# RunpeiDong/ACT

Hardware: AMD Instinct MI355X
Metric: stage2_pretrain_point_clouds_per_sec (higher is better)
Workload: dtype f32

## Files before the change

act_amd/_abi.py:

```python
import ctypes

_vp, _i, _f, _sz = ctypes.c_void_p, ctypes.c_int, ctypes.c_float, ctypes.c_size_t
_u, _u64, _ll, _str = ctypes.c_uint, ctypes.c_uint64, ctypes.c_longlong, ctypes.c_char_p
_d = ctypes.c_double
_P = ctypes.POINTER


class GemmEpilogue(ctypes.Structure):
    _fields_ = [("alpha", _f), ("act", _i), ("accumulate", _i), ("rows_per_scale", _i), ("ldr", _i), ("ldaux", _i),
                ("res_row_div", _i), ("bias", _vp), ("rowscale", _vp), ("res", _vp), ("aux", _vp)]


class GemmTnProblem(ctypes.Structure):
    _fields_ = [("A", _vp), ("lda", _i), ("B", _vp), ("ldb", _i), ("C", _vp), ("ldc", _i), ("M", _i), ("N", _i), ("bias_out", _vp)]


class GemmFx(ctypes.Structure):
    _fields_ = ([(n, _vp) for n in ("a_scale", "a_shift", "b_scale", "b_shift", "tile_stats", "gmax", "garg")] + [("group", _i), ("store_c", _i)]
                + [(n, _vp) for n in ("sa_src", "sa_arg", "ep_src", "ep_arg", "row_groups")])


class BlockParams(ctypes.Structure):
    _fields_ = [(n, _vp) for n in ("norm1_w", "norm1_b", "qkv_w", "qkv_b", "proj_w", "proj_b", "norm2_w", "norm2_b",
                                   "fc1_w", "fc1_b", "fc2_w", "fc2_b")]


class BlockDims(ctypes.Structure):
    _fields_ = [("B", _i), ("S", _i), ("D", _i), ("heads", _i), ("hidden", _i), ("eps", _f)]


class BlockStack(ctypes.Structure):
    _fields_ = [("depth", _i), ("blocks", _vp), ("gate1", _vp), ("gate2", _vp)]


class PrefixVit(ctypes.Structure):
    _fields_ = ([(n, _i) for n in ("B", "P", "G", "D", "heads", "hidden", "depth", "tokens_dims", "pos_hidden")] +
                [("eps", _f), ("drop_p", _f), ("seed_base", _u64), ("seed_dev", _vp)] +
                [(n, _vp) for n in ("pos_w0", "pos_b0", "pos_w1", "pos_b1", "pre_w", "pre_b", "post_w", "post_b", "norm_w", "norm_b")] +
                [("prompt_tok", _P(_vp)), ("prompt_pos", _P(_vp)), ("blocks", _P(BlockParams))])


class VitBf16x3(ctypes.Structure):
    _fields_ = [("w_planes", _vp), ("a_planes", _vp), ("a_planes_elems", _sz)]


class VitF16x3(ctypes.Structure):
    _fields_ = [("w_planes", _vp), ("w_inv_scale", _vp), ("a_scale", _vp), ("a_planes", _vp), ("a_planes_elems", _sz)]


class PointnetParams(ctypes.Structure):
    _fields_ = [(n, _vp) for n in ("c1_w", "c1_b", "bn1_w", "bn1_b", "c2_w", "c2_b", "c3_w", "c3_b", "bn2_w", "bn2_b", "c4_w", "c4_b",
                                   "bn1_mean", "bn1_var", "bn2_mean", "bn2_var")]


class PointnetGrads(ctypes.Structure):
    _fields_ = [(n, _vp) for n in ("c1_w", "c1_b", "bn1_w", "bn1_b", "c2_w", "c2_b", "c3_w", "c3_b", "bn2_w", "bn2_b", "c4_w", "c4_b")]


class PointnetDims(ctypes.Structure):
    _fields_ = [("BG", _i), ("n", _i), ("C", _i), ("eps1", _f), ("eps2", _f), ("momentum1", _f), ("momentum2", _f)]


class Dgcnn(ctypes.Structure):
    _fields_ = ([(n, _i) for n in ("B", "G", "k", "Cin", "Cout", "groups")] + [("eps", _f), ("slope", _f)] +
                [(n, _vp) for n in ("w_in", "b_in", "w5")] + [("stacked", _vp * 4), ("gn_w", _vp * 4), ("gn_b", _vp * 4)])


class DgcnnF16x3(ctypes.Structure):
    _fields_ = [("w5_planes", _vp), ("w5_inv_scale", _vp), ("a_scale", _f), ("a_planes", _vp), ("a_planes_elems", _sz)]


class AugmentOp(ctypes.Structure):
    _fields_ = [("kind", _i), ("p0", _f), ("p1", _f), ("p2", _f), ("draws", _vp), ("draws2", _vp)]


STRUCTS = {
    "act_gemm_epilogue_t": GemmEpilogue, "act_gemm_tn_problem_t": GemmTnProblem, "act_gemm_fx_t": GemmFx,
    "act_block_params_t": BlockParams, "act_block_grads_t": BlockParams, "act_block_dims_t": BlockDims, "act_block_stack_t": BlockStack,
    "act_prefix_vit_t": PrefixVit, "act_vit_bf16x3_t": VitBf16x3, "act_vit_f16x3_t": VitF16x3,
    "act_pointnet_params_t": PointnetParams,
    "act_pointnet_grads_t": PointnetGrads, "act_pointnet_dims_t": PointnetDims, "act_dgcnn_t": Dgcnn, "act_dgcnn_f16x3_t": DgcnnF16x3,
    "act_augment_op_t": AugmentOp,
}

_epi, _probs, _fx = _P(GemmEpilogue), _P(GemmTnProblem), _P(GemmFx)
_dims, _blk, _x3 = _P(BlockDims), _P(BlockParams), _P(VitBf16x3)
_pnd, _pnp = _P(PointnetDims), _P(PointnetParams)

_TABLE = {
    "act_version": [],
    "act_arch": (_str, []),
    "act_prof_enable": [_i],
    "act_prof_reset": [],
    "act_prof_num_kernels": [],
    "act_prof_kernel_name": (_str, [_i]),
    "act_prof_read": [_i, _vp, _vp, _vp, _vp],
    "act_fps_scratch_floats": (_sz, [_i, _i]),
    "act_fps_f32": [_vp, _i, _i, _i, _vp, _vp, _i, _vp, _vp],
    "act_fps_chain_probe": [_i, _i, _vp, _vp, _vp, _vp],
    "act_knn_group_f32": [_vp, _vp, _i, _i, _i, _i, _vp, _i, _vp, _vp, _vp],
    "act_gather_points_f32": [_vp, _vp, _i, _i, _i, _i, _vp, _vp],
    "act_gather_points_bwd_f32": [_vp, _vp, _i, _i, _i, _i, _vp, _vp],
    "act_scale_translate_f32": [_vp, _vp, _vp, _i, _i, _vp],
    "act_rotate_points_f32": [_vp, _vp, _i, _i, _vp],
    "act_augment_f32": [_vp, _i, _i, _P(AugmentOp), _i, _u64, _vp, _i, _vp],
    "act_chamfer_fwd_f32": [_vp, _vp, _i, _i, _i, _vp, _vp, _vp, _vp, _vp],
    "act_chamfer_fwd_ex_f32": [_vp, _vp, _i, _i, _i, _vp, _vp, _vp, _vp, _i, _vp],
    "act_chamfer_bwd_f32": [_vp, _vp, _vp, _vp, _vp, _vp, _i, _i, _i, _vp, _vp, _vp],
    "act_sgemm_f32": [_i, _i, _i, _i, _i, _vp, _i, _vp, _i, _vp, _i, _epi, _vp, _sz, _vp],
    "act_sgemm_ex_f32": [_i, _i, _i, _i, _i, _vp, _i, _vp, _i, _vp, _i, _epi, _vp, _sz, _i, _i, _vp],
    "act_sgemm_tn_grouped_workspace": (_sz, [_probs, _i, _i, _i]),
    "act_sgemm_tn_grouped_splits": [_probs, _i, _i],
    "act_sgemm_tn_grouped_f32": [_probs, _i, _i, _i, _vp, _sz, _vp],
    "act_sgemm_fx_tile_stats_floats": (_sz, [_i, _i]),
    "act_gemm_fx_asm": [_i],
    "act_sgemm_fx_f32": [_i, _i, _i, _i, _i, _vp, _i, _vp, _i, _vp, _i, _epi, _fx, _vp, _sz, _vp],
    "act_bn_tiles_finalize_f32": [_vp, _i, _i, _i, _vp, _vp, _f, _f, _vp, _vp, _vp, _vp, _vp, _vp, _vp],
    "act_layernorm_fwd_f32": [_vp, _vp, _vp, _vp, _vp, _vp, _vp, _vp, _i, _i, _f, _vp],
    "act_prompt_layernorm_fwd_f32": [_vp, _vp, _i, _i, _i, _f, _u64, _vp, _vp, _vp, _f, _vp, _vp],
    "act_prompt_rows_fwd_f32": [_vp, _vp, _vp, _i, _i, _i, _f, _u64, _vp, _vp],
    "act_prompt_rows_bwd_f32": [_vp, _vp, _i, _i, _i, _f, _u64, _vp, _vp, _vp],
    "act_layernorm_bwd_workspace": (_sz, [_i, _i]),
    "act_layernorm_bwd_f32": [_vp, _vp, _vp, _vp, _vp, _vp, _vp, _vp, _vp, _i, _vp, _sz, _i, _i, _vp],
    "act_colsum_workspace": (_sz, [_i, _i]),
    "act_colsum_f32": [_vp, _i, _i, _i, _vp, _i, _vp, _sz, _vp],
    "act_attention_fwd_f32": [_vp, _vp, _vp, _i, _i, _i, _i, _f, _vp],
    "act_attention_fwd_prefix_f32": [_vp, _i, _vp, _i, _vp, _vp, _i, _i, _i, _f, _vp],
    "act_attention_bwd_f32": [_vp, _vp, _vp, _vp, _vp, _i, _i, _i, _i, _f, _vp],
    "act_attention_bwd_prefix_f32": [_vp, _i, _vp, _i, _vp, _vp, _vp, _vp, _vp, _i, _i, _i, _f, _vp],
    "act_cosine_loss_fwd_f32": [_vp, _vp, _i, _i, _f, _vp, _vp, _vp, _vp],
    "act_cosine_loss_bwd_f32": [_vp, _vp, _vp, _vp, _i, _i, _f, _vp, _vp],
    "act_regression_loss_fwd_f32": [_vp, _vp, _i, _i, _i, _vp, _vp, _vp],
    "act_regression_loss_bwd_f32": [_vp, _vp, _vp, _i, _i, _i, _vp, _vp],
    "act_softmax_xent_fwd_f32": [_vp, _vp, _i, _i, _vp, _vp, _vp, _vp],
    "act_softmax_xent_bwd_f32": [_vp, _vp, _vp, _vp, _i, _i, _vp, _vp],
    "act_colstats_workspace": (_sz, [_i, _i]),
    "act_bn_stats_f32": [_vp, _i, _i, _vp, _vp, _f, _f, _vp, _vp, _vp, _vp, _vp, _vp, _vp, _sz, _vp],
    "act_affine_act_f32": [_vp, _vp, _vp, _i, _i, _i, _vp, _vp],
    "act_bn_bwd_f32": [_vp, _vp, _vp, _vp, _vp, _vp, _i, _i, _i, _vp, _vp, _vp, _vp, _sz, _vp],
    "act_bn_bwd_groups_f32": [_vp, _vp, _vp, _vp, _vp, _vp, _i, _i, _i, _vp, _i, _vp, _vp, _vp, _vp, _sz, _vp],
    "act_col_mean_var_f32": [_vp, _i, _i, _vp, _vp, _vp, _sz, _vp],
    "act_bn_bwd_sums_f32": [_vp, _vp, _vp, _vp, _vp, _vp, _i, _i, _i, _vp, _vp, _vp, _sz, _vp],
    "act_bn_bwd_apply_f32": [_vp, _vp, _vp, _vp, _vp, _vp, _vp, _vp, _f, _i, _i, _i, _vp, _vp],
    "act_group_max_f32": [_vp, _i, _i, _i, _vp, _vp, _vp],
    "act_group_max_bwd_f32": [_vp, _vp, _i, _i, _i, _i, _vp, _vp],
    "act_group_max_bwd_matmul_f32": [_vp, _vp, _i, _i, _i, _vp, _i, _i, _vp, _i, _vp],
    "act_group_live_i32": [_vp, _i, _i, _vp, _vp],
    "act_group_max_bwd_matmul_live_f32": [_vp, _vp, _i, _i, _i, _vp, _i, _i, _vp, _i, _vp, _vp],
    "act_group_max_bwd_wgrad_workspace": (_sz, [_i, _i, _i, _i]),
    "act_group_max_bwd_wgrad_f32": [_vp, _vp, _i, _i, _i, _vp, _i, _i, _vp, _vp, _vp, _i, _vp, _sz, _vp],
    "act_group_sum_f32": [_vp, _i, _i, _i, _vp, _vp],
    "act_edge_gn_lrelu_max_f32": [_vp, _i, _i, _vp, _i, _i, _i, _i, _i, _vp, _vp, _f, _f, _vp, _vp, _i, _i, _vp],
    "act_edge_gn_lrelu_max_bwd_f32": [_vp, _i, _i, _vp, _i, _i, _i, _i, _i, _vp, _vp, _vp, _f, _vp, _i, _vp, _vp, _vp, _vp],
    "act_edge_bwd_lds": [_i],
    "act_gn_gumbel_argmax_gather_f32": [_vp, _i, _i, _i, _i, _vp, _vp, _f, _f, _vp, _u64, _vp, _f, _vp, _i, _vp, _vp, _vp, _vp, _vp],
    "act_gumbel_softmax_fwd_f32": [_vp, _i, _i, _vp, _u64, _f, _vp, _vp],
    "act_gumbel_softmax_bwd_f32": [_vp, _vp, _i, _i, _f, _vp, _vp],
    "act_kl_uniform_fwd_f32": [_vp, _i, _i, _i, _vp, _vp, _vp, _vp],
    "act_kl_uniform_bwd_f32": [_vp, _vp, _vp, _vp, _i, _i, _i, _vp, _vp],
    "act_split_bf16x2_f32": [_vp, _i, _i, _i, _vp, _vp, _vp],
    "act_sgemm_nt_bf16x3_supported": [_i, _i, _i],
    "act_sgemm_nt_bf16x3_f32": [_i, _i, _i, _vp, _vp, _vp, _vp, _vp, _i, _epi, _vp],
    "act_layernorm_fwd_planes_f32": [_vp, _vp, _vp, _vp, _vp, _vp, _vp, _vp, _vp, _vp, _i, _i, _f, _vp],
    "act_prompt_layernorm_fwd_planes_f32": [_vp, _vp, _i, _i, _i, _f, _u64, _vp, _vp, _vp, _f, _vp, _vp, _vp],
    "act_attention_fwd_prefix_planes_f32": [_vp, _i, _vp, _i, _vp, _vp, _vp, _vp, _i, _i, _i, _f, _vp],
    "act_sgemm_nt_bf16x3_planes_f32": [_i, _i, _i, _vp, _vp, _vp, _vp, _vp, _i, _vp, _vp, _epi, _vp],
    "act_split_f16x2_f32": [_vp, _i, _i, _i, _f, _vp, _vp, _vp, _vp],
    "act_sgemm_nt_f16x3_supported": [_i, _i, _i],
    "act_sgemm_nt_f16x3_planes_f32": [_i, _i, _i, _vp, _vp, _f, _vp, _vp, _vp, _vp, _i, _vp, _vp, _f, _epi, _vp],
    "act_sgemm_nt_f16x3_pick_tile": [_i, _i, _i, _i],
    "act_sgemm_nt_f16x3_planes_tile_f32": [_i, _i, _i, _vp, _vp, _f, _vp, _vp, _vp, _vp, _i, _vp, _vp, _f, _epi, _vp, _i],
    "act_layernorm_fwd_f16_planes_f32": [_vp, _vp, _vp, _vp, _vp, _vp, _vp, _vp, _f, _vp, _vp, _i, _i, _f, _vp],
    "act_attention_fwd_prefix_f16_planes_f32": [_vp, _i, _vp, _i, _vp, _vp, _vp, _f, _vp, _i, _i, _i, _f, _vp],
    "act_gemm_tune_set": [_i] * 7,
    "act_gemm_tune_get": [_i] * 5 + [_P(_i), _P(_i)],
    "act_gemm_tune_clear": [],
    "act_gemm_tile_info": [_i] + [_P(_i)] * 4,
    "act_scale_rows_f32": [_vp, _vp, _i, _i, _i, _vp, _vp],
    "act_bn_eval_affine_f32": [_vp, _vp, _vp, _vp, _f, _i, _vp, _vp, _vp],
    "act_composite_collect_begin": [],
    "act_composite_collect_end": [_P(_i), _i],
    "act_composite_shutdown": [],
    "act_block_saved_floats": (_sz, [_dims]),
    "act_block_fwd_f32": [_dims, _blk, _vp, _vp, _vp, _vp, _i, _vp, _vp, _vp, _sz, _vp],
    "act_block_bwd_scratch_floats": (_sz, [_dims]),
    "act_block_bwd_f32": [_dims, _blk, _vp, _vp, _vp, _vp, _vp, _blk, _vp, _vp, _sz, _vp, _sz, _vp, _vp],
    "act_block_stack_saved_floats": (_sz, [_dims, _i, _i]),
    "act_block_stack_bwd_scratch_floats": (_sz, [_dims, _i]),
    "act_block_stack_fwd_f32": [_dims, _P(BlockStack), _vp, _vp, _i, _vp, _vp, _vp, _sz, _vp],
    "act_block_stack_bwd_f32": [_dims, _P(BlockStack), _vp, _vp, _vp, _vp, _vp, _vp, _vp, _vp, _sz, _vp, _sz, _vp, _vp],
    "act_add_f32": [_vp, _vp, _vp, _ll, _vp],
    "act_prefix_block_saved_floats": (_sz, [_dims, _i]),
    "act_prefix_block_fwd_f32": [_dims, _i, _blk, _vp, _vp, _vp, _vp, _i, _vp, _vp, _vp, _sz, _vp],
    "act_prefix_block_fwd_kv_f32": [_dims, _i, _blk, _vp, _vp, _vp, _vp, _vp, _vp, _sz, _vp],
    "act_prompt_kv_sparse": [_i],
    "act_prompt_kv_workspace": (_sz, [_i, _i, _i, _i]),
    "act_prompt_kv_fwd_f32": [_vp, _vp, _i, _i, _i, _i, _f, _u64, _vp, _vp, _vp, _f, _vp, _vp, _vp, _vp, _sz, _vp, _sz, _vp],
    "act_prefix_block_bwd_scratch_floats": (_sz, [_dims, _i]),
    "act_prefix_block_bwd_f32": [_dims, _i, _blk, _vp, _vp, _vp, _vp, _vp, _vp, _vp, _sz, _vp],
    "act_prefix_vit_scratch_floats": (_sz, [_P(PrefixVit)]),
    "act_prefix_vit_fwd_bf16x3_f32": [_P(PrefixVit), _x3, _vp, _vp, _vp, _vp, _vp, _sz, _vp],
    "act_prefix_block_fwd_bf16x3_f32": [_dims, _i, _blk, _x3, _vp, _vp, _vp, _i, _vp, _vp, _vp, _sz, _vp],
    "act_prefix_block_bwd_bf16x3_f32": [_dims, _i, _blk, _x3, _vp, _vp, _vp, _vp, _vp, _vp, _vp, _sz, _vp],
    "act_prefix_vit_fwd_f32": [_P(PrefixVit), _vp, _vp, _vp, _vp, _vp, _sz, _vp],
    "act_prefix_vit_fwd_f16x3_f32": [_P(PrefixVit), _P(VitF16x3), _vp, _vp, _vp, _vp, _vp, _sz, _vp],
    "act_pointnet_saved_floats": (_sz, [_pnd]),
    "act_pointnet_fwd_f32": [_pnd, _pnp, _vp, _i, _i, _vp, _vp, _vp, _sz, _vp],
    "act_pointnet_fwd_groups_f32": [_pnd, _pnp, _vp, _i, _i, _vp, _vp, _vp, _i, _vp, _sz, _vp],
    "act_pointnet_bwd_scratch_floats": (_sz, [_pnd]),
    "act_pointnet_bwd_f32": [_pnd, _pnp, _vp, _vp, _vp, _P(PointnetGrads), _vp, _vp, _sz, _vp],
    "act_dgcnn_scratch_floats": (_sz, [_P(Dgcnn)]),
    "act_dgcnn_features_f32": [_P(Dgcnn), _vp, _vp, _vp, _vp, _vp, _sz, _vp],
    "act_dgcnn_features_f16x3_f32": [_P(Dgcnn), _P(DgcnnF16x3), _vp, _vp, _vp, _vp, _vp, _sz, _vp],
    "act_three_nn_f32": [_vp, _vp, _i, _i, _i, _vp, _vp, _vp, _vp, _vp],
    "act_interp_rows_fwd_f32": [_vp, _vp, _vp, _vp, _vp, _vp, _i, _i, _i, _i, _vp, _vp],
    "act_interp_rows_bwd_f32": [_vp, _vp, _vp, _vp, _i, _i, _i, _i, _vp, _vp],
    "act_interp_xyz_grad_workspace": (_sz, [_ll, _i]),
    "act_interp_xyz_grad_f32": [_vp, _vp, _ll, _i, _vp, _vp, _vp, _sz, _vp],
    "act_log_softmax_fwd_f32": [_vp, _ll, _i, _vp, _vp],
    "act_log_softmax_bwd_f32": [_vp, _vp, _ll, _i, _vp, _vp],
    "act_nll_weighted_workspace": (_sz, [_ll]),
    "act_nll_weighted_fwd_f32": [_vp, _vp, _vp, _ll, _i, _vp, _vp, _vp, _vp, _sz, _vp],
    "act_nll_weighted_bwd_f32": [_vp, _vp, _vp, _vp, _ll, _i, _vp, _vp],
    "act_confusion_i64": [_vp, _vp, _ll, _i, _vp, _vp],
    "act_label_branch_fwd_f32": [_vp, _vp, _vp, _vp, _i, _i, _f, _f, _f, _vp, _vp, _vp, _vp],
    "act_label_branch_bwd_f32": [_vp, _vp, _vp, _vp, _vp, _i, _f, _f, _vp, _vp, _vp, _vp],
    "act_part_eval_f32": [_vp, _vp, _i, _i, _i, _vp, _vp, _i, _vp, _vp, _i, _i, _vp, _vp, _vp],
    "act_scene_member_workspace": (_sz, [_ll, _i, _i]),
    "act_scene_member_count": [_vp, _ll, _vp, _i, _i, _vp, _vp, _vp, _sz, _vp],
    "act_scene_member_fill": [_vp, _ll, _vp, _i, _i, _vp, _vp, _vp, _sz, _vp],
    "act_scene_rows": [_vp, _vp, _vp, _vp, _i, _ll, _i, _u, _u, _u, _vp, _vp],
    "act_scene_gather": [_vp, _ll, _vp, _vp, _vp, _vp, _i, _ll, _vp, _vp],
    "act_scene_vote": [_vp, _vp, _ll, _ll, _i, _vp, _vp, _vp, _vp],
    "act_scene_finish": [_vp, _vp, _ll, _i, _vp, _vp, _vp],
    "act_s3dis_sample_workspace": (_sz, [_i, _ll]),
    "act_s3dis_sample_f32": [_vp, _vp, _vp, _i, _vp, _vp, _vp, _vp, _d, _d, _i, _i, _ll, _vp, _vp, _vp, _i, _i, _u, _u, _vp, _vp, _vp, _vp, _vp, _vp,
                             _vp, _sz, _vp],
    "act_cloud_sample_max_points": [],
    "act_cloud_sample_f32": [_vp, _ll, _i, _i, _vp, _vp, _i, _i, _u, _u, _i, _vp, _vp, _vp],
    "act_recon_eval_f32": [_vp, _vp, _vp, _i, _i, _i, _i, _f, _vp, _i, _i, _vp],
    "act_svm_scores_f32": [_vp, _vp, _vp, _vp, _i, _i, _i, _vp, _vp],
    "act_svm_hinge_workspace": (_sz, [_i, _i]),
    "act_svm_hinge_f32": [_vp, _vp, _vp, _i, _i, _vp, _vp, _vp, _sz, _vp],
    "act_svm_tprod_workspace": (_sz, [_i, _i, _i]),
    "act_svm_tprod_f32": [_vp, _vp, _i, _i, _i, _vp, _vp, _vp, _sz, _vp],
    "act_svm_newton_workspace": (_sz, [_i, _i, _i]),
    "act_svm_newton_f32": [_vp, _vp, _vp, _i, _i, _i, _f, _f, _i, _vp, _vp, _vp, _vp, _vp, _sz, _vp],
    "act_tsne_knn_workspace": (_sz, [_i, _i]),
    "act_tsne_knn_cosine_f32": [_vp, _i, _i, _i, _vp, _vp, _vp, _sz, _vp],
    "act_tsne_conditional_p_f32": [_vp, _i, _i, _f, _vp, _vp, _vp],
    "act_tsne_symmetrize_workspace": (_sz, [_i, _i]),
    "act_tsne_symmetrize_f32": [_vp, _vp, _i, _i, _vp, _vp, _vp, _ll, _vp, _sz, _vp],
    "act_tsne_step_workspace": (_sz, [_i]),
    "act_tsne_step_f32": [_vp, _vp, _vp, _i, _f, _f, _f, _vp, _vp, _vp, _vp, _sz, _vp],
    "act_tsne_steps_f32": [_vp, _vp, _vp, _i, _i, _f, _f, _f, _vp, _vp, _vp, _vp, _sz, _vp],
    "act_tsne_kl_f32": [_vp, _vp, _vp, _vp, _i, _vp, _vp, _sz, _vp],
    "act_tsne_pca_workspace": (_sz, [_i, _i]),
    "act_tsne_pca_init_f32": [_vp, _i, _i, _vp, _vp, _vp, _sz, _vp],
    "act_dropout_add_layernorm_fwd_f32": [_vp, _vp, _vp, _i, _i, _f, _u64, _vp, _vp, _vp, _f, _vp, _vp, _vp],
    "act_dropout_add_layernorm_bwd_f32": [_vp, _vp, _vp, _i, _i, _f, _u64, _vp, _vp, _vp, _vp, _vp, _vp, _vp],
    "act_attention_dropout_fwd_f32": [_vp, _vp, _vp, _vp, _i, _i, _i, _i, _f, _f, _u64, _vp, _vp],
    "act_attention_dropout_bwd_f32": [_vp, _vp, _vp, _vp, _vp, _vp, _vp, _i, _i, _i, _i, _f, _f, _u64, _vp, _vp],
    "act_quickgelu_fwd_f32": [_vp, _vp, _i, _i, _vp],
    "act_quickgelu_bwd_f32": [_vp, _vp, _vp, _i, _i, _vp],
    "act_knn_probe_normalize_f32": [_vp, _i, _i, _vp, _vp],
    "act_knn_probe_splits": [_i, _i, _i, _i],
    "act_knn_probe_workspace": (_sz, [_i, _i, _i, _i, _i]),
    "act_knn_probe_search_f32": [_vp, _i, _vp, _i, _i, _i, _i, _i, _i, _vp, _vp, _vp, _sz, _vp],
    "act_knn_probe_vote_f32": [_vp, _vp, _i, _i, _vp, _i, _vp, _i, _P(_i), _i, _f, _vp, _vp, _vp, _vp],
    "act_emd_max_points": [],
    "act_emd_fwd_f32": [_vp, _vp, _i, _i, _f, _i, _vp, _vp, _vp, _vp],
    "act_emd_fwd_ex_f32": [_vp, _vp, _i, _i, _f, _i, _vp, _vp, _vp, _vp, _vp],
    "act_emd_bwd_f32": [_vp, _vp, _vp, _vp, _i, _i, _vp, _vp, _vp],
    "act_emd_wave_max_points": [],
    "act_emd_wave_fwd_f32": [_vp, _vp, _i, _i, _f, _f, _i, _vp, _vp, _vp, _vp, _vp],
    "act_ball_query_f32": [_vp, _vp, _i, _i, _i, _f, _i, _i, _vp, _vp, _vp],
    "act_group_rows_fwd_f32": [_vp, _vp, _vp, _vp, _i, _i, _i, _i, _i, _i, _vp, _vp],
    "act_group_rows_bwd_workspace": (_sz, [_i, _i, _i, _i]),
    "act_group_rows_bwd_f32": [_vp, _vp, _i, _i, _i, _i, _i, _i, _vp, _vp, _sz, _vp],
    "act_group_gather_f32": [_vp, _vp, _i, _i, _i, _i, _i, _vp, _vp],
    "act_group_gather_bwd_f32": [_vp, _vp, _i, _i, _i, _i, _i, _vp, _vp, _sz, _vp],
    "act_three_nn_any_f32": [_vp, _vp, _i, _i, _i, _vp, _vp, _vp, _vp, _vp, _vp],
    "act_three_adj_i32": [_vp, _i, _i, _i, _vp, _vp, _vp],
    "act_interp_rows_any_fwd_f32": [_vp, _vp, _vp, _i, _i, _i, _i, _vp, _vp],
    "act_interp_rows_any_bwd_f32": [_vp, _vp, _vp, _vp, _i, _i, _i, _i, _vp, _vp],
    "act_knn_feat_f32": [_vp, _i, _i, _i, _i, _vp, _vp, _vp],
    "act_edge_bn_workspace": (_sz, [_i, _i, _i, _i]),
    "act_edge_bn_lrelu_max_fwd_f32": [_vp, _i, _i, _vp, _i, _i, _i, _i, _vp, _vp, _vp, _vp, _i, _f, _f, _f, _vp, _i, _i, _vp, _vp, _vp, _vp,
                                      _vp, _vp, _sz, _vp],
    "act_edge_bn_lrelu_max_bwd_f32": [_vp, _i, _i, _vp, _i, _i, _i, _i, _vp, _vp, _vp, _vp, _vp, _f, _vp, _vp, _vp, _i, _vp, _vp, _vp, _vp, _sz, _vp],
    "act_affine_lrelu_f32": [_vp, _vp, _vp, _f, _i, _i, _vp, _vp],
    "act_bn_lrelu_bwd_workspace": (_sz, [_i, _i]),
    "act_bn_lrelu_bwd_f32": [_vp, _vp, _vp, _vp, _vp, _vp, _f, _i, _i, _vp, _vp, _vp, _vp, _sz, _vp],
}

SIGNATURES = {name: sig if isinstance(sig, tuple) else (_i, sig) for name, sig in _TABLE.items()}
```

act_amd/composite.py:

```python
import ctypes
import math
import os
import weakref

import torch

from . import _C
from . import kernels as K
from ._abi import BlockDims, BlockParams, BlockStack, Dgcnn, PointnetDims, PointnetGrads, PointnetParams, PrefixVit, VitBf16x3, VitF16x3, DgcnnF16x3
from ._abi import GemmFx

lib, check = _C.lib, _C.check
_vp, _i = ctypes.c_void_p, ctypes.c_int

ENABLED = os.environ.get("ACT_COMPOSITE", "1") != "0"


def _p(t):
    if t is None:
        return None
    if not t.is_cuda or not t.is_contiguous():
        raise _C.ActHipError("act_amd kernels need contiguous CUDA tensors (there is no CPU fallback)")
    _C._same_device(t)
    return t.data_ptr()


K.publish_table()
_TUNED = set()
_SHAPE_BUF = (_i * (5 * 256))()


def _tune_shape(ak, bk, M, N, Kd, device):
    return lib.act_gemm_tune_get(ak, bk, M, N, Kd, None, None) == 0 or K.gemm_config(ak, bk, M, N, Kd, device, publish=True) is not None


def ensure_tuned(key, call, device):
    if key in _TUNED:
        return
    check(lib.act_composite_collect_begin(), "act_composite_collect_begin")
    try:
        rc = call()
    finally:
        n = lib.act_composite_collect_end(_SHAPE_BUF, 256)
    check(rc, "composite dry call")
    done = True
    for i in range(min(n, 256)):
        done = _tune_shape(*[int(_SHAPE_BUF[5 * i + j]) for j in range(5)], device) and done
    if done:
        _TUNED.add(key)


def reset_tuning():
    _TUNED.clear()
    lib.act_gemm_tune_clear()
    K.publish_table()


def shutdown():
    torch.cuda.synchronize()
    return int(lib.act_composite_shutdown())


_DIMS = {}


def _block_dims(B, S, D, heads, hidden, eps):
    key = (B, S, D, heads, hidden, float(eps))
    d = _DIMS.get(key)
    if d is None:
        d = BlockDims(B, S, D, heads, hidden, float(eps))
        _DIMS[key] = d = (d, int(lib.act_block_saved_floats(ctypes.byref(d))), int(lib.act_block_bwd_scratch_floats(ctypes.byref(d))))
    return d


def _block_params(n1w, n1b, wqkv, bqkv, wproj, bproj, n2w, n2b, w1, b1, w2, b2):
    return BlockParams(_p(n1w), _p(n1b), _p(wqkv), _p(bqkv), _p(wproj), _p(bproj), _p(n2w), _p(n2b), _p(w1), _p(b1), _p(w2), _p(b2))


class BlockFn(torch.autograd.Function):

    @staticmethod
    def forward(ctx, x, pos, gate1, gate2, n1w, n1b, wqkv, bqkv, wproj, bproj, n2w, n2b, w1, b1, w2, b2, heads, eps, train_w):
        B, S, D = x.shape
        dev = x.device
        dims, n_saved, _ = _block_dims(B, S, D, heads, w1.shape[0], eps)
        x2d = K._f32c(x).reshape(B * S, D)
        pos2d = K._f32c(pos).reshape(B * S, D) if pos is not None else None
        need_grad = any(ctx.needs_input_grad)
        prm = _block_params(n1w, n1b, wqkv, bqkv, wproj, bproj, n2w, n2b, w1, b1, w2, b2)
        saved = torch.empty(n_saved, dtype=torch.float32, device=dev)
        out = torch.empty(B, S, D, dtype=torch.float32, device=dev)
        ws = K.workspace(dev)
        args = (ctypes.byref(dims), ctypes.byref(prm), _p(x2d), _p(pos2d), _p(gate1), _p(gate2), int(need_grad), _p(saved), _p(out),
                _p(ws), ws.numel() * 4)
        ensure_tuned(("blk_fwd", B, S, D, heads, w1.shape[0]), lambda: lib.act_block_fwd_f32(*args, _C.stream()), dev)
        check(lib.act_block_fwd_f32(*args, _C.stream()), "act_block_fwd_f32")
        if need_grad:
            ctx.save_for_backward(saved, gate1, gate2, n1w, wqkv, bqkv, wproj, n2w, w1, w2)
            ctx.dims = (B, S, D, heads, w1.shape[0], eps)
            ctx.has_pos = pos is not None
            ctx.train_w = int(train_w)
        return out

    @staticmethod
    def backward(ctx, dout):
        saved, gate1, gate2, n1w, wqkv, bqkv, wproj, n2w, w1, w2 = ctx.saved_tensors
        B, S, D, heads, hidden, eps = ctx.dims
        dev = dout.device
        dims, _, n_scratch = _block_dims(B, S, D, heads, hidden, eps)
        dout = K._f32c(dout).reshape(B * S, D)
        tw = ctx.train_w
        prm = _block_params(n1w, None, wqkv, bqkv, wproj, None, n2w, None, w1, None, w2, None)
        dx = torch.empty(B, S, D, dtype=torch.float32, device=dev)
        scratch = torch.empty(n_scratch, dtype=torch.float32, device=dev)
        grads, gp = (None,) * 12, None
        if tw:
            e = lambda *shape: torch.empty(*shape, dtype=torch.float32, device=dev)
            grads = (e(D), e(D), e(3 * D, D), e(3 * D) if bqkv is not None else None, e(D, D), e(D), e(D), e(D),
                     e(hidden, D), e(hidden), e(D, hidden), e(D))
            gp = ctypes.byref(BlockParams(*[_p(g) for g in grads]))
        ws = K.workspace(dev)
        side, sws = None, None
        if tw == 2 and K.OVERLAP_DW:
            side = K.side_stream(dev, 1).cuda_stream
            sws = K.workspace(dev, stream_handle=side)
        args = (ctypes.byref(dims), ctypes.byref(prm), _p(gate1), _p(gate2), _p(saved), _p(dout), _p(dx), gp, _p(scratch),
                _p(ws), ws.numel() * 4, _p(sws), (sws.numel() * 4 if sws is not None else 0))
        ensure_tuned(("blk_bwd", B, S, D, heads, hidden, bool(tw)), lambda: lib.act_block_bwd_f32(*args, _C.stream(), side), dev)
        check(lib.act_block_bwd_f32(*args, _C.stream(), side), "act_block_bwd_f32")
        dg1, dbt1, dwqkv, dbqkv, dwproj, dbproj, dg2, dbt2, dw1, db1, dw2, db2 = grads
        return (dx, dx if ctx.has_pos else None, None, None, dg1, dbt1, dwqkv, dbqkv, dwproj, dbproj, dg2, dbt2,
                dw1, db1, dw2, db2, None, None, None)


STACK = os.environ.get("ACT_BLOCK_STACK", "1") != "0"
STACK_CHUNK = int(os.environ.get("ACT_BLOCK_STACK_CHUNK", "0"))
_SDIMS = {}
_NPB = 12


def _stack_dims(B, S, D, heads, hidden, eps, depth):
    key = (B, S, D, heads, hidden, float(eps), depth)
    d = _SDIMS.get(key)
    if d is None:
        dims = BlockDims(B, S, D, heads, hidden, float(eps))
        r = ctypes.byref(dims)
        _SDIMS[key] = d = (dims, int(lib.act_block_stack_saved_floats(r, depth, 1)), int(lib.act_block_stack_saved_floats(r, depth, 0)),
                           int(lib.act_block_stack_bwd_scratch_floats(r, depth)))
    return d


def _ptr_array(tensors, dev_index):
    ptrs = []
    for t in tensors:
        if t is None:
            ptrs.append(None)
            continue
        if not t.is_cuda or not t.is_contiguous() or t.device.index != dev_index:
            raise _C.ActHipError("act_amd kernels need contiguous CUDA tensors on the current device (there is no CPU fallback)")
        ptrs.append(t.data_ptr())
    return (_vp * len(ptrs))(*ptrs)


class BlockStackFn(torch.autograd.Function):

    @staticmethod
    def forward(ctx, x, pos, gates, heads, eps, train_w, emit_pos, *params):
        B, S, D = x.shape
        dev = x.device
        depth = len(params) // _NPB
        hidden = params[8].shape[0]
        dims, n_keep, n_nokeep, _ = _stack_dims(B, S, D, heads, hidden, eps, depth)
        _C._same_device(x)
        x2d = K._f32c(x).reshape(B * S, D)
        pos2d = K._f32c(pos).reshape(B * S, D) if pos is not None else None
        need_grad = any(ctx.needs_input_grad)
        parr = _ptr_array(params, dev.index)
        g1 = g2 = None
        gts = ()
        if gates is not None and any(g is not None for g in gates):
            gts = tuple(t for g in gates for t in (g if g is not None else (None, None)))
            g1, g2 = _ptr_array(gts[0::2], dev.index), _ptr_array(gts[1::2], dev.index)
        st = BlockStack(depth, ctypes.cast(parr, _vp), ctypes.cast(g1, _vp) if g1 is not None else None,
                        ctypes.cast(g2, _vp) if g2 is not None else None)
        saved = torch.empty(n_keep if need_grad else n_nokeep, dtype=torch.float32, device=dev)
        out = torch.empty(B, S, D, dtype=torch.float32, device=dev)
        ws = K.workspace(dev)
        args = (ctypes.byref(dims), ctypes.byref(st), x2d.data_ptr(), pos2d.data_ptr() if pos2d is not None else None, int(need_grad),
                saved.data_ptr(), out.data_ptr(), ws.data_ptr(), ws.numel() * 4)
        ensure_tuned(("stack_fwd", B, S, D, heads, hidden, depth), lambda: lib.act_block_stack_fwd_f32(*args, _C.stream()), dev)
        check(lib.act_block_stack_fwd_f32(*args, _C.stream()), "act_block_stack_fwd_f32")
        ctx.set_materialize_grads(False)
        if need_grad:
            ctx.save_for_backward(saved, *[t for t in params if t is not None], *[t for t in gts if t is not None])
            ctx.layout = ([t is not None for t in params], [t is not None for t in gts])
            ctx.dims = (B, S, D, heads, hidden, eps, depth)
            ctx.has_pos = pos is not None
            ctx.train_w = int(train_w)
        return (out, pos) if emit_pos else out

    @staticmethod
    def backward(ctx, dout, dpos_in=None):
        sv = ctx.saved_tensors
        saved = sv[0]
        B, S, D, heads, hidden, eps, depth = ctx.dims
        dev = saved.device
        it = iter(sv[1:])
        params = tuple(next(it) if has else None for has in ctx.layout[0])
        gts = tuple(next(it) if has else None for has in ctx.layout[1])
        parr = _ptr_array(params, dev.index)
        g1 = g2 = None
        if gts:
            g1, g2 = _ptr_array(gts[0::2], dev.index), _ptr_array(gts[1::2], dev.index)
        st = BlockStack(depth, ctypes.cast(parr, _vp), ctypes.cast(g1, _vp) if g1 is not None else None,
                        ctypes.cast(g2, _vp) if g2 is not None else None)
        dims, _, _, n_scratch = _stack_dims(B, S, D, heads, hidden, eps, depth)
        tw = ctx.train_w
        dx = torch.empty(B, S, D, dtype=torch.float32, device=dev)
        if dout is None:
            dout = torch.zeros(B * S, D, dtype=torch.float32, device=dev)
        dout = K._f32c(dout).reshape(B * S, D)
        if dpos_in is not None:
            dpos_in = K._f32c(dpos_in).reshape(B * S, D)
        dpos = torch.empty(B, S, D, dtype=torch.float32, device=dev) if (ctx.has_pos and (depth > 1 or dpos_in is not None)) else None
        scratch = torch.empty(n_scratch, dtype=torch.float32, device=dev)
        grads, garr = (None,) * len(params), None
        if tw:
            grads = tuple(torch.empty_like(t) if t is not None else None for t in params)
            garr = _ptr_array(grads, dev.index)
        ws = K.workspace(dev)
        side, sws = None, None
        if tw == 2 and K.OVERLAP_DW:
            side = K.side_stream(dev, 1).cuda_stream
            sws = K.workspace(dev, stream_handle=side)
        args = (ctypes.byref(dims), ctypes.byref(st), saved.data_ptr(), dout.data_ptr(), dx.data_ptr(), dpos.data_ptr() if dpos is not None else None,
                dpos_in.data_ptr() if (dpos_in is not None and dpos is not None) else None,
                ctypes.cast(garr, _vp) if garr is not None else None, scratch.data_ptr(), ws.data_ptr(), ws.numel() * 4,
                sws.data_ptr() if sws is not None else None, (sws.numel() * 4 if sws is not None else 0))
        ensure_tuned(("stack_bwd", B, S, D, heads, hidden, depth, bool(tw)), lambda: lib.act_block_stack_bwd_f32(*args, _C.stream(), side), dev)
        check(lib.act_block_stack_bwd_f32(*args, _C.stream(), side), "act_block_stack_bwd_f32")
        return (dx, (dpos if dpos is not None else dx) if ctx.has_pos else None, None, None, None, None, None) + grads


_LEAVES = weakref.WeakKeyDictionary()
_VIT_LEAVES = weakref.WeakKeyDictionary()
_VIT_STRUCT = weakref.WeakKeyDictionary()
_VIT_PLANES = weakref.WeakKeyDictionary()
TEACHER_BF16X3 = os.environ.get("ACT_TEACHER_BF16X3", "0") == "1"
TEACHER_BF16X3_BWD = os.environ.get("ACT_TEACHER_BF16X3_BWD", "1") == "1"
TEACHER_F16X3 = os.environ.get("ACT_TEACHER_F16X3", "1") != "0"
_VIT_F16 = weakref.WeakKeyDictionary()
TOKENIZER_F16X3 = os.environ.get("ACT_TOKENIZER_F16X3", "1") != "0"
_DGCNN_F16 = weakref.WeakKeyDictionary()


def _stack_leaves(blocks):
    cache = _LEAVES.get(blocks)
    if cache is None or len(cache) != len(blocks) or any(c[6] is not b for c, b in zip(cache, blocks)):
        cache = _LEAVES[blocks] = [(b.norm1, b.attn.qkv, b.attn.proj, b.norm2, b.mlp.fc1, b.mlp.fc2, b) for b in blocks]
    return cache


def _stock_blocks(blocks):
    from act_amd.models.act import Block
    for b in blocks:
        if type(b).forward is not Block.forward or b._forward_hooks or b._forward_pre_hooks or b._backward_hooks or b._backward_pre_hooks:
            return False
    return True


def block_stack(blocks, x, pos, gates, draws=None, tag="enc", chunk=None, taps=False):
    n = len(blocks)

    def per_block(x, draws):
        outs = []
        every = chunk if chunk else n
        for i, blk in enumerate(blocks):
            x = blk(x, pos, draws, f"{tag}.{i}", gates[i] if gates is not None else None)
            if (i + 1) % every == 0 or i == n - 1:
                outs.append(x)
        return outs if taps else x
    if not (ENABLED and STACK) or n == 0 or not _stock_blocks(blocks):
        return per_block(x, draws)
    if draws is not None:
        gates = [blk.gates(x.shape[0], x.device, draws, f"{tag}.{i}") for i, blk in enumerate(blocks)]
        gates = [tuple(g) if g[0] is not None else None for g in gates]
    leaves = _stack_leaves(blocks)
    b0 = blocks[0]
    heads, eps, tw = b0.attn.num_heads, b0.norm1.eps, (2 if b0.overlap_wgrad else 1)
    if any(l[6].attn.num_heads != heads or l[0].eps != eps or l[3].eps != eps or bool(l[6].overlap_wgrad) != bool(b0.overlap_wgrad) for l in leaves[1:]):
        return per_block(x, None)
    if chunk is None:
        chunk = STACK_CHUNK
    chunk = chunk if chunk > 0 else n
    carry = pos is not None and chunk < n and torch.is_grad_enabled() and pos.requires_grad
    outs = []
    for c0 in range(0, n, chunk):
        params = []
        for n1, qkv, proj, n2, fc1, fc2, _ in leaves[c0:c0 + chunk]:
            p1, pq, pp, p2, pf1, pf2 = n1._parameters, qkv._parameters, proj._parameters, n2._parameters, fc1._parameters, fc2._parameters
            params += [p1["weight"], p1["bias"], pq["weight"], pq["bias"], pp["weight"], pp["bias"], p2["weight"], p2["bias"],
                       pf1["weight"], pf1["bias"], pf2["weight"], pf2["bias"]]
        emit = carry and c0 + chunk < n
        r = BlockStackFn.apply(x, pos, gates[c0:c0 + chunk] if gates is not None else None, heads, eps, tw, emit, *params)
        x, pos = r if emit else (r, pos)
        outs.append(x)
    return outs if taps else x


_PDIMS = {}


def _prefix_dims(B, G, D, heads, hidden, eps, P):
    key = (B, G, D, heads, hidden, float(eps), P)
    d = _PDIMS.get(key)
    if d is None:
        d = BlockDims(B, G, D, heads, hidden, float(eps))
        _PDIMS[key] = d = (d, int(lib.act_prefix_block_saved_floats(ctypes.byref(d), P)),
                           int(lib.act_prefix_block_bwd_scratch_floats(ctypes.byref(d), P)))
    return d


class PrefixBlockFn(torch.autograd.Function):

    @staticmethod
    def forward(ctx, x2d, pos2d, prm2d, B, P, G, n1w, n1b, wqkv, bqkv, wproj, bproj, n2w, n2b, w1, b1, w2, b2, heads, eps):
        D = x2d.shape[1]
        dev = x2d.device
        dims, n_saved, _ = _prefix_dims(B, G, D, heads, w1.shape[0], eps, P)
        x2d, pos2d, prm2d = K._f32c(x2d), K._f32c(pos2d), K._f32c(prm2d)
        prm = _block_params(n1w, n1b, wqkv, bqkv, wproj, bproj, n2w, n2b, w1, b1, w2, b2)
        saved = torch.empty(n_saved, dtype=torch.float32, device=dev)
        out = torch.empty(B * G, D, dtype=torch.float32, device=dev)
        ws = K.workspace(dev)
        args = (ctypes.byref(dims), P, ctypes.byref(prm), _p(x2d), _p(pos2d), _p(prm2d), None, 1, _p(saved), _p(out), _p(ws), ws.numel() * 4)
        ensure_tuned(("pfx_fwd", B, G, D, heads, w1.shape[0], P), lambda: lib.act_prefix_block_fwd_f32(*args, _C.stream()), dev)
        if TEACHER_BF16X3 and not any(w.requires_grad for w in (wqkv, wproj, w1, w2)):
            x3, keep = _block_planes((wqkv, wproj, w1, w2), B * G * w1.shape[0] + B * max(G, P) * D, dev)
            check(lib.act_prefix_block_fwd_bf16x3_f32(*args[:3], ctypes.byref(x3), *args[3:6], 1, *args[8:], _C.stream()), "act_prefix_block_fwd_bf16x3_f32")
            del keep
            ctx.x3 = True
        else:
            check(lib.act_prefix_block_fwd_f32(*args, _C.stream()), "act_prefix_block_fwd_f32")
            ctx.x3 = False
        ctx.save_for_backward(saved, prm2d, n1w, wqkv, wproj, n2w, w1, w2)
        ctx.dims = (B, P, G, D, heads, w1.shape[0], eps)
        return out

    @staticmethod
    def backward(ctx, dout):
        saved, prm2d, n1w, wqkv, wproj, n2w, w1, w2 = ctx.saved_tensors
        B, P, G, D, heads, hidden, eps = ctx.dims
        dev = dout.device
        dims, _, n_scratch = _prefix_dims(B, G, D, heads, hidden, eps, P)
        dout = K._f32c(dout)
        prm = _block_params(n1w, None, wqkv, None, wproj, None, n2w, None, w1, None, w2, None)
        dx = torch.empty(B * G, D, dtype=torch.float32, device=dev)
        dprm = torch.empty(B * P, D, dtype=torch.float32, device=dev)
        scratch = torch.empty(n_scratch, dtype=torch.float32, device=dev)
        ws = K.workspace(dev)
        args = (ctypes.byref(dims), P, ctypes.byref(prm), _p(prm2d), _p(saved), _p(dout), _p(dx), _p(dprm), _p(scratch), _p(ws), ws.numel() * 4)
        ensure_tuned(("pfx_bwd", B, G, D, heads, hidden, P), lambda: lib.act_prefix_block_bwd_f32(*args, _C.stream()), dev)
        if ctx.x3 and TEACHER_BF16X3_BWD:
            x3, keep = _block_planes((wqkv, wproj, w1, w2), B * G * hidden + B * max(G, P) * D, dev, transposed=True)
            check(lib.act_prefix_block_bwd_bf16x3_f32(*args[:3], ctypes.byref(x3), *args[3:], _C.stream()), "act_prefix_block_bwd_bf16x3_f32")
            del keep
            return (dx, dx, dprm) + (None,) * 17
        check(lib.act_prefix_block_bwd_f32(*args, _C.stream()), "act_prefix_block_bwd_f32")
        return (dx, dx, dprm) + (None,) * 17


def block_forward_prefix(x2d, pos2d, prm2d, B, P, G, n1w, n1b, wqkv, bqkv, wproj, bproj, n2w, n2b, w1, b1, w2, b2, heads, eps, n1p=None, kvp=None):
    D = x2d.shape[1]
    dev = x2d.device
    dims, n_saved, _ = _prefix_dims(B, G, D, heads, w1.shape[0], eps, P)
    x2d, pos2d = K._f32c(x2d), K._f32c(pos2d)
    prm2d = K._f32c(prm2d) if prm2d is not None else None
    n1p = K._f32c(n1p) if n1p is not None else None
    prm = _block_params(n1w, n1b, wqkv, bqkv, wproj, bproj, n2w, n2b, w1, b1, w2, b2)
    tmp = torch.empty(n_saved, dtype=torch.float32, device=dev)
    out = torch.empty(B * G, D, dtype=torch.float32, device=dev)
    ws = K.workspace(dev)
    if kvp is not None:
        kargs = (ctypes.byref(dims), P, ctypes.byref(prm), _p(x2d), _p(pos2d), _p(K._f32c(kvp)), _p(tmp), _p(out), _p(ws), ws.numel() * 4)
        ensure_tuned(("pfx_fwd_kv", B, G, D, heads, w1.shape[0], P), lambda: lib.act_prefix_block_fwd_kv_f32(*kargs, _C.stream()), dev)
        check(lib.act_prefix_block_fwd_kv_f32(*kargs, _C.stream()), "act_prefix_block_fwd_kv_f32")
        return out
    args = (ctypes.byref(dims), P, ctypes.byref(prm), _p(x2d), _p(pos2d), _p(prm2d), _p(n1p), 0, _p(tmp), _p(out), _p(ws), ws.numel() * 4)
    ensure_tuned(("pfx_fwd", B, G, D, heads, w1.shape[0], P), lambda: lib.act_prefix_block_fwd_f32(*args, _C.stream()), dev)
    check(lib.act_prefix_block_fwd_f32(*args, _C.stream()), "act_prefix_block_fwd_f32")
    return out


def _vit_tensors(tok):
    lv = _VIT_LEAVES.get(tok)
    blocks = tok.visual_embed[0]
    if lv is None or lv[0] is not blocks:
        vp = tok.visual_pos_embed
        lv = _VIT_LEAVES[tok] = (blocks, vp[0], vp[2], tok.proj_pre, tok.proj_post, tok.visual_embed[1])
    _, vp0, vp2, pre, post, nrm = lv
    ts = []
    for m in (vp0, vp2, pre, post, nrm):
        pr = m._parameters
        ts += [pr["weight"], pr["bias"]]
    for n1, qkv, proj, n2, fc1, fc2, _ in _stack_leaves(blocks):
        p1, pq, pp, p2, pf1, pf2 = n1._parameters, qkv._parameters, proj._parameters, n2._parameters, fc1._parameters, fc2._parameters
        ts += [p1["weight"], p1["bias"], pq["weight"], pq["bias"], pp["weight"], pp["bias"], p2["weight"], p2["bias"],
               pf1["weight"], pf1["bias"], pf2["weight"], pf2["bias"]]
    tp = tok._parameters
    ts += [tp["visual_prompt_token"], tp["visual_prompt_pos"], tp.get("deep_prompt_tokens"), tp.get("deep_prompt_pos")]
    return ts, blocks


def prefix_vit_forward(tok, tokens, center, drop_p, seed_base, seed_dev):
    B, G, td = tokens.shape
    dev = tokens.device
    ts, blocks = _vit_tensors(tok)
    depth = tok.visual_embed_depth
    sig = (B, G, td, dev.index, depth, tuple([t.data_ptr() if t is not None else 0 for t in ts]))
    cache = _VIT_STRUCT.get(tok)
    if cache is None or cache[0] != sig:
        Pn, D = tok.num_prompt_token, tok.visual_embed_dim
        b0 = blocks[0]
        if depth > 1 and (ts[-2] is None or ts[-1] is None):
            raise _C.ActHipError("prefix_vit_forward: a depth > 1 prompt-tuned Transformer needs deep_prompt_tokens / deep_prompt_pos")
        ptr = _ptr_array(ts, dev.index)
        m = PrefixVit()
        m.B, m.P, m.G, m.D, m.heads, m.hidden, m.depth, m.tokens_dims, m.pos_hidden = (B, Pn, G, D, b0.num_heads, ts[18].shape[0], depth, td,
                                                                                        ts[0].shape[0])
        m.eps = float(b0.eps)
        (m.pos_w0, m.pos_b0, m.pos_w1, m.pos_b1, m.pre_w, m.pre_b, m.post_w, m.post_b, m.norm_w, m.norm_b) = [ptr[i] for i in range(10)]
        row = Pn * D * 4
        nb = 10 + _NPB * depth
        toks = (_vp * depth)(*[ptr[nb] if i == 0 else ptr[nb + 2] + (i - 1) * row for i in range(depth)])
        poss = (_vp * depth)(*[ptr[nb + 1] if i == 0 else ptr[nb + 3] + (i - 1) * row for i in range(depth)])
        blks = (_vp * (_NPB * depth))(*[ptr[10 + i] for i in range(_NPB * depth)])
        m.prompt_tok, m.prompt_pos, m.blocks = toks, poss, ctypes.cast(blks, ctypes.POINTER(BlockParams))
        n_scratch = int(lib.act_prefix_vit_scratch_floats(ctypes.byref(m)))
        cache = _VIT_STRUCT[tok] = (sig, m, n_scratch, (toks, poss, blks, ptr))
    _, m, n_scratch, _ = cache
    m.drop_p, m.seed_base, m.seed_dev = float(drop_p), int(seed_base) & (2 ** 64 - 1), _p(seed_dev)
    scratch = torch.empty(n_scratch, dtype=torch.float32, device=dev)
    out = torch.empty(B, G, td, dtype=torch.float32, device=dev)
    ws = K.workspace(dev)
    tokens, center = K._f32c(tokens), K._f32c(center)
    args = (ctypes.byref(m), _p(tokens), _p(center), _p(out), _p(scratch), _p(ws), ws.numel() * 4)
    ensure_tuned(("vit", B, m.P, G, m.D, m.heads, m.hidden, depth, td), lambda: lib.act_prefix_vit_fwd_f32(*args, _C.stream()), dev)
    if TEACHER_BF16X3:
        x3, keep = _vit_planes(tok, ts, depth, B * G * m.hidden + B * max(G, m.P) * m.D, dev)
        check(lib.act_prefix_vit_fwd_bf16x3_f32(args[0], ctypes.byref(x3), *args[1:], _C.stream()), "act_prefix_vit_fwd_bf16x3_f32")
        del keep
        return out
    if TEACHER_F16X3:
        x3, keep = _vit_f16_planes(tok, ts, depth, B * G * m.hidden + B * max(G, m.P) * m.D, dev)
        check(lib.act_prefix_vit_fwd_f16x3_f32(args[0], ctypes.byref(x3), *args[1:], _C.stream()), "act_prefix_vit_fwd_f16x3_f32")
        del keep
        return out
    check(lib.act_prefix_vit_fwd_f32(*args, _C.stream()), "act_prefix_vit_fwd_f32")
    return out


_BLOCK_PLANES = {}


def _block_planes(ws_, act_elems, dev, transposed=False):
    sig = tuple((w.data_ptr(), w._version) for w in ws_)
    key = (id(ws_[0]), transposed)
    cache = _BLOCK_PLANES.get(key)
    if cache is None or cache[0]() is not ws_[0] or cache[1] != sig:
        with torch.no_grad():
            if transposed:
                wqkv, wproj, w1, w2 = (w.detach() for w in ws_)
                D = wqkv.shape[1]
                src = [w2.t(), w1.t(), wproj.t(), wqkv.t(), wqkv[D:].t()]
            else:
                src = [w.detach() for w in ws_]
            planes = [K.split_bf16x2(w.contiguous()) for w in src]
        parr = (_vp * len(planes))(*[pl.data_ptr() for pl in planes])
        cache = _BLOCK_PLANES[key] = (weakref.ref(ws_[0], lambda _, k=key: _BLOCK_PLANES.pop(k, None)), sig, planes, parr)
    a_planes = torch.empty(2 * act_elems, dtype=torch.bfloat16, device=dev)
    return VitBf16x3(ctypes.cast(cache[3], _vp), a_planes.data_ptr(), a_planes.numel()), (a_planes, cache)


def _vit_planes(tok, ts, depth, act_elems, dev):
    ws_ = [ts[10 + _NPB * i + j] for i in range(depth) for j in (2, 4, 8, 10)]
    sig = tuple((w.data_ptr(), w._version) for w in ws_)
    cache = _VIT_PLANES.get(tok)
    if cache is None or cache[0] != sig:
        with torch.no_grad():
            planes = [K.split_bf16x2(w.detach()) for w in ws_]
        parr = (_vp * len(planes))(*[pl.data_ptr() for pl in planes])
        cache = _VIT_PLANES[tok] = (sig, planes, parr)
    a_planes = torch.empty(2 * act_elems, dtype=torch.bfloat16, device=dev)
    x3 = VitBf16x3(ctypes.cast(cache[2], _vp), a_planes.data_ptr(), a_planes.numel())
    return x3, (a_planes, cache)


def f16x3_act_scale(bound):
    bound = float(bound)
    if not math.isfinite(bound) or bound > 32768.0:
        return 0.0
    if bound < 2.0 ** -15:
        return 2.0 ** 30
    s = 2.0 ** (math.frexp(32768.0 / bound)[1] - 1)
    return s if bound * s <= 32768.0 else s / 2


def f16x3_vit_bounds(ts, depth, D):
    rows, rt = [], math.sqrt(D)
    for i in range(depth):
        n1w, n1b, wqkv, bqkv, _, _, n2w, n2b, w1, b1 = (None if t is None else t.detach().double() for t in ts[10 + _NPB * i: 20 + _NPB * i])
        u1, u2 = rt * n1w.abs() + n1b.abs(), rt * n2w.abs() + n2b.abs()
        v = wqkv[2 * D:].abs() @ u1 + (bqkv[2 * D:].abs() if bqkv is not None else 0)
        h = w1.abs() @ u2 + (b1.abs() if b1 is not None else 0)
        rows.append(torch.stack([u1.max(), v.max(), u2.max(), h.max()]))
    return torch.stack(rows)


def _vit_f16_planes(tok, ts, depth, act_elems, dev):
    blk = ts[10:10 + _NPB * depth]
    sig = tuple((t.data_ptr(), t._version) if t is not None else None for t in blk)
    cache = _VIT_F16.get(tok)
    if cache is None or cache[0] != sig:
        ws_ = [ts[10 + _NPB * i + j] for i in range(depth) for j in (2, 4, 8, 10)]
        with torch.no_grad():
            scales = [K.f16x3_row_scales(w) for w in ws_]
            planes = [K.split_f16x2(w.detach(), 1.0, sc[0]) for w, sc in zip(ws_, scales)]
            inv = [sc[1].contiguous() for sc in scales]
            a_scale = [f16x3_act_scale(b) for b in f16x3_vit_bounds(ts, depth, ws_[0].shape[1]).flatten().tolist()]
        parr = (_vp * len(planes))(*[pl.data_ptr() for pl in planes])
        iarr = (_vp * len(inv))(*[t.data_ptr() for t in inv])
        sarr = (ctypes.c_float * len(a_scale))(*a_scale)
        cache = _VIT_F16[tok] = (sig, planes, inv, a_scale, (parr, iarr, sarr))
    a_planes = torch.empty(2 * act_elems, dtype=torch.float16, device=dev)
    parr, iarr, sarr = cache[4]
    x3 = VitF16x3(ctypes.cast(parr, _vp), ctypes.cast(iarr, _vp), ctypes.cast(sarr, _vp), a_planes.data_ptr(), a_planes.numel())
    return x3, (a_planes, cache)


def _pointnet_structs(enc, BG, n):
    c1, bn1, _, c2 = enc.first_conv
    c3, bn2, _, c4 = enc.second_conv
    dims = PointnetDims(BG, n, c4.weight.shape[0], float(bn1.eps), float(bn2.eps), float(bn1.momentum), float(bn2.momentum))
    return dims, (c1, bn1, c2, c3, bn2, c4)


class PointnetFn(torch.autograd.Function):

    @staticmethod
    def forward(ctx, x, c1w, c1b, g1, b1, c2w, c2b, c3w, c3b, g2, b2, c4w, c4b, buffers, dims, training, groups=None):
        dev = x.device
        x = K._f32c(x)
        need_grad = any(ctx.needs_input_grad)
        prm = PointnetParams(*[_p(t) for t in (c1w, c1b, g1, b1, c2w, c2b, c3w, c3b, g2, b2, c4w, c4b) + tuple(buffers)])
        saved = torch.empty(int(lib.act_pointnet_saved_floats(ctypes.byref(dims))), dtype=torch.float32, device=dev)
        out = torch.empty(dims.BG, dims.C, dtype=torch.float32, device=dev)
        ws = K.workspace(dev)
        ng = 0 if groups is None else int(groups.numel())
        args = (ctypes.byref(dims), ctypes.byref(prm), _p(x), int(training), int(need_grad), _p(saved), _p(out),
                _p(groups) if ng else None, ng, _p(ws), ws.numel() * 4)
        ensure_tuned(("pn_fwd", dims.BG, dims.n, dims.C, ng), lambda: lib.act_pointnet_fwd_groups_f32(*args, _C.stream()), dev)
        check(lib.act_pointnet_fwd_groups_f32(*args, _C.stream()), "act_pointnet_fwd_groups_f32")
        if need_grad:
            ctx.save_for_backward(x, saved, c1w, c1b, g1, b1, c2w, c2b, c3w, c3b, g2, b2, c4w, c4b)
            ctx.dims, ctx.training = dims, bool(training)
        return out

    @staticmethod
    def backward(ctx, dout):
        if not ctx.training:
            raise NotImplementedError("mini-PointNet backward in eval mode (running statistics) is off the training path")
        x, saved = ctx.saved_tensors[:2]
        params = ctx.saved_tensors[2:]
        dims = ctx.dims
        dev = dout.device
        dout = K._f32c(dout)
        prm = PointnetParams(*([_p(t) for t in params] + [None] * 4))
        grads = tuple(torch.empty_like(t) for t in params)
        gp = PointnetGrads(*[_p(g) for g in grads])
        scratch = torch.empty(int(lib.act_pointnet_bwd_scratch_floats(ctypes.byref(dims))), dtype=torch.float32, device=dev)
        ws = K.workspace(dev)
        args = (ctypes.byref(dims), ctypes.byref(prm), _p(x), _p(saved), _p(dout), ctypes.byref(gp), _p(scratch), _p(ws), ws.numel() * 4)
        ensure_tuned(("pn_bwd", dims.BG, dims.n, dims.C), lambda: lib.act_pointnet_bwd_f32(*args, _C.stream()), dev)
        check(lib.act_pointnet_bwd_f32(*args, _C.stream()), "act_pointnet_bwd_f32")
        return (None,) + grads + (None, None, None, None)


def pointnet_forward(enc, point_groups, need=None):
    bs, g, n, _ = point_groups.shape
    groups = None
    if need is not None and need.shape[1] < g and n in (32, 64):
        ids = (need + torch.arange(bs, device=need.device).unsqueeze(1) * g).reshape(-1).to(torch.int32)
        pad = (-ids.numel()) % (128 // n)
        groups = torch.cat([ids, ids[-1:].expand(pad)]) if pad else ids
        groups = groups.contiguous()
    dims, (c1, bn1, c2, c3, bn2, c4) = _pointnet_structs(enc, bs * g, n)
    training = enc.training
    if training:
        for bn in (bn1, bn2):
            if bn.num_batches_tracked is not None:
                bn.num_batches_tracked.add_(1)
    w2 = lambda c: c.weight.view(c.weight.shape[0], c.weight.shape[1])
    out = PointnetFn.apply(point_groups.reshape(bs * g * n, 3), w2(c1), c1.bias, bn1.weight, bn1.bias, w2(c2), c2.bias, w2(c3), c3.bias,
                           bn2.weight, bn2.bias, w2(c4), c4.bias,
                           (bn1.running_mean, bn1.running_var, bn2.running_mean, bn2.running_var), dims, training, groups)
    return out.reshape(bs, g, dims.C)


def dgcnn_features(dg, f, idx, stacked):
    B, G, Cin = f.shape
    dev = f.device
    w5 = dg.layer5[0].weight
    m = Dgcnn()
    gn0 = dg.layer1[1]
    m.B, m.G, m.k, m.Cin, m.Cout, m.groups = B, G, idx.shape[1], Cin, w5.shape[0], gn0.num_groups
    m.eps, m.slope = float(gn0.eps), 0.2
    m.w_in, m.b_in, m.w5 = _p(dg.input_trans.weight), _p(dg.input_trans.bias), _p(w5)
    for l, layer in enumerate((dg.layer1, dg.layer2, dg.layer3, dg.layer4)):
        m.stacked[l], m.gn_w[l], m.gn_b[l] = _p(stacked[l]), _p(layer[1].weight), _p(layer[1].bias)
    scratch = torch.empty(int(lib.act_dgcnn_scratch_floats(ctypes.byref(m))), dtype=torch.float32, device=dev)
    h = torch.empty(B * G, m.Cout, dtype=torch.float32, device=dev)
    ws = K.workspace(dev)
    f = K._f32c(f)
    args = (ctypes.byref(m), _p(f), _p(idx), _p(h), _p(scratch), _p(ws), ws.numel() * 4)
    ensure_tuned(("dgcnn", B, G, Cin, m.Cout), lambda: lib.act_dgcnn_features_f32(*args, _C.stream()), dev)
    if TOKENIZER_F16X3 and m.Cout >= 1024:
        x3, keep = _dgcnn_f16_planes(dg, B * G, G, m.k, dev)
        check(lib.act_dgcnn_features_f16x3_f32(args[0], ctypes.byref(x3), *args[1:], _C.stream()), "act_dgcnn_features_f16x3_f32")
        del keep
        return h
    check(lib.act_dgcnn_features_f32(*args, _C.stream()), "act_dgcnn_features_f32")
    return h


def f16x3_dgcnn_bound(gmax, bmax, couts, groups, G, k):
    return max(math.sqrt((c // g) * G * k) * gm + bm for gm, bm, c, g in zip(gmax, bmax, couts, groups))


def _dgcnn_f16_planes(dg, T, G, k, dev):
    gns = [layer[1] for layer in (dg.layer1, dg.layer2, dg.layer3, dg.layer4)]
    w5 = dg.layer5[0].weight
    sig = tuple((t.data_ptr(), t._version) for t in [w5] + [t for gn in gns for t in (gn.weight, gn.bias)])
    cache = _DGCNN_F16.get(dg)
    if cache is None or cache[0] != sig:
        with torch.no_grad():
            w = w5.detach().reshape(w5.shape[0], w5.shape[1])
            scale, inv = K.f16x3_row_scales(w)
            planes = K.split_f16x2(w, 1.0, scale)
            inv = inv.contiguous()
            mx = torch.stack([t.detach().double().abs().max() for gn in gns for t in (gn.weight, gn.bias)]).tolist()
        cache = _DGCNN_F16[dg] = (sig, planes, inv, mx[0::2], mx[1::2], [gn.num_channels for gn in gns], [gn.num_groups for gn in gns], {})
    _, planes, inv, gmax, bmax, couts, groups, scales = cache
    a_scale = scales.get((G, k))
    if a_scale is None:
        a_scale = scales[(G, k)] = f16x3_act_scale(f16x3_dgcnn_bound(gmax, bmax, couts, groups, G, k))
    a_planes = torch.empty(2 * T * planes.shape[2], dtype=torch.float16, device=dev)
    x3 = DgcnnF16x3(planes.data_ptr(), inv.data_ptr(), a_scale, a_planes.data_ptr(), a_planes.numel())
    return x3, (a_planes, cache)
```

act_amd/csrc/composite.hip:

```cpp
#include "common.h"
#include "split_planes.h"
#include <atomic>
#include <mutex>
#include <unordered_map>
#include <vector>
#include <stdlib.h>

#define CK(expr) do { const int rc__ = (expr); if (rc__ != 0) return rc__; } while (0)
#define RUN(expr) do { if (!t_collect) { const int rc__ = (expr); if (rc__ != 0) return rc__; } } while (0)

namespace {

struct GemmShape { int ak, bk, M, N, K; };
thread_local std::vector<GemmShape>* t_collect = nullptr;
inline bool collecting(int ak, int bk, int M, int N, int K) {
    if (!t_collect) return false;
    t_collect->push_back({ak, bk, M, N, K});
    return true;
}

struct EventRing {
    std::vector<hipEvent_t> ev;
    size_t next = 0;
    hipEvent_t get() {
// ... 507 lines not shown
}
static bool bad_vit(const act_prefix_vit_t* m) {
    return !m || m->B <= 0 || m->P <= 0 || m->G <= 0 || m->D <= 0 || m->heads <= 0 || m->D % m->heads || m->hidden <= 0 || m->depth <= 0 ||
           m->tokens_dims <= 0 || m->pos_hidden <= 0;
}
size_t act_prefix_vit_scratch_floats(const act_prefix_vit_t* m) {
    if (bad_vit(m)) return 0;
    float *a, *b, *c, *d, *e, *f, *g;
    return carve_vit(nullptr, *m, a, b, c, d, e, f, g);
}

static int prefix_vit_fwd(const act_prefix_vit_t* m, const act_vit_bf16x3_t* x3, const act_vit_f16x3_t* h3, const float* tokens, const float* center, float* out,
                          float* scratch, float* ws, size_t wsb, act_stream_t stream);
int act_prefix_vit_fwd_f32(const act_prefix_vit_t* m, const float* tokens, const float* center, float* out, float* scratch, float* ws,
                           size_t wsb, act_stream_t stream) {
    return prefix_vit_fwd(m, nullptr, nullptr, tokens, center, out, scratch, ws, wsb, stream);
}
int act_prefix_vit_fwd_bf16x3_f32(const act_prefix_vit_t* m, const act_vit_bf16x3_t* x3, const float* tokens, const float* center, float* out,
                                  float* scratch, float* ws, size_t wsb, act_stream_t stream) {
    if (!x3 || !x3->w_planes || !x3->a_planes) return ACT_E_NULLPTR;
    return prefix_vit_fwd(m, x3, nullptr, tokens, center, out, scratch, ws, wsb, stream);
}
int act_prefix_vit_fwd_f16x3_f32(const act_prefix_vit_t* m, const act_vit_f16x3_t* h3, const float* tokens, const float* center, float* out,
                                 float* scratch, float* ws, size_t wsb, act_stream_t stream) {
    if (!h3 || !h3->w_planes || !h3->w_inv_scale || !h3->a_scale || !h3->a_planes) return ACT_E_NULLPTR;
    return prefix_vit_fwd(m, nullptr, h3, tokens, center, out, scratch, ws, wsb, stream);
}
static int prefix_vit_fwd(const act_prefix_vit_t* m, const act_vit_bf16x3_t* x3, const act_vit_f16x3_t* h3, const float* tokens, const float* center, float* out,
                          float* scratch, float* ws, size_t wsb, act_stream_t stream) {
    if (bad_vit(m)) return ACT_E_BADARG;
    if (!tokens || !center || !out || !scratch || !m->blocks || !m->prompt_tok || !m->prompt_pos) return ACT_E_NULLPTR;
    hipStream_t s = (hipStream_t)stream;
    const int TG = m->B * m->G, D = m->D;
    float *pos_h, *pos, *xa, *xb, *n1p, *blk, *feat, *pkv;
    carve_vit(scratch, *m, pos_h, pos, xa, xb, n1p, blk, feat, &pkv);
    const size_t pkv_bytes = act_prompt_kv_workspace(m->B, m->P, m->D, 2 * m->D);
    const act_block_dims_t d{m->B, m->G, m->D, m->heads, m->hidden, m->eps};
    PrefixSaved sv; carve_prefix(blk, d, m->P, sv);
    act_gemm_epilogue_t e = epi0(); e.bias = m->pos_b0; e.act = ACT_EPI_GELU;
    CK(gemm_nt(TG, m->pos_hidden, 3, center, 3, m->pos_w0, 3, pos_h, m->pos_hidden, e, ws, wsb, s));
    e = epi0(); e.bias = m->pos_b1;
    CK(gemm_nt(TG, D, m->pos_hidden, pos_h, m->pos_hidden, m->pos_w1, m->pos_hidden, pos, D, e, ws, wsb, s));
    e = epi0(); e.bias = m->pre_b;
    CK(gemm_nt(TG, D, m->tokens_dims, tokens, m->tokens_dims, m->pre_w, m->tokens_dims, xa, D, e, ws, wsb, s));
    float* cur = xa; float* nxt = xb;
    for (int i = 0; i < m->depth; ++i) {
        const act_block_params_t& w = m->blocks[i];
        const uint64_t seed = (m->seed_base + 7919ull * (uint64_t)(i + 1)) & ((1ull << 62) - 1);
        X3Block hb{};
        if (h3) {
            hb.a_planes = h3->a_planes; hb.a_elems = h3->a_planes_elems;
            const size_t sD = D, sHd = m->hidden, elems[4] = {3 * sD * sD, sD * sD, sHd * sD, sD * sHd};
            X3Linear* lin[4] = {&hb.qkv, &hb.proj, &hb.fc1, &hb.fc2};
            for (int j = 0; j < 4; ++j) {
                const float sa = h3->a_scale[4 * i + j];
                if (sa > 0.f && h3->w_planes[4 * i + j] && h3->w_inv_scale[4 * i + j])
                    *lin[j] = x3_linear_of(h3->w_planes[4 * i + j], elems[j], PlaneFmt::f16(sa), h3->w_inv_scale[4 * i + j]);
            }
        }
        if (!x3) {
            const int rc = act_prompt_kv_fwd_f32(m->prompt_tok[i], m->prompt_pos[i], m->B, m->P, D, 2 * D, m->drop_p, seed, m->seed_dev, w.norm1_w, w.norm1_b,
                                                 m->eps, w.qkv_w + (size_t)D * D, w.qkv_b ? w.qkv_b + D : nullptr, sv.kvp, pkv, pkv_bytes, ws, wsb, stream);
            if (rc == 0) {
                (void)collecting(1, 1, m->B * m->P, 2 * D, D);
                CK(prefix_block_core(d, m->P, w, cur, pos, nullptr, false, sv, nxt, ws, wsb, s, h3 ? &hb : nullptr, true));
                float* t = cur; cur = nxt; nxt = t;
                continue;
            }
            if (rc != ACT_E_UNSUPPORTED) return rc;
        }
        X3Block xb{};
        if (x3) xb = x3_block_bf16(d, x3->w_planes + 4 * i, x3->a_planes, x3->a_planes_elems);
        if (x3 && x3_fits(d, m->P, x3->a_planes_elems) && x3_takes(xb.kv, m->B * m->P, 2 * D, D)) {
            uint16_t* tp = x3->a_planes + (size_t)2 * TG * m->hidden;
            RUN(act_prompt_layernorm_fwd_planes_f32(m->prompt_tok[i], m->prompt_pos[i], m->B, m->P, D, m->drop_p, seed, m->seed_dev, w.norm1_w, w.norm1_b,
                                                   m->eps, tp, tp + (size_t)m->B * m->P * D, s));
            xb.n1p_is_planes = true;
        } else
        RUN(act_prompt_layernorm_fwd_f32(m->prompt_tok[i], m->prompt_pos[i], m->B, m->P, D, m->drop_p, seed, m->seed_dev, w.norm1_w, w.norm1_b,
                                        m->eps, n1p, s));
        CK(prefix_block_core(d, m->P, w, cur, pos, n1p, false, sv, nxt, ws, wsb, s, x3 ? &xb : (h3 ? &hb : nullptr)));
        float* t = cur; cur = nxt; nxt = t;
    }
    RUN(act_layernorm_fwd_f32(cur, nullptr, m->norm_w, m->norm_b, nullptr, feat, nullptr, nullptr, TG, D, m->eps, s));
    e = epi0(); e.bias = m->post_b;
    CK(gemm_nt(TG, m->tokens_dims, D, feat, D, m->post_w, D, out, m->tokens_dims, e, ws, wsb, s));
    return 0;
}

namespace {
struct PnSaved { float *h1, *a1, *h2, *fg, *gw, *h3, *a3, *h4, *st1, *st2, *tstats, *w32, *b32; int32_t *arg1, *arg2; };
bool pn_fused(const act_pointnet_dims_t& d) {
    static const bool on = [] { const char* e = getenv("ACT_PN_FUSE"); return !(e && e[0] == '0'); }();
    const long long R = (long long)d.BG * d.n;
    return on && (d.n == 32 || d.n == 64) && R % 128 == 0 && d.C % 64 == 0;
}
bool pn_compose(const act_pointnet_dims_t& d) {
    static const bool on = [] { const char* e = getenv("ACT_PN_COMPOSE"); return !(e && e[0] == '0'); }();
    return on && pn_fused(d);
}
bool pn_pool_bwd_on_load(const act_pointnet_dims_t& d) {
    static const bool on = [] { const char* e = getenv("ACT_PN_POOL_BWD_FUSE"); return !(e && e[0] == '0'); }();
    return on && pn_fused(d) && d.C % 128 == 0;
}
bool pn_pool_bwd_sparse() {
    static const bool on = [] { const char* e = getenv("ACT_PN_POOL_BWD_SPARSE"); return !(e && e[0] == '0'); }();
    return on;
}
bool pn_pool_bwd_live() {
    static const bool on = [] { const char* e = getenv("ACT_POOL_BWD_LIVE"); return !(e && e[0] == '0'); }();
    return on;
}
size_t carve_pn(float* base, const act_pointnet_dims_t& d, PnSaved& sv) {
    const size_t R = (size_t)d.BG * d.n, BG = d.BG, C = d.C;
    const bool fused = pn_fused(d), composed = pn_compose(d);
    Carver c(base);
    sv.h1 = c.take(R * 128); sv.h2 = composed ? nullptr : c.take(R * 256); sv.fg = c.take(BG * 256); sv.gw = c.take(BG * 512); sv.h3 = c.take(R * 512);
    sv.w32 = composed ? c.take(512 * 128) : nullptr; sv.b32 = composed ? c.take(512) : nullptr;
    sv.st1 = c.take(4 * 128); sv.st2 = c.take(4 * 512);
    sv.arg1 = reinterpret_cast<int32_t*>(c.take(BG * 256)); sv.arg2 = reinterpret_cast<int32_t*>(c.take(BG * C));
    if (fused) { sv.a1 = sv.a3 = sv.h4 = nullptr; sv.tstats = c.take(act_sgemm_fx_tile_stats_floats((int)R, 512)); }
    else { sv.a1 = c.take(R * 128); sv.a3 = c.take(R * 512); sv.h4 = c.take(R * C); sv.tstats = nullptr; }
    return c.used;
}
struct PnBwdScratch { float *dh4, *da3, *dh3, *dgw, *dh2, *dfg, *da1, *dh1, *act, *g32; int32_t* live; };
size_t carve_pn_bwd(float* base, const act_pointnet_dims_t& d, PnBwdScratch& sc) {
    const size_t R = (size_t)d.BG * d.n, BG = d.BG, C = d.C;
    Carver c(base);
    sc.dh4 = pn_pool_bwd_on_load(d) ? nullptr : c.take(R * C); sc.da3 = c.take(R * 512); sc.dh3 = c.take(R * 512); sc.dgw = c.take(BG * 512);
    const bool composed = pn_compose(d);
    sc.dh2 = composed ? nullptr : c.take(R * 256); sc.g32 = composed ? c.take(512 * 128) : nullptr;
    sc.dfg = c.take(BG * 256); sc.da1 = c.take(R * 128); sc.dh1 = c.take(R * 128);
    sc.act = (pn_fused(d) && d.C % 128 != 0) ? c.take(R * 512) : nullptr;
    sc.live = reinterpret_cast<int32_t*>(c.take(BG));
    return c.used;
}
bool bad_pn(const act_pointnet_dims_t* d) { return !d || d->BG <= 0 || d->n <= 0 || d->C <= 0 || (d->C & 3); }

int gemm_fx(int ak, int bk, int M, int N, int K, const float* A, int lda, const float* B, int ldb, float* C, int ldc, const act_gemm_epilogue_t& e,
            const act_gemm_fx_t& fx, float* ws, size_t wsb, hipStream_t s) {
    if (collecting(ak, bk, M, N, K)) return 0;
    return act_sgemm_fx_f32(ak, bk, M, N, K, A, lda, B, ldb, C, ldc, &e, &fx, ws, wsb, s);
}
}

size_t act_pointnet_saved_floats(const act_pointnet_dims_t* d) { if (bad_pn(d)) return 0; PnSaved sv; return carve_pn(nullptr, *d, sv); }
size_t act_pointnet_bwd_scratch_floats(const act_pointnet_dims_t* d) { if (bad_pn(d)) return 0; PnBwdScratch sc; return carve_pn_bwd(nullptr, *d, sc); }

int act_pointnet_fwd_f32(const act_pointnet_dims_t* d, const act_pointnet_params_t* w, const float* x, int training, int keep_for_backward,
                         float* saved, float* out, float* ws, size_t wsb, act_stream_t stream) {
    return act_pointnet_fwd_groups_f32(d, w, x, training, keep_for_backward, saved, out, nullptr, 0, ws, wsb, stream);
}

int act_pointnet_fwd_groups_f32(const act_pointnet_dims_t* d, const act_pointnet_params_t* w, const float* x, int training, int keep_for_backward,
                                float* saved, float* out, const int32_t* groups, int n_groups, float* ws, size_t wsb, act_stream_t stream) {
    if (!w || !x || !saved || !out) return ACT_E_NULLPTR;
    if (bad_pn(d)) return ACT_E_BADARG;
    if (groups && (n_groups <= 0 || ((long long)n_groups * d->n) % 128)) return ACT_E_BADARG;
    if (groups && !pn_fused(*d)) groups = nullptr;
    hipStream_t s = (hipStream_t)stream;
    const int BG = d->BG, n = d->n, C = d->C, R = BG * n;
    const bool fused = pn_fused(*d), composed = pn_compose(*d);
    PnSaved sv; carve_pn(saved, *d, sv);
    float *scale1 = sv.st1 + 2 * 128, *shift1 = sv.st1 + 3 * 128, *scale2 = sv.st2 + 2 * 512, *shift2 = sv.st2 + 3 * 512;
    auto stats = [&](const float* h, int Cc, const float* g_, const float* b_, float* rm, float* rv, float eps, float mom, float* st) -> int {
        if (training) {
            if (wsb < act_colstats_workspace(R, Cc)) return ACT_E_BADARG;
            RUN(act_bn_stats_f32(h, R, Cc, g_, b_, eps, mom, rm, rv, st, st + Cc, st + 2 * Cc, st + 3 * Cc, ws, wsb, s));
        } else {
            RUN(act_bn_eval_affine_f32(g_, b_, rm, rv, eps, Cc, st + 2 * Cc, st + 3 * Cc, s));
        }
        return 0;
    };
    act_gemm_epilogue_t e = epi0(); e.bias = w->c1_b;
    CK(gemm_nt(R, 128, 3, x, 3, w->c1_w, 3, sv.h1, 128, e, ws, wsb, s));
    CK(stats(sv.h1, 128, w->bn1_w, w->bn1_b, w->bn1_mean, w->bn1_var, d->eps1, d->momentum1, sv.st1));
    if (!fused) {
        RUN(act_affine_act_f32(sv.h1, scale1, shift1, 1, R, 128, sv.a1, s));
        e = epi0(); e.bias = w->c2_b;
        CK(gemm_nt(R, 256, 128, sv.a1, 128, w->c2_w, 128, sv.h2, 256, e, ws, wsb, s));
        RUN(act_group_max_f32(sv.h2, BG, n, 256, sv.fg, sv.arg1, s));
    } else {
        act_gemm_fx_t fx{}; fx.a_scale = scale1; fx.a_shift = shift1; fx.gmax = sv.fg; fx.garg = sv.arg1; fx.group = n; fx.store_c = composed ? 0 : 1;
        e = epi0(); e.bias = w->c2_b;
        CK(gemm_fx(1, 1, R, 256, 128, sv.h1, 128, w->c2_w, 128, sv.h2, 256, e, fx, ws, wsb, s));
    }
    if (composed) {
        CK(gemm_nn(512, 128, 256, w->c3_w + 256, 512, w->c2_w, 128, sv.w32, 128, epi0(), ws, wsb, s));
        CK(gemm_nt(1, 512, 256, w->c2_b, 256, w->c3_w + 256, 512, sv.b32, 512, epi0(), ws, wsb, s));
    }
    e = epi0(); e.bias = w->c3_b;
    CK(gemm_nt(BG, 512, 256, sv.fg, 256, w->c3_w, 512, sv.gw, 512, e, ws, wsb, s));
    e = epi0(); e.res = sv.gw; e.ldr = 512; e.res_row_div = n;
    if (!fused) {
        CK(gemm_nt(R, 512, 256, sv.h2, 256, w->c3_w + 256, 512, sv.h3, 512, e, ws, wsb, s));
        CK(stats(sv.h3, 512, w->bn2_w, w->bn2_b, w->bn2_mean, w->bn2_var, d->eps2, d->momentum2, sv.st2));
        RUN(act_affine_act_f32(sv.h3, scale2, shift2, 1, R, 512, sv.a3, s));
        e = epi0(); e.bias = w->c4_b;
        CK(gemm_nt(R, C, 512, sv.a3, 512, w->c4_w, 512, sv.h4, C, e, ws, wsb, s));
        RUN(act_group_max_f32(sv.h4, BG, n, C, out, keep_for_backward ? sv.arg2 : nullptr, s));
        return 0;
    }
    if (composed) {
        e.bias = sv.b32;
        act_gemm_fx_t fx{}; fx.a_scale = scale1; fx.a_shift = shift1; fx.tile_stats = training ? sv.tstats : nullptr; fx.store_c = 1;
        CK(gemm_fx(1, 1, R, 512, 128, sv.h1, 128, sv.w32, 128, sv.h3, 512, e, fx, ws, wsb, s));
        if (training) RUN(act_bn_tiles_finalize_f32(sv.tstats, R / 128, 128, 512, w->bn2_w, w->bn2_b, d->eps2, d->momentum2, w->bn2_mean, w->bn2_var, sv.st2,
                                                    sv.st2 + 512, scale2, shift2, s));
        else RUN(act_bn_eval_affine_f32(w->bn2_w, w->bn2_b, w->bn2_mean, w->bn2_var, d->eps2, 512, scale2, shift2, s));
    } else if (training) {
        act_gemm_fx_t fx{}; fx.tile_stats = sv.tstats; fx.store_c = 1;
        CK(gemm_fx(1, 1, R, 512, 256, sv.h2, 256, w->c3_w + 256, 512, sv.h3, 512, e, fx, ws, wsb, s));
        RUN(act_bn_tiles_finalize_f32(sv.tstats, R / 128, 128, 512, w->bn2_w, w->bn2_b, d->eps2, d->momentum2, w->bn2_mean, w->bn2_var, sv.st2, sv.st2 + 512,
                                      scale2, shift2, s));
    } else {
        CK(gemm_nt(R, 512, 256, sv.h2, 256, w->c3_w + 256, 512, sv.h3, 512, e, ws, wsb, s));
        RUN(act_bn_eval_affine_f32(w->bn2_w, w->bn2_b, w->bn2_mean, w->bn2_var, d->eps2, 512, scale2, shift2, s));
    }
    {
        act_gemm_fx_t fx{}; fx.a_scale = scale2; fx.a_shift = shift2; fx.gmax = out; fx.garg = keep_for_backward ? sv.arg2 : nullptr; fx.group = n; fx.store_c = 0;
        e = epi0(); e.bias = w->c4_b;
        if (groups) {
            if (!t_collect) {
                if (hipMemsetAsync(out, 0, (size_t)BG * C * sizeof(float), s) != hipSuccess) return ACT_E_BADARG;
                if (keep_for_backward && hipMemsetAsync(sv.arg2, 0xFF, (size_t)BG * C * sizeof(int32_t), s) != hipSuccess) return ACT_E_BADARG;
            }
            fx.row_groups = groups;
            CK(gemm_fx(1, 1, n_groups * n, C, 512, sv.h3, 512, w->c4_w, 512, nullptr, C, e, fx, ws, wsb, s));
        } else {
            CK(gemm_fx(1, 1, R, C, 512, sv.h3, 512, w->c4_w, 512, nullptr, C, e, fx, ws, wsb, s));
        }
    }
    return 0;
}

int act_pointnet_bwd_f32(const act_pointnet_dims_t* d, const act_pointnet_params_t* w, const float* x, const float* saved, const float* dout,
                         const act_pointnet_grads_t* g, float* scratch, float* ws, size_t wsb, act_stream_t stream) {
    if (!w || !x || !saved || !dout || !g || !scratch) return ACT_E_NULLPTR;
    if (bad_pn(d)) return ACT_E_BADARG;
    hipStream_t s = (hipStream_t)stream;
    const int BG = d->BG, n = d->n, C = d->C, R = BG * n;
    const bool fused = pn_fused(*d), composed = pn_compose(*d);
    PnSaved sv; carve_pn(const_cast<float*>(saved), *d, sv);
    PnBwdScratch sc; carve_pn_bwd(scratch, *d, sc);
    auto st = [](float* base, int Cc, int which) { return base + which * Cc; };
    auto wgrad_act = [&](const float* dy, int N_, const float* h, const float* a, float* stt, int Cc, float* dw) -> int {
        if (!fused) return gemm_tn(N_, Cc, R, dy, N_, a, Cc, dw, Cc, ws, wsb, s);
        if (N_ % 128 == 0 && Cc % 128 == 0) {
            act_gemm_fx_t fx{}; fx.b_scale = st(stt, Cc, 2); fx.b_shift = st(stt, Cc, 3);
            return gemm_fx(0, 0, N_, Cc, R, dy, N_, h, Cc, dw, Cc, epi0(), fx, ws, wsb, s);
        }
        RUN(act_affine_act_f32(h, st(stt, Cc, 2), st(stt, Cc, 3), 1, R, Cc, sc.act, s));
        return gemm_tn(N_, Cc, R, dy, N_, sc.act, Cc, dw, Cc, ws, wsb, s);
    };
    const bool pool_on_load = pn_pool_bwd_on_load(*d);
    const int32_t* live = nullptr;
    if (pool_on_load && pn_pool_bwd_sparse()) {
        RUN(act_group_max_bwd_wgrad_f32(dout, sv.arg2, BG, n, C, sv.h3, 512, 512, st(sv.st2, 512, 2), st(sv.st2, 512, 3), g->c4_w, 512, ws, wsb, s));
        CK(colsum(dout, BG, C, g->c4_b, ws, wsb, s));
        live = pn_pool_bwd_live() ? sc.live : nullptr;
        if (live) RUN(act_group_live_i32(dout, BG, C, sc.live, s));
        RUN(act_group_max_bwd_matmul_live_f32(dout, sv.arg2, BG, n, C, w->c4_w, 512, 512, sc.da3, 512, live, s));
    } else if (pool_on_load) {
        act_gemm_fx_t fx{}; fx.sa_src = dout; fx.sa_arg = sv.arg2; fx.group = n; fx.b_scale = st(sv.st2, 512, 2); fx.b_shift = st(sv.st2, 512, 3);
        CK(gemm_fx(0, 0, C, 512, R, nullptr, C, sv.h3, 512, g->c4_w, 512, epi0(), fx, ws, wsb, s));
        CK(colsum(dout, BG, C, g->c4_b, ws, wsb, s));
        act_gemm_fx_t fa{}; fa.sa_src = dout; fa.sa_arg = sv.arg2; fa.group = n;
        CK(gemm_fx(1, 0, R, 512, C, nullptr, C, w->c4_w, 512, sc.da3, 512, epi0(), fa, ws, wsb, s));
    } else {
        RUN(act_group_max_bwd_f32(dout, sv.arg2, BG, n, C, 0, sc.dh4, s));
        CK(wgrad_act(sc.dh4, C, sv.h3, sv.a3, sv.st2, 512, g->c4_w));
        if (fused) CK(colsum(dout, BG, C, g->c4_b, ws, wsb, s));
        else       CK(colsum(sc.dh4, R, C, g->c4_b, ws, wsb, s));
        CK(gemm_nn(R, 512, C, sc.dh4, C, w->c4_w, 512, sc.da3, 512, epi0(), ws, wsb, s));
    }
    RUN(act_bn_bwd_groups_f32(sv.h3, sc.da3, st(sv.st2, 512, 2), st(sv.st2, 512, 3), st(sv.st2, 512, 0), st(sv.st2, 512, 1), 1, R, 512, live, n, sc.dh3,
                              g->bn2_w, g->bn2_b, ws, wsb, s));
    if (!composed) CK(gemm_tn(512, 256, R, sc.dh3, 512, sv.h2, 256, g->c3_w + 256, 512, ws, wsb, s));
    RUN(act_group_sum_f32(sc.dh3, BG, n, 512, sc.dgw, s));
    CK(gemm_tn(512, 256, BG, sc.dgw, 512, sv.fg, 256, g->c3_w, 512, ws, wsb, s));
    CK(colsum(sc.dgw, BG, 512, g->c3_b, ws, wsb, s));
    CK(gemm_nn(BG, 256, 512, sc.dgw, 512, w->c3_w, 512, sc.dfg, 256, epi0(), ws, wsb, s));
    if (composed) {
        act_gemm_epilogue_t ea = epi0(); ea.accumulate = 1;
        CK(wgrad_act(sc.dh3, 512, sv.h1, nullptr, sv.st1, 128, sc.g32));
        CK(gemm_nt(512, 256, 128, sc.g32, 128, w->c2_w, 128, g->c3_w + 256, 512, epi0(), ws, wsb, s));
        CK(gemm_nt(512, 256, 1, g->c3_b, 1, w->c2_b, 1, g->c3_w + 256, 512, ea, ws, wsb, s));
        RUN(act_group_max_bwd_wgrad_f32(sc.dfg, sv.arg1, BG, n, 256, sv.h1, 128, 128, st(sv.st1, 128, 2), st(sv.st1, 128, 3), g->c2_w, 128, ws, wsb, s));
        CK(gemm_tn(256, 128, 512, w->c3_w + 256, 512, sc.g32, 128, g->c2_w, 128, ea, ws, wsb, s));
        CK(colsum(sc.dfg, BG, 256, g->c2_b, ws, wsb, s));
        CK(gemm_nn(1, 256, 512, g->c3_b, 512, w->c3_w + 256, 512, g->c2_b, 256, ea, ws, wsb, s));
        RUN(act_group_max_bwd_matmul_live_f32(sc.dfg, sv.arg1, BG, n, 256, w->c2_w, 128, 128, sc.da1, 128, nullptr, s));
        CK(gemm_nn(R, 128, 512, sc.dh3, 512, sv.w32, 128, sc.da1, 128, ea, ws, wsb, s));
    } else {
        if (pool_on_load) {
            act_gemm_fx_t fe{}; fe.ep_src = sc.dfg; fe.ep_arg = sv.arg1; fe.group = n;
            CK(gemm_fx(1, 0, R, 256, 512, sc.dh3, 512, w->c3_w + 256, 512, sc.dh2, 256, epi0(), fe, ws, wsb, s));
        } else {
            CK(gemm_nn(R, 256, 512, sc.dh3, 512, w->c3_w + 256, 512, sc.dh2, 256, epi0(), ws, wsb, s));
            RUN(act_group_max_bwd_f32(sc.dfg, sv.arg1, BG, n, 256, 1, sc.dh2, s));
        }
        CK(wgrad_act(sc.dh2, 256, sv.h1, sv.a1, sv.st1, 128, g->c2_w));
        CK(colsum(sc.dh2, R, 256, g->c2_b, ws, wsb, s));
        CK(gemm_nn(R, 128, 256, sc.dh2, 256, w->c2_w, 128, sc.da1, 128, epi0(), ws, wsb, s));
    }
    RUN(act_bn_bwd_f32(sv.h1, sc.da1, st(sv.st1, 128, 2), st(sv.st1, 128, 3), st(sv.st1, 128, 0), st(sv.st1, 128, 1), 1, R, 128, sc.dh1, g->bn1_w, g->bn1_b,
                       ws, wsb, s));
    CK(gemm_tn(128, 3, R, sc.dh1, 128, x, 3, g->c1_w, 3, ws, wsb, s));
    CK(colsum(sc.dh1, R, 128, g->c1_b, ws, wsb, s));
    return 0;
}

static const int kDgcnnCin[4] = {128, 256, 512, 512}, kDgcnnCout[4] = {256, 512, 512, 1024};
static size_t carve_dgcnn(float* base, const act_dgcnn_t& m, float*& x0, float*& yz, float*& cat, float*& stats) {
    const size_t T = (size_t)m.B * m.G;
    Carver c(base);
    x0 = c.take(T * 128); yz = c.take(T * 2048); cat = c.take(T * 2304); stats = c.take((size_t)18 * m.B * m.groups);
    return c.used;
}
size_t act_dgcnn_scratch_floats(const act_dgcnn_t* m) {
    if (!m || m->B <= 0 || m->G <= 0 || m->groups <= 0) return 0;
    float *a, *b, *c, *d; return carve_dgcnn(nullptr, *m, a, b, c, d);
}
static int dgcnn_features(const act_dgcnn_t* m, const act_dgcnn_f16x3_t* x3, const float* f, const int64_t* idx, float* h, float* scratch, float* ws, size_t wsb,
                          act_stream_t stream);
int act_dgcnn_features_f32(const act_dgcnn_t* m, const float* f, const int64_t* idx, float* h, float* scratch, float* ws, size_t wsb,
                           act_stream_t stream) {
    return dgcnn_features(m, nullptr, f, idx, h, scratch, ws, wsb, stream);
}
int act_dgcnn_features_f16x3_f32(const act_dgcnn_t* m, const act_dgcnn_f16x3_t* x3, const float* f, const int64_t* idx, float* h, float* scratch,
                                 float* ws, size_t wsb, act_stream_t stream) {
    return dgcnn_features(m, x3, f, idx, h, scratch, ws, wsb, stream);
}
static int dgcnn_features(const act_dgcnn_t* m, const act_dgcnn_f16x3_t* x3, const float* f, const int64_t* idx, float* h, float* scratch, float* ws, size_t wsb,
                          act_stream_t stream) {
    if (!m || !f || !idx || !h || !scratch) return ACT_E_NULLPTR;
    if (m->B <= 0 || m->G <= 0 || m->k <= 0 || m->Cin <= 0 || m->Cout <= 0 || m->groups <= 0) return ACT_E_BADARG;
    hipStream_t s = (hipStream_t)stream;
    const int T = m->B * m->G;
    float *x0, *yz, *cat, *stats;
    carve_dgcnn(scratch, *m, x0, yz, cat, stats);
    act_gemm_epilogue_t e = epi0(); e.bias = m->b_in;
    CK(gemm_nt(T, 128, m->Cin, f, m->Cin, m->w_in, m->Cin, x0, 128, e, ws, wsb, s));
    const float* xin = x0; int ldx = 128, off = 0;
    for (int l = 0; l < 4; ++l) {
        const int cin = kDgcnnCin[l], cout = kDgcnnCout[l];
        CK(gemm_nt(T, 2 * cout, cin, xin, ldx, m->stacked[l], cin, yz, 2 * cout, epi0(), ws, wsb, s));
        RUN(act_edge_gn_lrelu_max_f32(yz, 2 * cout, cout, idx, m->B, m->G, m->k, cout, m->groups, m->gn_w[l], m->gn_b[l], m->eps, m->slope, stats,
                                     cat, 2304, off, s));
        xin = cat + off; ldx = 2304; off += cout;
    }
    if (x3 && x3->w5_planes && x3->w5_inv_scale && x3->a_planes && x3->a_scale > 0.f && x3->a_planes_elems >= (size_t)2 * T * 2304) {
        const X3Linear w5 = x3_linear_of(x3->w5_planes, (size_t)m->Cout * 2304, PlaneFmt::f16(x3->a_scale), x3->w5_inv_scale);
        if (x3_takes(w5, T, m->Cout, 2304)) return x3_linear(w5, T, m->Cout, 2304, cat, nullptr, x3->a_planes, h, nullptr, w5.a_fmt, epi0(), s);
    }
    CK(gemm_nt(T, m->Cout, 2304, cat, 2304, m->w5, 2304, h, m->Cout, epi0(), ws, wsb, s));
    return 0;
}

}
```

act_amd/csrc/gemm_bf16x3.hip:

```cpp
#include "gemm_common.h"
#include "split_planes.h"
#include <stdlib.h>

typedef short bf16x8 __attribute__((ext_vector_type(8)));
typedef _Float16 f16x8 __attribute__((ext_vector_type(8)));
typedef unsigned u32x4v __attribute__((ext_vector_type(4)));

namespace {

template <bool F16>
__global__ __launch_bounds__(256) void split_planes_kernel(const float* __restrict__ x, int K4, int ldx, long long n4, float scale,
                                                           const float* __restrict__ row_scale, unsigned short* __restrict__ p1, unsigned short* __restrict__ p2) {
    for (long long i = (long long)blockIdx.x * blockDim.x + threadIdx.x; i < n4; i += (long long)gridDim.x * blockDim.x) {
        const long long row = i / K4; const int c4 = (int)(i - row * K4);
        const float4 v = *reinterpret_cast<const float4*>(x + row * ldx + c4 * 4);
        store_planes4<F16>(p1, p2, (size_t)i, v, F16 && row_scale ? scale * row_scale[row] : scale);
    }
}

constexpr int BK = 32;
constexpr int LROW = 40;

struct X3Params {
    const unsigned short *Ah, *Al, *Bh, *Bl;
    float* C; int ldc;
    unsigned short *Oh, *Ol;
    int M, N, K;
    act_gemm_epilogue_t epi;
    const float* b_inv; float a_inv, o_scale;
};

template <bool F16>
__device__ __forceinline__ f32x4 x3_mfma(const bf16x8& b, const bf16x8& a, const f32x4& c) {
    if constexpr (F16) return __builtin_amdgcn_mfma_f32_16x16x32_f16(__builtin_bit_cast(f16x8, b), __builtin_bit_cast(f16x8, a), c, 0, 0, 0);
    else return __builtin_amdgcn_mfma_f32_16x16x32_bf16(b, a, c, 0, 0, 0);
}

constexpr int x3_wgs_per_cu(int waves) { return waves <= 4 ? 2 : 1; }

template <int BM, int BN, int WGM, int WGN, int ACT, bool PLANES, bool F16>
__global__ __launch_bounds__(64 * WGM * WGN, x3_wgs_per_cu(WGM * WGN) * WGM * WGN / 4) void sgemm_nt_bf16x3_kernel(const X3Params p) {
    constexpr int NT = 64 * WGM * WGN, RP = NT / 4;
    constexpr int WM = BM / WGM, WN = BN / WGN;
    constexpr int TM = WM / 16, TN = WN / 16;
    constexpr int PA = BM * LROW, PB = BN * LROW;
    constexpr int NA = (BM + RP - 1) / RP, NB = (BN + RP - 1) / RP;
    constexpr int STAGE = 2 * (PA + PB);
    static_assert(WM % 16 == 0 && WN % 16 == 0 && BM % 16 == 0 && BN % 16 == 0, "whole 16 x 16 blocks per wave, whole waves per staging row test");
    __shared__ __attribute__((aligned(16))) unsigned short L[2 * STAGE];
    const int tid = threadIdx.x, lane = tid & 63, wave = tid >> 6;
    const int wm = wave / WGN, wn = wave % WGN;
    const int tiles_n = p.N / BN, tiles_m = p.M / BM;
    int wg = blockIdx.x;
    {
        const int nwg = tiles_m * tiles_n, q = nwg >> 3, r = nwg & 7, xcd = wg & 7, loc = wg >> 3;
        wg = (xcd < r ? xcd * (q + 1) : r * (q + 1) + (xcd - r) * q) + loc;
    }
    constexpr int GM = 8;
    const int per_group = GM * tiles_n, group = wg / per_group, first_m = group * GM;
    const int gsz = min(tiles_m - first_m, GM), in_group = wg - group * per_group;
    const int tile_m = first_m + in_group % gsz, tile_n = in_group / gsz;
    const int m0 = tile_m * BM, n0 = tile_n * BN;
    const int K = p.K, ntiles = K / BK, last = ntiles - 1;

    constexpr int X = F16 ? 1 : 0;
    f32x4 acc[X + 1][TM][TN];
#pragma unroll
    for (int x = 0; x <= X; ++x)
#pragma unroll
        for (int i = 0; i < TM; ++i)
#pragma unroll
            for (int j = 0; j < TN; ++j) acc[x][i][j] = f32x4{0.f, 0.f, 0.f, 0.f};

    const int srow = tid >> 2, sch = tid & 3;
    const size_t goa = (size_t)(m0 + srow) * K + sch * 8, gob = (size_t)(n0 + srow) * K + sch * 8;
    const unsigned short* gA[2] = {p.Ah + goa, p.Al + goa};
    const unsigned short* gB[2] = {p.Bh + gob, p.Bl + gob};
    u32x4v ra0[2][NA], rb0[2][NB], ra1[2][NA], rb1[2][NB];
    const int s_off = srow * LROW + sch * 8;
    const int r = lane & 15, g = lane >> 4;
    const int a_off = (wm * WM + r) * LROW + g * 8, b_off = (wn * WN + r) * LROW + g * 8;
    const long long ta = (long long)(min(srow + RP * (NA - 1), BM - 1) - srow) * K, tb = (long long)(min(srow + RP * (NB - 1), BN - 1) - srow) * K;
#define X3_WHOLE(I, ROWS) (RP * ((I) + 1) <= (ROWS))
#define X3_LOAD(RA, RB, T)                                                                                                             \
    _Pragma("unroll") for (int s_ = 0; s_ < 2; ++s_) {                                                                                 \
        _Pragma("unroll") for (int i_ = 0; i_ < NA; ++i_)                                                                              \
            RA[s_][i_] = *reinterpret_cast<const u32x4v*>(gA[s_] + (X3_WHOLE(i_, BM) ? (long long)(RP * i_) * K : ta) + (T) * BK);      \
        _Pragma("unroll") for (int i_ = 0; i_ < NB; ++i_)                                                                              \
            RB[s_][i_] = *reinterpret_cast<const u32x4v*>(gB[s_] + (X3_WHOLE(i_, BN) ? (long long)(RP * i_) * K : tb) + (T) * BK);      \
    }
#define X3_STORE(RA, RB, STG)                                                                                                          \
    _Pragma("unroll") for (int s_ = 0; s_ < 2; ++s_) {                                                                                 \
        _Pragma("unroll") for (int i_ = 0; i_ < NA; ++i_)                                                                              \
            if (X3_WHOLE(i_, BM) || srow + RP * i_ < BM)                                                                               \
                *reinterpret_cast<u32x4v*>(&L[(STG) * STAGE + s_ * PA + s_off + RP * i_ * LROW]) = RA[s_][i_];                         \
        _Pragma("unroll") for (int i_ = 0; i_ < NB; ++i_)                                                                              \
            if (X3_WHOLE(i_, BN) || srow + RP * i_ < BN)                                                                               \
                *reinterpret_cast<u32x4v*>(&L[(STG) * STAGE + 2 * PA + s_ * PB + s_off + RP * i_ * LROW]) = RB[s_][i_];                \
    }
#define X3_COMPUTE(STG)                                                                                                                \
    {                                                                                                                                  \
        const unsigned short* As_ = L + (STG) * STAGE; const unsigned short* Bs_ = As_ + 2 * PA;                                       \
        bf16x8 af[TM][2];                                                                                                              \
        _Pragma("unroll") for (int i_ = 0; i_ < TM; ++i_)                                                                              \
            _Pragma("unroll") for (int s_ = 0; s_ < 2; ++s_) af[i_][s_] = *reinterpret_cast<const bf16x8*>(&As_[s_ * PA + a_off + i_ * 16 * LROW]); \
        _Pragma("unroll") for (int j_ = 0; j_ < TN; ++j_) {                                                                            \
            bf16x8 bf[2];                                                                                                              \
            _Pragma("unroll") for (int s_ = 0; s_ < 2; ++s_) bf[s_] = *reinterpret_cast<const bf16x8*>(&Bs_[s_ * PB + b_off + j_ * 16 * LROW]); \
             \
             \
            _Pragma("unroll") for (int i_ = 0; i_ < TM; ++i_) acc[X][i_][j_] = x3_mfma<F16>(bf[0], af[i_][1], acc[X][i_][j_]);           \
            _Pragma("unroll") for (int i_ = 0; i_ < TM; ++i_) acc[X][i_][j_] = x3_mfma<F16>(bf[1], af[i_][0], acc[X][i_][j_]);           \
            _Pragma("unroll") for (int i_ = 0; i_ < TM; ++i_) acc[0][i_][j_] = x3_mfma<F16>(bf[0], af[i_][0], acc[0][i_][j_]);           \
        }                                                                                                                              \
    }
    X3_LOAD(ra0, rb0, 0)
    X3_LOAD(ra1, rb1, min(1, last))
    X3_STORE(ra0, rb0, 0)
    __syncthreads();
    for (int t = 0; t < ntiles; t += 2) {
        X3_LOAD(ra0, rb0, min(t + 2, last))
        X3_COMPUTE(0)
        X3_STORE(ra1, rb1, 1)
        __syncthreads();
        X3_LOAD(ra1, rb1, min(t + 3, last))
        X3_COMPUTE(1)
        X3_STORE(ra0, rb0, 0)
        __syncthreads();
    }
#undef X3_WHOLE
#undef X3_LOAD
#undef X3_STORE
#undef X3_COMPUTE
    const bool vec = (((uintptr_t)p.C | (uintptr_t)p.epi.bias | (uintptr_t)p.epi.res | (uintptr_t)p.epi.aux) & 15) == 0 &&
                     ((p.ldc | (p.epi.res ? p.epi.ldr : 0) | (p.epi.aux ? p.epi.ldaux : 0)) & 3) == 0;
#pragma unroll
    for (int i = 0; i < TM; ++i)
#pragma unroll
        for (int j = 0; j < TN; ++j) {
            const int row = m0 + wm * WM + i * 16 + r;
            const int col = n0 + wn * WN + j * 16 + g * 4;
            float4 v = make_float4(acc[0][i][j][0], acc[0][i][j][1], acc[0][i][j][2], acc[0][i][j][3]);
            if constexpr (F16) {
                const float4 bi = *reinterpret_cast<const float4*>(p.b_inv + col);
                constexpr float W = 1.0f / 2048.0f;
                v.x = __builtin_fmaf(acc[1][i][j][0], W, v.x) * bi.x * p.a_inv; v.y = __builtin_fmaf(acc[1][i][j][1], W, v.y) * bi.y * p.a_inv;
                v.z = __builtin_fmaf(acc[1][i][j][2], W, v.z) * bi.z * p.a_inv; v.w = __builtin_fmaf(acc[1][i][j][3], W, v.w) * bi.w * p.a_inv;
            }
            if (vec) v = epilogue_apply4_act<ACT>(p.epi, v, row, col);
            else {
                v.x = epilogue_apply<ACT>(p.epi, v.x, row, col); v.y = epilogue_apply<ACT>(p.epi, v.y, row, col + 1);
                v.z = epilogue_apply<ACT>(p.epi, v.z, row, col + 2); v.w = epilogue_apply<ACT>(p.epi, v.w, row, col + 3);
            }
            if (!PLANES || p.C) {
                float* cp = p.C + (size_t)row * p.ldc + col;
                if (vec) *reinterpret_cast<float4*>(cp) = v; else { cp[0] = v.x; cp[1] = v.y; cp[2] = v.z; cp[3] = v.w; }
            }
            if constexpr (PLANES) store_planes4<F16>(p.Oh, p.Ol, ((size_t)row * p.N + col) >> 2, v, p.o_scale);
        }
}

template <int BM, int BN, int WGM, int WGN, bool F16>
int launch_x3(const X3Params& p, hipStream_t s) {
    const dim3 grid((p.M / BM) * (p.N / BN)), block(64 * WGM * WGN);
    const bool planes = p.Oh != nullptr;
    switch (p.epi.act) {
        case ACT_EPI_NONE:
            if (planes) hipLaunchKernelGGL((sgemm_nt_bf16x3_kernel<BM, BN, WGM, WGN, ACT_EPI_NONE, true, F16>), grid, block, 0, s, p);
            else        hipLaunchKernelGGL((sgemm_nt_bf16x3_kernel<BM, BN, WGM, WGN, ACT_EPI_NONE, false, F16>), grid, block, 0, s, p);
            break;
        case ACT_EPI_GELU:
            if (planes) hipLaunchKernelGGL((sgemm_nt_bf16x3_kernel<BM, BN, WGM, WGN, ACT_EPI_GELU, true, F16>), grid, block, 0, s, p);
            else        hipLaunchKernelGGL((sgemm_nt_bf16x3_kernel<BM, BN, WGM, WGN, ACT_EPI_GELU, false, F16>), grid, block, 0, s, p);
            break;
        case ACT_EPI_MUL_GELU_GRAD:
            if (planes) hipLaunchKernelGGL((sgemm_nt_bf16x3_kernel<BM, BN, WGM, WGN, ACT_EPI_MUL_GELU_GRAD, true, F16>), grid, block, 0, s, p);
            else        hipLaunchKernelGGL((sgemm_nt_bf16x3_kernel<BM, BN, WGM, WGN, ACT_EPI_MUL_GELU_GRAD, false, F16>), grid, block, 0, s, p);
            break;
        default: return ACT_E_BADARG;
    }
    ACT_LAUNCH_CHECK();
    return 0;
}

template <bool F16>
int split_planes(const float* x, int R, int K, int ldx, float scale, const float* row_scale, uint16_t* p1, uint16_t* p2, act_stream_t stream) {
    if (!x || !p1 || !p2) return ACT_E_NULLPTR;
    if (R < 0 || K <= 0 || (K & 3) || ldx < K || (ldx & 3) || (F16 && !(scale > 0.f)) || (((uintptr_t)x | (uintptr_t)p1 | (uintptr_t)p2) & 15)) return ACT_E_BADARG;
    const long long n4 = (long long)R * K / 4; if (n4 == 0) return 0;
    hipStream_t s = (hipStream_t)stream;
    ActProfScope ps(KID_ELTWISE, s, 0.0, 8.0 * R * (double)K);
    long long g = (n4 + 255) / 256; if (g > 8192) g = 8192;
    hipLaunchKernelGGL(split_planes_kernel<F16>, dim3((unsigned)g), dim3(256), 0, s, x, K / 4, ldx, n4, scale, row_scale, p1, p2);
    ACT_LAUNCH_CHECK(); return 0;
}

}

extern "C" int act_split_bf16x2_f32(const float* x, int R, int K, int ldx, uint16_t* hi, uint16_t* lo, act_stream_t stream) {
    return split_planes<false>(x, R, K, ldx, 0.f, nullptr, hi, lo, stream);
}
extern "C" int act_split_f16x2_f32(const float* x, int R, int K, int ldx, float scale, const float* row_scale, uint16_t* h1, uint16_t* h2,
                                   act_stream_t stream) {
    return split_planes<true>(x, R, K, ldx, scale, row_scale, h1, h2, stream);
}

extern "C" int act_sgemm_nt_bf16x3_supported(int M, int N, int K) { return M > 0 && N > 0 && K > 0 && M % 128 == 0 && N % 128 == 0 && K % 64 == 0; }
extern "C" int act_sgemm_nt_f16x3_supported(int M, int N, int K) { return act_sgemm_nt_bf16x3_supported(M, N, K); }

extern "C" int act_sgemm_nt_f16x3_pick_tile(int M, int N, int K, int cus) {
    if (!act_sgemm_nt_f16x3_supported(M, N, K) || cus <= 0) return 0;
    if (N % 384) return 128;
    const long long t128 = (long long)(M / 128) * (N / 128), t192 = (long long)(M / 128) * (N / 192);
    const long long tail = t128 % (2 * cus);
    const long long c128 = t128 / (2 * cus) * 4 + (tail == 0 ? 0 : tail <= cus ? 2 : 4), c192 = (t192 + cus - 1) / cus * 3;
    return 8 * c192 <= 7 * c128 ? 192 : 128;
}

namespace {
int x3_cu_count() {
    static const int n = [] {
        int dev = 0, v = 0;
        if (hipGetDevice(&dev) != hipSuccess || hipDeviceGetAttribute(&v, hipDeviceAttributeMultiprocessorCount, dev) != hipSuccess || v <= 0) v = 256;
        return v;
    }();
    return n;
}
bool x3_only_128() {
    static const bool v = [] { const char* e = getenv("ACT_X3_TILE"); return e && atoi(e) == 128; }();
    return v;
}
template <bool F16>
int multiply_planes(int M, int N, int K, const uint16_t* a1, const uint16_t* a2, float a_scale, const uint16_t* b1, const uint16_t* b2, const float* b_inv,
                    float* C, int ldc, uint16_t* o1, uint16_t* o2, float out_scale, const act_gemm_epilogue_t* epilogue, act_stream_t stream, int tile) {
    if (!a1 || !a2 || !b1 || !b2 || (F16 && !b_inv) || (!C && !o1) || ((o1 == nullptr) != (o2 == nullptr))) return ACT_E_NULLPTR;
    if (!act_sgemm_nt_bf16x3_supported(M, N, K) || (C && ldc < N) || (F16 && (!(a_scale > 0.f) || (o1 && !(out_scale > 0.f))))) return ACT_E_BADARG;
    if ((((uintptr_t)a1 | (uintptr_t)a2 | (uintptr_t)b1 | (uintptr_t)b2 | (uintptr_t)o1 | (uintptr_t)o2 | (uintptr_t)b_inv) & 15)) return ACT_E_BADARG;
    if (F16 && tile != 0 && tile != 128 && !(tile == 192 && N % 192 == 0)) return ACT_E_BADARG;
    if (F16 && tile == 0) tile = x3_only_128() ? 128 : act_sgemm_nt_f16x3_pick_tile(M, N, K, x3_cu_count());
    X3Params p{};
    p.Ah = a1; p.Al = a2; p.Bh = b1; p.Bl = b2; p.C = C; p.ldc = ldc; p.M = M; p.N = N; p.K = K; p.Oh = o1; p.Ol = o2;
    if (F16) { p.b_inv = b_inv; p.a_inv = 1.0f / a_scale; p.o_scale = out_scale; }
    if (epilogue) p.epi = *epilogue; else { p.epi = act_gemm_epilogue_t{}; p.epi.alpha = 1.0f; }
    if (p.epi.accumulate || (p.epi.act != ACT_EPI_NONE && p.epi.act != ACT_EPI_GELU && p.epi.act != ACT_EPI_MUL_GELU_GRAD)) return ACT_E_BADARG;
    hipStream_t s = (hipStream_t)stream;
    ActProfScope ps(KID_GEMM_BF16X3, s, 2.0 * M * (double)N * K, 4.0 * ((double)M * K + (double)N * K + (double)M * N));
    if constexpr (F16) return tile == 192 ? launch_x3<128, 192, 2, 4, true>(p, s) : launch_x3<128, 128, 2, 2, true>(p, s);
    else return launch_x3<128, 128, 2, 2, false>(p, s);
}
}

extern "C" int act_sgemm_nt_bf16x3_f32(int M, int N, int K, const uint16_t* a_hi, const uint16_t* a_lo, const uint16_t* b_hi, const uint16_t* b_lo,
                                       float* C, int ldc, const act_gemm_epilogue_t* epilogue, act_stream_t stream) {
    return multiply_planes<false>(M, N, K, a_hi, a_lo, 0.f, b_hi, b_lo, nullptr, C, ldc, nullptr, nullptr, 0.f, epilogue, stream, 128);
}
extern "C" int act_sgemm_nt_bf16x3_planes_f32(int M, int N, int K, const uint16_t* a_hi, const uint16_t* a_lo, const uint16_t* b_hi, const uint16_t* b_lo,
                                              float* C, int ldc, uint16_t* out_hi, uint16_t* out_lo, const act_gemm_epilogue_t* epilogue,
                                              act_stream_t stream) {
    return multiply_planes<false>(M, N, K, a_hi, a_lo, 0.f, b_hi, b_lo, nullptr, C, ldc, out_hi, out_lo, 0.f, epilogue, stream, 128);
}
extern "C" int act_sgemm_nt_f16x3_planes_f32(int M, int N, int K, const uint16_t* a_h1, const uint16_t* a_h2, float a_scale, const uint16_t* b_h1,
                                             const uint16_t* b_h2, const float* b_inv_scale, float* C, int ldc, uint16_t* out_h1, uint16_t* out_h2,
                                             float out_scale, const act_gemm_epilogue_t* epilogue, act_stream_t stream) {
    return multiply_planes<true>(M, N, K, a_h1, a_h2, a_scale, b_h1, b_h2, b_inv_scale, C, ldc, out_h1, out_h2, out_scale, epilogue, stream, 0);
}
extern "C" int act_sgemm_nt_f16x3_planes_tile_f32(int M, int N, int K, const uint16_t* a_h1, const uint16_t* a_h2, float a_scale, const uint16_t* b_h1,
                                                  const uint16_t* b_h2, const float* b_inv_scale, float* C, int ldc, uint16_t* out_h1, uint16_t* out_h2,
                                                  float out_scale, const act_gemm_epilogue_t* epilogue, act_stream_t stream, int tile) {
    return multiply_planes<true>(M, N, K, a_h1, a_h2, a_scale, b_h1, b_h2, b_inv_scale, C, ldc, out_h1, out_h2, out_scale, epilogue, stream, tile);
}
```

act_amd/kernels.py:

```python
import ctypes
import os

import numpy as np

import torch

from . import _C
from ._abi import GemmEpilogue, GemmTnProblem

EPI_NONE, EPI_GELU, EPI_RELU, EPI_MUL_GELU_GRAD, EPI_MUL_RELU_MASK = 0, 1, 2, 3, 4

lib, ptr, stream, check = _C.lib, _C.ptr, _C.stream, _C.check

_WS = {}
_WS_BYTES = 160 << 20


def workspace(device, nbytes=_WS_BYTES, stream_handle=None):
    idx = device.index if device.index is not None else torch.cuda.current_device()
    key = (idx, _C.stream_handle(idx) if stream_handle is None else stream_handle)
    w = _WS.get(key)
    if w is None or w.numel() * 4 < nbytes:
        w = torch.empty(max(nbytes, _WS_BYTES) // 4, dtype=torch.float32, device=device)
        _WS[key] = w
# ... 42 lines not shown

def _f32c(t, name="tensor"):
    if t.dtype != torch.float32:
        raise _C.ActHipError(f"{name}: expected float32")
    return t if t.is_contiguous() else t.contiguous()


def _f32rows(t, name="tensor"):
    if t.dtype != torch.float32:
        raise _C.ActHipError(f"{name}: expected float32")
    if t.dim() == 2 and t.stride(1) == 1 and t.stride(0) >= t.shape[1] and (
            t.is_contiguous() or (t.stride(0) % 4 == 0 and t.data_ptr() % 16 == 0)):
        return t
    return t.contiguous()


def gemm(a, b, a_kmajor=True, b_kmajor=True, bias=None, act=EPI_NONE, aux=None, res=None, rowscale=None,
         rows_per_scale=0, out=None, accumulate=False, alpha=1.0, res_row_div=0, cfg=None):
    a = _f32rows(a, "a"); b = _f32rows(b, "b")
    if a_kmajor:
        M, K = a.shape
    else:
        K, M = a.shape
    if b_kmajor:
        N, Kb = b.shape
    else:
        Kb, N = b.shape
    if K != Kb:
        raise _C.ActHipError(f"gemm: inner dimensions differ ({K} vs {Kb})")
    if out is None:
        out = torch.empty(M, N, dtype=torch.float32, device=a.device)
    e = GemmEpilogue(alpha=alpha, act=act, accumulate=int(accumulate), rows_per_scale=int(rows_per_scale),
                     ldr=(res.stride(0) if res is not None else 0), ldaux=(aux.stride(0) if aux is not None else 0),
                     res_row_div=int(res_row_div), bias=ptr(bias), rowscale=ptr(rowscale), res=ptr(res), aux=ptr(aux))
    ws = workspace(a.device)
    if cfg is None:
        cfg = gemm_config(a_kmajor, b_kmajor, M, N, K, a.device, a, b, ws)
    tile, splits = cfg if cfg is not None else (0, 0)
    check(lib.act_sgemm_ex_f32(int(a_kmajor), int(b_kmajor), M, N, K, _C.ptr_rows(a), a.stride(0), _C.ptr_rows(b), b.stride(0), ptr(out),
                               out.stride(0), ctypes.byref(e), ptr(ws), ws.numel() * 4, tile, splits, stream()), "act_sgemm_f32")
    return out


def gemm_tn_grouped(pairs, want_bias=True, splits=0):
    if not pairs or len(pairs) > 8:
        raise _C.ActHipError(f"gemm_tn_grouped: 1..8 problems per launch, got {len(pairs)}")
    pairs = [(_f32rows(dy, "dy"), _f32rows(x, "x")) for dy, x in pairs]
    T = pairs[0][0].shape[0]
    dev = pairs[0][0].device
    probs = (GemmTnProblem * len(pairs))()
    dws, dbs = [], []
    for i, (dy, x) in enumerate(pairs):
        if dy.dim() != 2 or x.dim() != 2 or dy.shape[0] != T or x.shape[0] != T:
            raise _C.ActHipError("gemm_tn_grouped: every operand needs the same number of rows")
        M, N = dy.shape[1], x.shape[1]
        dw = torch.empty(M, N, dtype=torch.float32, device=dev)
        db = torch.empty(M, dtype=torch.float32, device=dev) if want_bias else None
        dws.append(dw); dbs.append(db)
        probs[i] = GemmTnProblem(_C.ptr_rows(dy).value, dy.stride(0), _C.ptr_rows(x).value, x.stride(0), dw.data_ptr(), N, M, N,
                                 db.data_ptr() if db is not None else None)
    ws = workspace(dev)
    if splits <= 0:
        splits = lib.act_sgemm_tn_grouped_splits(probs, len(pairs), T)
        while splits > 1 and lib.act_sgemm_tn_grouped_workspace(probs, len(pairs), T, splits) > ws.numel() * 4:
            splits -= 1
    else:
        ws = workspace(dev, lib.act_sgemm_tn_grouped_workspace(probs, len(pairs), T, splits))
    check(lib.act_sgemm_tn_grouped_f32(probs, len(pairs), T, splits, ptr(ws), ws.numel() * 4, stream()), "act_sgemm_tn_grouped_f32")
    return dws, dbs


def split_bf16x2(x, out=None):
    x = _f32rows(x, "x")
    R, Kd = x.shape
    if out is None:
        out = torch.empty(2, R, Kd, dtype=torch.bfloat16, device=x.device)
    check(lib.act_split_bf16x2_f32(_C.ptr_rows(x), R, Kd, x.stride(0), ptr(out[0]), ptr(out[1]), stream()), "act_split_bf16x2_f32")
    return out


def layernorm_planes(x, gamma, beta, eps, pos=None):
    x = _f32c(x)
    T, D = x.shape
    planes = torch.empty(2, T, D, dtype=torch.bfloat16, device=x.device)
    check(lib.act_layernorm_fwd_planes_f32(ptr(x), ptr(_f32c(pos)) if pos is not None else None, ptr(gamma), ptr(beta), None, None, ptr(planes[0]), ptr(planes[1]),
                                           None, None, T, D, float(eps), stream()), "act_layernorm_fwd_planes_f32")
    return planes


def _x3_problem(name, dtype, a_planes, b_planes, bias, act, res, out, planes_out):
    fmt = "bf16" if dtype == torch.bfloat16 else "f16"
    _, M, Kd = a_planes.shape
    _, N, Kb = b_planes.shape
    if Kd != Kb or a_planes.dtype != dtype or b_planes.dtype != dtype or not (a_planes.is_contiguous() and b_planes.is_contiguous()):
        raise _C.ActHipError(f"{name}: contiguous {fmt} planes [2, rows, K] with equal K expected")
    if not lib.act_sgemm_nt_bf16x3_supported(M, N, Kd):
        raise _C.ActHipError(f"{name}: unsupported shape {M} x {N} x {Kd} (M, N % 128, K % 64)")
    if out is None:
        out = torch.empty(M, N, dtype=torch.float32, device=a_planes.device)
    e = GemmEpilogue(alpha=1.0, act=act, accumulate=0, rows_per_scale=0, ldr=(res.stride(0) if res is not None else 0), ldaux=0, res_row_div=0,
                     bias=ptr(bias), rowscale=None, res=ptr(res), aux=None)
    o1, o2 = (None, None)
    if planes_out is not None:
        if planes_out.dtype != dtype or tuple(planes_out.shape) != (2, M, N) or not planes_out.is_contiguous():
            raise _C.ActHipError(f"{name}: planes_out must be a contiguous {fmt} tensor [2, M, N]")
        o1, o2 = ptr(planes_out[0]), ptr(planes_out[1])
    return M, N, Kd, ptr(a_planes[0]), ptr(a_planes[1]), ptr(b_planes[0]), ptr(b_planes[1]), out, o1, o2, e


def gemm_nt_bf16x3(a_planes, b_planes, bias=None, act=EPI_NONE, res=None, out=None, planes_out=None):
    M, N, Kd, a1, a2, b1, b2, out, o1, o2, e = _x3_problem("gemm_nt_bf16x3", torch.bfloat16, a_planes, b_planes, bias, act, res, out, planes_out)
    if planes_out is not None:
        check(lib.act_sgemm_nt_bf16x3_planes_f32(M, N, Kd, a1, a2, b1, b2, ptr(out), out.stride(0), o1, o2, ctypes.byref(e), stream()),
              "act_sgemm_nt_bf16x3_planes_f32")
    else:
        check(lib.act_sgemm_nt_bf16x3_f32(M, N, Kd, a1, a2, b1, b2, ptr(out), out.stride(0), ctypes.byref(e), stream()), "act_sgemm_nt_bf16x3_f32")
    return out


def f16x3_row_scales(w):
    mx = w.detach().abs().amax(dim=1).float()
    e = torch.frexp(mx).exponent
    e = torch.where(mx > 0, e, torch.full_like(e, 15))
    one = torch.ones(e.shape, dtype=torch.float32, device=w.device)
    return torch.ldexp(one, 15 - e), torch.ldexp(one, e - 15)


def split_f16x2(x, scale=1.0, row_scale=None, out=None):
    x = _f32rows(x, "x")
    R, Kd = x.shape
    if out is None:
        out = torch.empty(2, R, Kd, dtype=torch.float16, device=x.device)
    check(lib.act_split_f16x2_f32(_C.ptr_rows(x), R, Kd, x.stride(0), float(scale), ptr(_f32c(row_scale)) if row_scale is not None else None,
                                  ptr(out[0]), ptr(out[1]), stream()), "act_split_f16x2_f32")
    return out


def layernorm_f16_planes(x, gamma, beta, eps, scale, pos=None):
    x = _f32c(x)
    T, D = x.shape
    planes = torch.empty(2, T, D, dtype=torch.float16, device=x.device)
    check(lib.act_layernorm_fwd_f16_planes_f32(ptr(x), ptr(_f32c(pos)) if pos is not None else None, ptr(gamma), ptr(beta), None, None, ptr(planes[0]),
                                               ptr(planes[1]), float(scale), None, None, T, D, float(eps), stream()), "act_layernorm_fwd_f16_planes_f32")
    return planes


def gemm_nt_f16x3(a_planes, a_scale, b_planes, b_inv_scale, bias=None, act=EPI_NONE, res=None, out=None, planes_out=None, out_scale=1.0, tile=0):
    M, N, Kd, a1, a2, b1, b2, out, o1, o2, e = _x3_problem("gemm_nt_f16x3", torch.float16, a_planes, b_planes, bias, act, res, out, planes_out)
    b_inv_scale = _f32c(b_inv_scale)
    if b_inv_scale.numel() != N:
        raise _C.ActHipError("gemm_nt_f16x3: b_inv_scale must hold one value per row of b")
    check(lib.act_sgemm_nt_f16x3_planes_tile_f32(M, N, Kd, a1, a2, float(a_scale), b1, b2, ptr(b_inv_scale), ptr(out), out.stride(0), o1, o2, float(out_scale),
                                                 ctypes.byref(e), stream(), int(tile)), "act_sgemm_nt_f16x3_planes_tile_f32")
    return out


_GEMM_CACHE = {}
AUTOTUNE = os.environ.get("ACT_GEMM_AUTOTUNE", "1") != "0"
AUTOTUNE_FULL = os.environ.get("ACT_GEMM_AUTOTUNE", "1") == "full"
_TUNE_FILE = os.environ.get("ACT_GEMM_TUNE_FILE") or os.path.join(os.path.dirname(os.path.abspath(__file__)), "gemm_tune_gfx950.json")
_GEMM_TABLE = {}
_MAX_SPLIT = int(os.environ.get("ACT_GEMM_MAX_SPLIT", "0"))
if os.environ.get("ACT_GEMM_TUNE_TABLE", "1") != "0" and os.path.exists(_TUNE_FILE):
    import json as _json
    with open(_TUNE_FILE) as _fh:
        _GEMM_TABLE = {tuple(int(v) for v in k.split(",")): tuple(c) for k, c in _json.load(_fh)["configs"].items()}
    if _MAX_SPLIT > 0:
        _GEMM_TABLE = {k: c for k, c in _GEMM_TABLE.items() if c[1] <= _MAX_SPLIT or k[4] > 8192}
_NEW_TUNED = {}
if os.environ.get("ACT_GEMM_TUNE_SAVE"):
    import atexit as _atexit

    def _dump_tuned(path=os.environ["ACT_GEMM_TUNE_SAVE"].replace("%p", str(os.getpid()))):
        import json
        merged = dict(_GEMM_TABLE); merged.update(_NEW_TUNED)
        with open(path, "w") as f:
            json.dump({"arch": "gfx950", "key": "a_kmajor,b_kmajor,M,N,K", "value": "[tile id, split-K]",
                       "configs": {",".join(str(v) for v in k): list(c) for k, c in sorted(merged.items())}}, f, indent=0)
    _atexit.register(_dump_tuned)


def stable_split(M, N, K, ws_bytes):
    nb = -(-M // 64) * -(-N // 64)
    if nb >= 384 or K < 1024:
        return 1
    s = max(1, min(8, K // 256, int(round(512.0 / nb))))
    while s > 1 and s * M * N * 4 > ws_bytes:
        s -= 1
    return s


_TILE_BN = {}


def tile_bn(tile):
    if not _TILE_BN:
        bn = ctypes.c_int()
        for t in range(1, 64):
            if lib.act_gemm_tile_info(t, None, ctypes.byref(bn), None, None) == 0:
                _TILE_BN[t] = bn.value
    return _TILE_BN[tile]


def stable_candidates(a, b, ak, bk, M, N, K, ws):
    aligned = ((a.data_ptr() | b.data_ptr()) & 15) == 0 and a.stride(0) % 4 == 0 and b.stride(0) % 4 == 0
    if not aligned or K % 32 != 0:
        return []
    sp = stable_split(M, N, K, ws.numel() * 4)
    if ak and bk:
        return [(t, sp) for t in (30, 31, 32, 10, 11, 12) if N % tile_bn(t) == 0]
    if ak and not bk:
        return [(t, sp) for t in (33, 34, 36, 35, 13, 14, 16, 15) if N % tile_bn(t) == 0]
    if not ak and not bk and M % 128 == 0 and N % 128 == 0:
        return [(33, sp), (13, sp)]
    return []


def first_use_config(a, b, ak, bk, M, N, K, ws):
    if AUTOTUNE_FULL:
        return gemm_tune(a, b, ak, bk, M, N, K, ws)[0]
    cands = stable_candidates(a, b, ak, bk, M, N, K, ws)
    if not cands:
        return 0, 0
    if len(cands) == 1:
        return cands[0]
    best, t = gemm_tune(a, b, ak, bk, M, N, K, ws, cands=cands)
    return best if t < float("inf") else (0, 0)


def gemm_candidates(ak, bk, M, N, K, ws_bytes, max_split=0):
    k32 = K % 32 == 0

    def fits(s):
        return s * M * N * 4 <= ws_bytes

    def capped(sp):
        return [s for s in sp if s <= max_split] if max_split > 0 and K <= 8192 else sp

    def quad_splits(nbq):
        sp = [1]
        if K >= 1024 and nbq < 2048:
            sp += [s for s in (2, 3, 4, 6, 8, 12, 16, 24, 32) if K // s >= 256 and fits(s) and nbq * s <= 8192]
        if K >= 65536 and nbq <= 64:
            sp += [s for s in (48, 64, 96, 128, 192, 256) if fits(s) and nbq * s <= 1024]
        if K >= 512 and nbq < 128:
            sp += [s for s in (5, 7, 9, 10, 12, 14, 16) if s not in sp and K // s >= 128 and fits(s) and nbq * s <= 512]
        return capped(sp)

    cands = []
    for tile, (bm, bn) in ((1, (128, 128)), (2, (128, 64)), (3, (64, 64))):
        nb = -(-M // bm) * -(-N // bn)
        if nb > 16384 and tile > 1:
            continue
        sp = [1]
        if K >= 1024 and nb < 2048:
            sp += [s for s in (2, 3, 4, 6, 8, 12, 16, 24, 32) if K // s >= 256 and fits(s) and nb * s <= 8192]
        sp = capped([s for s in sp if not (K // s > 8192 and nb * s < 256) or s == sp[-1]])
        cands += [(tile, s) for s in sp]
        if k32 and N % bn == 0:
            if M % bm == 0:
                cands += [(tile + 3, s) for s in sp if s <= 4]
            if M % bm == 0 or ak:
                cands += [(tile + 6, s) for s in sp]
                if ak and bk:
                    cands += [(tile + 9, s) for s in sp]
                    cands += [(29 + tile, s) for s in sp]
                    if tile in (1, 2) and M % bm == 0:
                        cands += [(19 + tile, s) for s in sp]
                    if tile == 1 and M % bm == 0 and K >= 1536:
                        cands += [(17, s) for s in sp]
        if k32 and not bk and N % 128 == 0 and ((tile == 1 and (ak or M % 128 == 0)) or (tile == 2 and ak)):
            qsp = quad_splits(-(-M // (128 if tile == 1 else 64)) * (N // 128))
            cands += [(12 + tile, s) for s in qsp]
            cands += [(32 + tile, s) for s in qsp]
        if k32 and ak and not bk and N % 64 == 0 and tile in (2, 3):
            qsp = quad_splits(-(-M // (128 if tile == 2 else 64)) * (N // 64))
            cands += [(16 if tile == 2 else 15, s) for s in qsp]
            cands += [(36 if tile == 2 else 35, s) for s in qsp]
    return cands


def gemm_tune(a, b, ak, bk, M, N, K, ws, reps=3, rounds=1, trace=None, cands=None):
    cands = list(cands) if cands is not None else gemm_candidates(ak, bk, M, N, K, ws.numel() * 4, _MAX_SPLIT)
    scratch = torch.empty(M, N, dtype=torch.float32, device=a.device)
    e = GemmEpilogue(alpha=1.0)
    best, best_t = (0, 0), float("inf")
    ev = [torch.cuda.Event(enable_timing=True) for _ in range(2)]
    for tile, sp in cands:
        def run():
            return lib.act_sgemm_ex_f32(int(ak), int(bk), M, N, K, _C.ptr_rows(a), a.stride(0), _C.ptr_rows(b), b.stride(0), ptr(scratch), N,
                                        ctypes.byref(e), ptr(ws), ws.numel() * 4, tile, sp, stream())
        if run() != 0:
            continue
        t = float("inf")
        for _ in range(rounds):
            ev[0].record()
            for _ in range(reps):
                run()
            ev[1].record()
            ev[1].synchronize()
            t = min(t, ev[0].elapsed_time(ev[1]) / reps)
        if trace is not None:
            trace.append((tile, sp, t))
        if t < best_t:
            best, best_t = (tile, sp), t
    return best, best_t
# ... 2079 lines not shown
```

include/act_hip.h:

```cpp
#ifndef ACT_HIP_H
#define ACT_HIP_H
#include <stdint.h>
#include <stddef.h>
#ifdef __cplusplus
extern "C" {
#endif

typedef void* act_stream_t;

#define ACT_E_BADARG   (-1)
#define ACT_E_NULLPTR  (-2)
#define ACT_E_UNSUPPORTED (-3)

int         act_version(void);
const char* act_arch(void);

int         act_prof_enable(int on);
int         act_prof_reset(void);
int         act_prof_num_kernels(void);
const char* act_prof_kernel_name(int id);
int         act_prof_read(int id, double* total_ms, long long* launches, double* flops, double* bytes);

size_t act_fps_scratch_floats(int B, int N);
int act_fps_f32(const float* xyz, int B, int N, int G, int32_t* idx_out, float* centers_out,
// ... 59 lines not shown

typedef struct {
    const float* A; int lda;
    const float* B; int ldb;
    float* C; int ldc;
    int M, N;
    float* bias_out;
} act_gemm_tn_problem_t;
size_t act_sgemm_tn_grouped_workspace(const act_gemm_tn_problem_t* probs, int nprob, int K, int splits);
int act_sgemm_tn_grouped_splits(const act_gemm_tn_problem_t* probs, int nprob, int K);
int act_sgemm_tn_grouped_f32(const act_gemm_tn_problem_t* probs, int nprob, int K, int splits, float* workspace, size_t workspace_bytes,
                             act_stream_t stream);

typedef struct {
    const float *a_scale, *a_shift, *b_scale, *b_shift;
    float*   tile_stats;
    float*   gmax;
    int32_t* garg;
    int      group, store_c;
    const float*   sa_src;
    const int32_t* sa_arg;
    const float*   ep_src;
    const int32_t* ep_arg;
    const int32_t* row_groups;
} act_gemm_fx_t;
size_t act_sgemm_fx_tile_stats_floats(int M, int N);
int act_gemm_fx_asm(int on);
int act_sgemm_fx_f32(int a_kmajor, int b_kmajor, int M, int N, int K, const float* A, int lda, const float* B, int ldb, float* C, int ldc,
                     const act_gemm_epilogue_t* epilogue, const act_gemm_fx_t* fx, float* workspace, size_t workspace_bytes, act_stream_t stream);
int act_bn_tiles_finalize_f32(const float* tile_stats, int tiles, int rows_per_tile, int C, const float* gamma, const float* beta, float eps,
                              float momentum, float* running_mean, float* running_var, float* mean, float* rstd, float* scale, float* shift,
                              act_stream_t stream);

int act_layernorm_fwd_f32(const float* x, const float* pos, const float* gamma, const float* beta, float* xin_out,
                          float* y, float* mean, float* rstd, int T, int D, float eps, act_stream_t stream);
int act_prompt_layernorm_fwd_f32(const float* tok, const float* ppos, int B, int P, int D, float drop_p, uint64_t seed,
                                 const uint64_t* seed_dev, const float* gamma, const float* beta, float eps, float* y,
                                 act_stream_t stream);
int act_prompt_rows_fwd_f32(const float* tok, const float* ppos, const float* mask, int B, int P, int D, float drop_p, uint64_t seed,
                            float* y, act_stream_t stream);
int act_prompt_rows_bwd_f32(const float* dy, const float* mask, int B, int P, int D, float drop_p, uint64_t seed, float* dtok, float* dppos,
                            act_stream_t stream);
size_t act_layernorm_bwd_workspace(int T, int D);
int act_layernorm_bwd_f32(const float* dy, const float* xin, const float* gamma, const float* mean, const float* rstd,
                          const float* dres, float* dx, float* dgamma, float* dbeta, int accumulate_params,
                          float* workspace, size_t workspace_bytes, int T, int D, act_stream_t stream);
size_t act_colsum_workspace(int R, int C);
int act_colsum_f32(const float* in, int R, int C, int ld, float* out, int accumulate, float* workspace,
                   size_t workspace_bytes, act_stream_t stream);

int act_attention_fwd_f32(const float* qkv, float* out, float* lse, int B, int S, int H, int head_dim, float scale,
                          act_stream_t stream);
int act_attention_fwd_prefix_f32(const float* kv0, int S0, const float* qkv1, int Sq, float* out, float* lse, int B,
                                 int H, int head_dim, float scale, act_stream_t stream);
int act_attention_bwd_f32(const float* qkv, const float* out, const float* dout, const float* lse, float* dqkv,
                          int B, int S, int H, int head_dim, float scale, act_stream_t stream);
int act_attention_bwd_prefix_f32(const float* kv0, int S0, const float* qkv1, int Sq, const float* out, const float* dout,
                                 const float* lse, float* dkv0, float* dqkv1, int B, int H, int head_dim, float scale,
                                 act_stream_t stream);

int act_cosine_loss_fwd_f32(const float* student, const float* teacher, int R, int D, float eps, float* loss_out,
                            float* row_loss, float* stats, act_stream_t stream);
int act_cosine_loss_bwd_f32(const float* student, const float* teacher, const float* stats, const float* grad_loss,
                            int R, int D, float eps, float* grad_student, act_stream_t stream);

int act_regression_loss_fwd_f32(const float* student, const float* teacher, int R, int D, int kind, float* loss_out,
                                float* row_loss, act_stream_t stream);
int act_regression_loss_bwd_f32(const float* student, const float* teacher, const float* grad_loss, int R, int D, int kind,
                                float* grad_student, act_stream_t stream);

int act_softmax_xent_fwd_f32(const float* logits, const int64_t* labels, int R, int C, float* loss_out, float* row_buf,
                             float* acc_out, act_stream_t stream);
int act_softmax_xent_bwd_f32(const float* logits, const int64_t* labels, const float* row_buf, const float* grad_loss,
                             int R, int C, float* grad_logits, act_stream_t stream);

size_t act_colstats_workspace(int R, int C);
int act_bn_stats_f32(const float* x, int R, int C, const float* gamma, const float* beta, float eps, float momentum,
                     float* running_mean, float* running_var, float* mean, float* rstd, float* scale, float* shift,
                     float* workspace, size_t workspace_bytes, act_stream_t stream);
int act_affine_act_f32(const float* x, const float* scale, const float* shift, int relu, int R, int C, float* y,
                       act_stream_t stream);
int act_bn_bwd_f32(const float* x, const float* dy, const float* scale, const float* shift, const float* mean,
                   const float* rstd, int relu, int R, int C, float* dx, float* dgamma, float* dbeta,
                   float* workspace, size_t workspace_bytes, act_stream_t stream);
int act_bn_bwd_groups_f32(const float* x, const float* dy, const float* scale, const float* shift, const float* mean, const float* rstd, int relu,
                          int R, int C, const int32_t* live, int n, float* dx, float* dgamma, float* dbeta, float* workspace,
                          size_t workspace_bytes, act_stream_t stream);
int act_col_mean_var_f32(const float* x, int R, int C, float* mean, float* var, float* workspace, size_t workspace_bytes, act_stream_t stream);
int act_bn_bwd_sums_f32(const float* x, const float* dy, const float* scale, const float* shift, const float* mean, const float* rstd,
                        int relu, int R, int C, float* sum_dy, float* sum_dy_xhat, float* workspace, size_t workspace_bytes,
                        act_stream_t stream);
int act_bn_bwd_apply_f32(const float* x, const float* dy, const float* scale, const float* shift, const float* mean, const float* rstd,
                         const float* sum_dy, const float* sum_dy_xhat, float count, int relu, int R, int C, float* dx, act_stream_t stream);
int act_group_max_f32(const float* in, int G, int n, int C, float* out, int32_t* arg, act_stream_t stream);
int act_group_max_bwd_f32(const float* dout, const int32_t* arg, int G, int n, int C, int accumulate, float* din,
                          act_stream_t stream);
int act_group_max_bwd_matmul_f32(const float* dout, const int32_t* arg, int G, int n, int C, const float* w, int ldw, int N, float* dx, int lddx,
                                 act_stream_t stream);
int act_group_live_i32(const float* d, int G, int C, int32_t* live, act_stream_t stream);
int act_group_max_bwd_matmul_live_f32(const float* dout, const int32_t* arg, int G, int n, int C, const float* w, int ldw, int N, float* dx, int lddx,
                                      const int32_t* live, act_stream_t stream);
size_t act_group_max_bwd_wgrad_workspace(int G, int n, int C, int N);
int act_group_max_bwd_wgrad_f32(const float* dout, const int32_t* arg, int G, int n, int C, const float* x, int ldx, int N, const float* scale,
                                const float* shift, float* dw, int lddw, float* workspace, size_t workspace_bytes, act_stream_t stream);
int act_group_sum_f32(const float* in, int G, int n, int C, float* out, act_stream_t stream);

int act_edge_gn_lrelu_max_f32(const float* yz, int ldy, int zoff, const int64_t* idx, int B, int G, int k, int C,
                              int groups, const float* gamma, const float* beta, float eps, float slope, float* stats,
                              float* out, int ldo, int ooff, act_stream_t stream);
int act_edge_gn_lrelu_max_bwd_f32(const float* yz, int ldy, int zoff, const int64_t* idx, int B, int G, int k, int C, int groups,
                                  const float* gamma, const float* beta, const float* stats, float slope,
                                  const float* dout, int ldd, float* dyz, float* part, float* mstat, act_stream_t stream);
int act_edge_bwd_lds(int on);
int act_gn_gumbel_argmax_gather_f32(const float* h, int B, int G, int C, int groups, const float* gamma, const float* beta,
                                    float eps, float slope, const float* noise, uint64_t seed, const uint64_t* seed_dev, float tau,
                                    const float* codebook, int D, float* stats, int64_t* index_out, float* out,
                                    float* logits_out, act_stream_t stream);
int act_gumbel_softmax_fwd_f32(const float* logits, int R, int C, const float* noise, uint64_t seed, float tau, float* y,
                               act_stream_t stream);
int act_gumbel_softmax_bwd_f32(const float* y, const float* dy, int R, int C, float tau, float* dlogits, act_stream_t stream);
int act_kl_uniform_fwd_f32(const float* logits, int B, int G, int C, float* lse, float* qbar, float* klv_out, act_stream_t stream);
int act_kl_uniform_bwd_f32(const float* logits, const float* lse, const float* qbar, const float* grad_klv, int B, int G, int C,
                           float* dlogits, act_stream_t stream);

int act_split_bf16x2_f32(const float* x, int R, int K, int ldx, uint16_t* hi, uint16_t* lo, act_stream_t stream);
int act_sgemm_nt_bf16x3_supported(int M, int N, int K);
int act_sgemm_nt_bf16x3_f32(int M, int N, int K, const uint16_t* a_hi, const uint16_t* a_lo, const uint16_t* b_hi, const uint16_t* b_lo,
                            float* C, int ldc, const act_gemm_epilogue_t* epilogue, act_stream_t stream);
int act_layernorm_fwd_planes_f32(const float* x, const float* pos, const float* gamma, const float* beta, float* xin_out, float* y,
                                 uint16_t* y_hi, uint16_t* y_lo, float* mean , float* rstd , int T, int D, float eps,
                                 act_stream_t stream);
int act_prompt_layernorm_fwd_planes_f32(const float* tok, const float* ppos, int B, int P, int D, float drop_p, uint64_t seed,
                                        const uint64_t* seed_dev, const float* gamma, const float* beta, float eps, uint16_t* y_hi, uint16_t* y_lo,
                                        act_stream_t stream);
int act_attention_fwd_prefix_planes_f32(const float* kv0, int S0, const float* qkv1, int Sq, float* out, uint16_t* out_hi, uint16_t* out_lo, float* lse,
                                        int B, int H, int head_dim, float scale, act_stream_t stream);
int act_sgemm_nt_bf16x3_planes_f32(int M, int N, int K, const uint16_t* a_hi, const uint16_t* a_lo, const uint16_t* b_hi, const uint16_t* b_lo,
                                   float* C, int ldc, uint16_t* out_hi, uint16_t* out_lo, const act_gemm_epilogue_t* epilogue, act_stream_t stream);

int act_split_f16x2_f32(const float* x, int R, int K, int ldx, float scale, const float* row_scale, uint16_t* h1, uint16_t* h2, act_stream_t stream);
int act_sgemm_nt_f16x3_supported(int M, int N, int K);
int act_sgemm_nt_f16x3_planes_f32(int M, int N, int K, const uint16_t* a_h1, const uint16_t* a_h2, float a_scale, const uint16_t* b_h1,
                                  const uint16_t* b_h2, const float* b_inv_scale, float* C, int ldc, uint16_t* out_h1, uint16_t* out_h2, float out_scale,
                                  const act_gemm_epilogue_t* epilogue, act_stream_t stream);
int act_sgemm_nt_f16x3_pick_tile(int M, int N, int K, int cus);
int act_sgemm_nt_f16x3_planes_tile_f32(int M, int N, int K, const uint16_t* a_h1, const uint16_t* a_h2, float a_scale, const uint16_t* b_h1,
                                       const uint16_t* b_h2, const float* b_inv_scale, float* C, int ldc, uint16_t* out_h1, uint16_t* out_h2,
                                       float out_scale, const act_gemm_epilogue_t* epilogue, act_stream_t stream, int tile);
int act_layernorm_fwd_f16_planes_f32(const float* x, const float* pos, const float* gamma, const float* beta, float* xin_out, float* y,
                                     uint16_t* y_h1, uint16_t* y_h2, float plane_scale, float* mean , float* rstd , int T, int D,
                                     float eps, act_stream_t stream);
int act_attention_fwd_prefix_f16_planes_f32(const float* kv0, int S0, const float* qkv1, int Sq, float* out, uint16_t* out_h1, uint16_t* out_h2,
                                            float plane_scale, float* lse, int B, int H, int head_dim, float scale, act_stream_t stream);

int act_gemm_tune_set(int a_kmajor, int b_kmajor, int M, int N, int K, int tile, int splits);
int act_gemm_tune_get(int a_kmajor, int b_kmajor, int M, int N, int K, int* tile, int* splits);
int act_gemm_tune_clear(void);
#define ACT_GEMM_LAYOUT_TN 1
#define ACT_GEMM_LAYOUT_TT 2
#define ACT_GEMM_LAYOUT_NN 4
#define ACT_GEMM_LAYOUT_NT 8
#define ACT_GEMM_NEED_ANY           0
#define ACT_GEMM_NEED_FULL_OR_MTAIL 1
#define ACT_GEMM_NEED_FULL          2
#define ACT_GEMM_NEED_OFFSET32      4
int act_gemm_tile_info(int tile, int* bm, int* bn, int* layouts, int* need);

int act_scale_rows_f32(const float* x, const float* gate, int T, int D, int rows_per_scale, float* y, act_stream_t stream);
int act_bn_eval_affine_f32(const float* gamma, const float* beta, const float* running_mean, const float* running_var, float eps,
                           int C, float* scale, float* shift, act_stream_t stream);

int act_composite_collect_begin(void);
int act_composite_collect_end(int* shapes, int max);
int act_composite_shutdown(void);

typedef struct {
    const float *norm1_w, *norm1_b, *qkv_w, *qkv_b , *proj_w, *proj_b, *norm2_w, *norm2_b,
                *fc1_w, *fc1_b, *fc2_w, *fc2_b;
} act_block_params_t;
typedef struct {
    float *norm1_w, *norm1_b, *qkv_w, *qkv_b , *proj_w, *proj_b, *norm2_w, *norm2_b, *fc1_w, *fc1_b, *fc2_w, *fc2_b;
} act_block_grads_t;
typedef struct { int B, S, D, heads, hidden; float eps; } act_block_dims_t;

size_t act_block_saved_floats(const act_block_dims_t* d);
int act_block_fwd_f32(const act_block_dims_t* d, const act_block_params_t* w, const float* x, const float* pos,
                      const float* gate1, const float* gate2, int keep_for_backward, float* saved, float* out,
                      float* workspace, size_t workspace_bytes, act_stream_t stream);
size_t act_block_bwd_scratch_floats(const act_block_dims_t* d);
int act_block_bwd_f32(const act_block_dims_t* d, const act_block_params_t* w, const float* gate1, const float* gate2,
                      const float* saved, const float* dout, float* dx, const act_block_grads_t* grads, float* scratch,
                      float* workspace, size_t workspace_bytes, float* side_workspace, size_t side_workspace_bytes,
                      act_stream_t stream, act_stream_t side_stream);

typedef struct {
    int depth;
    const act_block_params_t* blocks;
    const float* const* gate1;
    const float* const* gate2;
} act_block_stack_t;
size_t act_block_stack_saved_floats(const act_block_dims_t* d, int depth, int keep_for_backward);
size_t act_block_stack_bwd_scratch_floats(const act_block_dims_t* d, int depth);
int act_block_stack_fwd_f32(const act_block_dims_t* d, const act_block_stack_t* st, const float* x, const float* pos, int keep_for_backward,
                            float* saved, float* out, float* workspace, size_t workspace_bytes, act_stream_t stream);
int act_block_stack_bwd_f32(const act_block_dims_t* d, const act_block_stack_t* st, const float* saved, const float* dout, float* dx, float* dpos,
                            const float* dpos_in, const act_block_grads_t* grads, float* scratch, float* workspace, size_t workspace_bytes, float* side_workspace,
                            size_t side_workspace_bytes, act_stream_t stream, act_stream_t side_stream);
int act_add_f32(const float* a, const float* b, float* out, long long n, act_stream_t stream);

size_t act_prefix_block_saved_floats(const act_block_dims_t* d, int P);
int act_prefix_block_fwd_f32(const act_block_dims_t* d, int P, const act_block_params_t* w, const float* x, const float* pos,
                             const float* prm, const float* n1p, int keep_for_backward, float* saved, float* out,
                             float* workspace, size_t workspace_bytes, act_stream_t stream);
int act_prefix_block_fwd_kv_f32(const act_block_dims_t* d, int P, const act_block_params_t* w, const float* x, const float* pos,
                                const float* kvp, float* saved, float* out, float* workspace, size_t workspace_bytes, act_stream_t stream);
int act_prompt_kv_sparse(int on );
size_t act_prompt_kv_workspace(int B, int P, int D, int N);
int act_prompt_kv_fwd_f32(const float* tok, const float* ppos, int B, int P, int D, int N, float drop_p, uint64_t seed,
                          const uint64_t* seed_dev, const float* gamma, const float* beta, float eps, const float* W, const float* bias,
                          float* kvp, float* scratch, size_t scratch_bytes, float* workspace, size_t workspace_bytes, act_stream_t stream);
size_t act_prefix_block_bwd_scratch_floats(const act_block_dims_t* d, int P);
int act_prefix_block_bwd_f32(const act_block_dims_t* d, int P, const act_block_params_t* w, const float* prm, const float* saved,
                             const float* dout, float* dx, float* dprm, float* scratch, float* workspace, size_t workspace_bytes,
                             act_stream_t stream);

typedef struct {
    int B, P, G, D, heads, hidden, depth, tokens_dims, pos_hidden;
    float eps, drop_p;
    uint64_t seed_base;
    const uint64_t* seed_dev;
    const float *pos_w0, *pos_b0, *pos_w1, *pos_b1, *pre_w, *pre_b, *post_w, *post_b, *norm_w, *norm_b;
    const float* const* prompt_tok;
    const float* const* prompt_pos;
    const act_block_params_t* blocks;
} act_prefix_vit_t;
size_t act_prefix_vit_scratch_floats(const act_prefix_vit_t* m);
typedef struct {
    const uint16_t* const* w_planes;
    uint16_t* a_planes;
    size_t a_planes_elems;
} act_vit_bf16x3_t;
int act_prefix_vit_fwd_bf16x3_f32(const act_prefix_vit_t* m, const act_vit_bf16x3_t* x3, const float* tokens, const float* center, float* out,
                                  float* scratch, float* workspace, size_t workspace_bytes, act_stream_t stream);
int act_prefix_block_fwd_bf16x3_f32(const act_block_dims_t* d, int P, const act_block_params_t* w, const act_vit_bf16x3_t* x3, const float* x, const float* pos,
                                    const float* prm, int keep_for_backward, float* saved, float* out, float* workspace, size_t workspace_bytes,
                                    act_stream_t stream);
int act_prefix_block_bwd_bf16x3_f32(const act_block_dims_t* d, int P, const act_block_params_t* w, const act_vit_bf16x3_t* x3, const float* prm,
                                    const float* saved, const float* dout, float* dx, float* dprm, float* scratch, float* workspace,
                                    size_t workspace_bytes, act_stream_t stream);
int act_prefix_vit_fwd_f32(const act_prefix_vit_t* m, const float* tokens, const float* center, float* out, float* scratch,
                           float* workspace, size_t workspace_bytes, act_stream_t stream);
typedef struct {
    const uint16_t* const* w_planes;
    const float* const* w_inv_scale;
    const float* a_scale;
    uint16_t* a_planes;
    size_t a_planes_elems;
} act_vit_f16x3_t;
int act_prefix_vit_fwd_f16x3_f32(const act_prefix_vit_t* m, const act_vit_f16x3_t* x3, const float* tokens, const float* center, float* out,
                                 float* scratch, float* workspace, size_t workspace_bytes, act_stream_t stream);

typedef struct {
    const float *c1_w, *c1_b, *bn1_w, *bn1_b, *c2_w, *c2_b, *c3_w, *c3_b, *bn2_w, *bn2_b, *c4_w, *c4_b;
    float *bn1_mean, *bn1_var, *bn2_mean, *bn2_var;
} act_pointnet_params_t;
typedef struct { float *c1_w, *c1_b, *bn1_w, *bn1_b, *c2_w, *c2_b, *c3_w, *c3_b, *bn2_w, *bn2_b, *c4_w, *c4_b; } act_pointnet_grads_t;
typedef struct { int BG, n, C; float eps1, eps2, momentum1, momentum2; } act_pointnet_dims_t;
size_t act_pointnet_saved_floats(const act_pointnet_dims_t* d);
int act_pointnet_fwd_f32(const act_pointnet_dims_t* d, const act_pointnet_params_t* w, const float* x, int training,
                         int keep_for_backward, float* saved, float* out, float* workspace, size_t workspace_bytes,
                         act_stream_t stream);
int act_pointnet_fwd_groups_f32(const act_pointnet_dims_t* d, const act_pointnet_params_t* w, const float* x, int training, int keep_for_backward,
                                float* saved, float* out, const int32_t* groups, int n_groups, float* workspace, size_t workspace_bytes,
                                act_stream_t stream);
size_t act_pointnet_bwd_scratch_floats(const act_pointnet_dims_t* d);
int act_pointnet_bwd_f32(const act_pointnet_dims_t* d, const act_pointnet_params_t* w, const float* x, const float* saved,
                         const float* dout, const act_pointnet_grads_t* grads, float* scratch, float* workspace,
                         size_t workspace_bytes, act_stream_t stream);

typedef struct {
    int B, G, k, Cin, Cout, groups;
    float eps, slope;
    const float *w_in, *b_in, *w5;
    const float* stacked[4];
    const float* gn_w[4];
    const float* gn_b[4];
} act_dgcnn_t;
size_t act_dgcnn_scratch_floats(const act_dgcnn_t* m);
int act_dgcnn_features_f32(const act_dgcnn_t* m, const float* f, const int64_t* idx, float* h, float* scratch, float* workspace,
                           size_t workspace_bytes, act_stream_t stream);
typedef struct {
    const uint16_t* w5_planes;
    const float* w5_inv_scale;
    float a_scale;
    uint16_t* a_planes;
    size_t a_planes_elems;
} act_dgcnn_f16x3_t;
int act_dgcnn_features_f16x3_f32(const act_dgcnn_t* m, const act_dgcnn_f16x3_t* x3, const float* f, const int64_t* idx, float* h, float* scratch,
                                 float* workspace, size_t workspace_bytes, act_stream_t stream);

int act_three_nn_f32(const float* xyz, const float* centers, int B, int N, int G, int32_t* idx, float* weight, int32_t* adj_off,
                     int32_t* adj_ent, act_stream_t stream);
int act_interp_rows_fwd_f32(const float* P, const int32_t* idx, const float* weight, const float* xyz, const float* wxyz, const float* bias,
                            int B, int N, int G, int C, float* Y, act_stream_t stream);
int act_interp_rows_bwd_f32(const float* dY, const int32_t* adj_off, const int32_t* adj_ent, const float* weight, int B, int N, int G, int C,
                            float* dP, act_stream_t stream);
size_t act_interp_xyz_grad_workspace(long long R, int C);
int act_interp_xyz_grad_f32(const float* dY, const float* xyz, long long R, int C, float* dwxyz, float* dbias, float* workspace,
                            size_t workspace_bytes, act_stream_t stream);
int act_log_softmax_fwd_f32(const float* z, long long R, int C, float* out, act_stream_t stream);
int act_log_softmax_bwd_f32(const float* logp, const float* dout, long long R, int C, float* dz, act_stream_t stream);
size_t act_nll_weighted_workspace(long long R);
int act_nll_weighted_fwd_f32(const float* logp, const int64_t* target, const float* weight, long long R, int C, float* loss, float* wsum,
                             int64_t* correct, float* workspace, size_t workspace_bytes, act_stream_t stream);
int act_nll_weighted_bwd_f32(const int64_t* target, const float* weight, const float* wsum, const float* gloss, long long R, int C, float* dlogp,
                             act_stream_t stream);
int act_confusion_i64(const float* pred, const int64_t* target, long long R, int C, int64_t* cm, act_stream_t stream);

int act_label_branch_fwd_f32(const float* cls, const float* W, const float* gamma, const float* beta, int B, int training, float eps, float momentum,
                             float slope, float* running_mean, float* running_var, float* y, act_stream_t stream);
int act_label_branch_bwd_f32(const float* cls, const float* W, const float* gamma, const float* beta, const float* dy, int B, float eps, float slope,
                             float* dW, float* dgamma, float* dbeta, act_stream_t stream);
int act_part_eval_f32(const float* logp, const int64_t* target, int B, int N, int P, const int32_t* part2cat, const int32_t* cat_first, int ncat,
                      int32_t* pred, int32_t* counts, int shape_offset, int num_shapes, int64_t* seen, int64_t* correct, act_stream_t stream);

size_t act_scene_member_workspace(long long P, int gx, int gy);
int act_scene_member_count(const double* xyz, long long P, const double* table, int gx, int gy, int32_t* counts, int32_t* offsets, void* ws,
                           size_t ws_bytes, act_stream_t stream);
int act_scene_member_fill(const double* xyz, long long P, const double* table, int gx, int gy, const int32_t* offsets, int32_t* members, void* ws,
                          size_t ws_bytes, act_stream_t stream);
int act_scene_rows(const int32_t* members, const int32_t* member_off, const int32_t* block_ids, const int32_t* row_off, int nb, long long R,
                   int block_points, unsigned seed, unsigned room, unsigned vote, int32_t* rows, act_stream_t stream);
int act_scene_gather(const double* xyz, long long P, const double* table, const int32_t* rows, const int32_t* block_ids, const int32_t* row_off,
                     int nb, long long R, float* out, act_stream_t stream);
int act_scene_vote(const float* logp, const int32_t* rows, long long n, long long P, int C, const int32_t* label, const float* labelweights,
                   int32_t* votes, act_stream_t stream);
int act_scene_finish(const int32_t* votes, const int32_t* label, long long P, int C, int32_t* pred, int64_t* cm, act_stream_t stream);

size_t act_s3dis_sample_workspace(int B, long long max_window);
int act_s3dis_sample_f32(const double* xyz, const int32_t* labels, const long long* room_off, int R, const double* grid_origin,
                         const long long* grid_dims, const long long* cell_off, const int32_t* cell_pts, double block_size, double cell,
                         int min_points, int max_tries, long long max_window, const int32_t* room_ids, const int32_t* item_ids,
                         const int32_t* center_in, int B, int num_point, unsigned seed, unsigned epoch, float* out_xyz, int64_t* out_labels,
                         int32_t* rows, int32_t* count, int32_t* center_idx, int32_t* info, void* ws, size_t ws_bytes, act_stream_t stream);

#define ACT_CLOUD_PERMUTE   1
#define ACT_CLOUD_NORMALIZE 2
int act_cloud_sample_max_points(void);
int act_cloud_sample_f32(const float* clouds, long long M, int N, int C, const int32_t* item_ids, const int32_t* draw_ids, int B, int n,
                         unsigned seed, unsigned epoch, int flags, float* out, int32_t* src_rows, act_stream_t stream);

#define ACT_RECON_FIELDS 12
int act_recon_eval_f32(const float* coarse, const float* dense, const float* gt, int B, int nc, int nd, int N, float th, double* out, int row0,
                       int num_rows, act_stream_t stream);

int act_svm_scores_f32(const float* X, const float* W, const float* b, const float* mask, int N, int D, int K, float* out, act_stream_t stream);
size_t act_svm_hinge_workspace(int N, int K);
int act_svm_hinge_f32(const float* M, const int64_t* labels, const int64_t* classes, int N, int K, float* R, double* sums, void* workspace,
                      size_t workspace_bytes, act_stream_t stream);
size_t act_svm_tprod_workspace(int N, int D, int K);
int act_svm_tprod_f32(const float* P, const float* X, int N, int D, int K, float* out, float* colsum, void* workspace, size_t workspace_bytes,
                      act_stream_t stream);
size_t act_svm_newton_workspace(int N, int D, int K);
int act_svm_newton_f32(const float* X, const int64_t* labels, const int64_t* classes, int N, int D, int K, float C, float tol, int max_cg,
                       float* W, float* b, int32_t* istate, double* dstate, void* workspace, size_t workspace_bytes, act_stream_t stream);

size_t act_tsne_knn_workspace(int N, int D);
int act_tsne_knn_cosine_f32(const float* X, int N, int D, int k, int32_t* idx, float* dist, void* workspace, size_t workspace_bytes,
                            act_stream_t stream);
int act_tsne_conditional_p_f32(const float* dist, int N, int k, float perplexity, float* p, float* beta, act_stream_t stream);
size_t act_tsne_symmetrize_workspace(int N, int k);
int act_tsne_symmetrize_f32(const int32_t* idx, const float* p, int N, int k, int32_t* indptr, int32_t* indices, float* values,
                            long long capacity, void* workspace, size_t workspace_bytes, act_stream_t stream);
size_t act_tsne_step_workspace(int N);
int act_tsne_step_f32(const int32_t* indptr, const int32_t* indices, const float* values, int N, float exaggeration, float momentum, float lr,
                      float* Y, float* update, float* gains, void* workspace, size_t workspace_bytes, act_stream_t stream);
int act_tsne_steps_f32(const int32_t* indptr, const int32_t* indices, const float* values, int N, int n_steps, float exaggeration,
                       float momentum, float lr, float* Y, float* update, float* gains, void* workspace, size_t workspace_bytes,
                       act_stream_t stream);
int act_tsne_kl_f32(const int32_t* indptr, const int32_t* indices, const float* values, const float* Y, int N, double* out, void* workspace,
                    size_t workspace_bytes, act_stream_t stream);
size_t act_tsne_pca_workspace(int N, int D);
int act_tsne_pca_init_f32(const float* X, int N, int D, float* Y, double* info, void* workspace, size_t workspace_bytes, act_stream_t stream);

int act_dropout_add_layernorm_fwd_f32(const float* t, const float* res, const float* mask, int T, int D, float drop_p, uint64_t seed,
                                      const uint64_t* seed_dev, const float* gamma, const float* beta, float eps, float* y, float* rstd,
                                      act_stream_t stream);
int act_dropout_add_layernorm_bwd_f32(const float* dy, const float* y, const float* mask, int T, int D, float drop_p, uint64_t seed,
                                      const uint64_t* seed_dev, const float* gamma, const float* beta, const float* rstd, float* dt,
                                      float* dres, act_stream_t stream);
int act_attention_dropout_fwd_f32(const float* qkv, const uint8_t* mask, float* out, float* lse, int B, int S, int H, int head_dim,
                                  float scale, float drop_p, uint64_t seed, const uint64_t* seed_dev, act_stream_t stream);
int act_attention_dropout_bwd_f32(const float* qkv, const uint8_t* mask, const float* out, const float* dout, const float* lse,
                                  float* delta, float* dqkv, int B, int S, int H, int head_dim, float scale, float drop_p, uint64_t seed,
                                  const uint64_t* seed_dev, act_stream_t stream);

int act_quickgelu_fwd_f32(const float* pre, float* out, int rows, int cols, act_stream_t stream);
int act_quickgelu_bwd_f32(const float* pre, const float* dy, float* dx, int rows, int cols, act_stream_t stream);

int act_knn_probe_normalize_f32(const float* X, int N, int D, float* out, act_stream_t stream);
int act_knn_probe_splits(int Nq, int Nb, int kmax, int splits);
size_t act_knn_probe_workspace(int Nq, int Nb, int D, int kmax, int splits);
int act_knn_probe_search_f32(const float* Q, int Nq, const float* bank, int Nb, int D, int kmax, int normalize, int exclude_self, int splits,
                             int32_t* idx, float* sim, void* workspace, size_t workspace_bytes, act_stream_t stream);
int act_knn_probe_vote_f32(const float* sim, const int32_t* idx, int Nq, int kmax, const int32_t* bank_cls, int Nb, const int32_t* q_cls, int C,
                           const int* ks, int nk, float T, float* scores, long long* pred, long long* counts, act_stream_t stream);

int act_emd_max_points(void);
int act_emd_fwd_f32(const float* xyz1, const float* xyz2, int B, int N, float eps_final, int max_rounds, float* dist, int32_t* assignment,
                    int32_t* info, act_stream_t stream);
int act_emd_fwd_ex_f32(const float* xyz1, const float* xyz2, int B, int N, float eps_final, int max_rounds, float* dist, int32_t* assignment,
                       int32_t* info, uint64_t* evals, act_stream_t stream);
int act_emd_wave_max_points(void);
int act_emd_wave_fwd_f32(const float* xyz1, const float* xyz2, int B, int N, float eps_final, float eps_rel, int max_bids, float* dist,
                         int32_t* assignment, int32_t* info, float* eps_used, act_stream_t stream);
int act_emd_bwd_f32(const float* xyz1, const float* xyz2, const int32_t* assignment, const float* grad_dist, int B, int N, float* gx1,
                    float* gx2, act_stream_t stream);

int act_ball_query_f32(const float* xyz, const float* new_xyz, int B, int N, int S, float radius, int nsample, int inclusive, int32_t* idx,
                       int32_t* cnt, act_stream_t stream);
int act_group_rows_fwd_f32(const float* xyz, const float* new_xyz, const float* feat, const int32_t* idx, int B, int N, int S, int nsample, int D,
                           int use_xyz, float* rows, act_stream_t stream);
size_t act_group_rows_bwd_workspace(int B, int N, int S, int nsample);
int act_group_rows_bwd_f32(const float* drows, const int32_t* idx, int B, int N, int S, int nsample, int D, int use_xyz, float* dfeat,
                           void* workspace, size_t workspace_bytes, act_stream_t stream);
int act_group_gather_f32(const float* features, const int32_t* idx, int B, int C, int N, int S, int nsample, float* out, act_stream_t stream);
int act_group_gather_bwd_f32(const float* dout, const int32_t* idx, int B, int C, int N, int S, int nsample, float* dfeatures, void* workspace,
// ... 30 lines not shown
```

Baseline: 7036.

## Run frozen PointNet tokenizer's last conv as f16x3 MFMA GEMM with fused group max

For the frozen tokenizer PointNet in no-grad training mode, the final 512->C conv now runs through a new f16x3 split-precision MFMA GEMM. That kernel loads f32 activations, applies the BN2 affine and ReLU, and splits them into f16 planes on load. Its epilogue reduces the per-group max directly, so the f32 FMA GEMM path is replaced with tensor-core work and no intermediate activation planes are written. Weight planes and activation scales are cached per module. The cost is a three-product f16 approximation whose accuracy depends on a scale bound derived from the BN parameters.

```diff
diff --git a/act_amd/_abi.py b/act_amd/_abi.py
--- a/act_amd/_abi.py
+++ b/act_amd/_abi.py
@@ -68,6 +68,10 @@
 
 class DgcnnF16x3(ctypes.Structure):
     _fields_ = [("w5_planes", _vp), ("w5_inv_scale", _vp), ("a_scale", _f), ("a_planes", _vp), ("a_planes_elems", _sz)]
+
+
+class PointnetF16x3(ctypes.Structure):
+    _fields_ = [("c4_planes", _vp), ("c4_inv_scale", _vp), ("a_scale", _f)]
 
 
 class AugmentOp(ctypes.Structure):
@@ -80,6 +84,7 @@
     "act_prefix_vit_t": PrefixVit, "act_vit_bf16x3_t": VitBf16x3, "act_vit_f16x3_t": VitF16x3,
     "act_pointnet_params_t": PointnetParams,
     "act_pointnet_grads_t": PointnetGrads, "act_pointnet_dims_t": PointnetDims, "act_dgcnn_t": Dgcnn, "act_dgcnn_f16x3_t": DgcnnF16x3,
+    "act_pointnet_f16x3_t": PointnetF16x3,
     "act_augment_op_t": AugmentOp,
 }
 
@@ -172,6 +177,10 @@
     "act_sgemm_nt_f16x3_planes_tile_f32": [_i, _i, _i, _vp, _vp, _f, _vp, _vp, _vp, _vp, _i, _vp, _vp, _f, _epi, _vp, _i],
     "act_layernorm_fwd_f16_planes_f32": [_vp, _vp, _vp, _vp, _vp, _vp, _vp, _vp, _f, _vp, _vp, _i, _i, _f, _vp],
     "act_attention_fwd_prefix_f16_planes_f32": [_vp, _i, _vp, _i, _vp, _vp, _vp, _f, _vp, _i, _i, _i, _f, _vp],
+    "act_split_f16x2_affine_relu_f32": [_vp, _i, _i, _i, _vp, _vp, _f, _vp, _vp, _vp],
+    "act_sgemm_nt_f16x3_gmax_supported": [_i, _i, _i, _i],
+    "act_sgemm_nt_f16x3_gmax_pick_tile": [_i, _i, _i, _i],
+    "act_sgemm_nt_f16x3_gmax_f32": [_i, _i, _i, _vp, _i, _vp, _vp, _vp, _vp, _f, _vp, _vp, _vp, _vp, _i, _vp, _i, _i, _vp],
     "act_gemm_tune_set": [_i] * 7,
     "act_gemm_tune_get": [_i] * 5 + [_P(_i), _P(_i)],
     "act_gemm_tune_clear": [],
@@ -207,6 +216,7 @@
     "act_pointnet_saved_floats": (_sz, [_pnd]),
     "act_pointnet_fwd_f32": [_pnd, _pnp, _vp, _i, _i, _vp, _vp, _vp, _sz, _vp],
     "act_pointnet_fwd_groups_f32": [_pnd, _pnp, _vp, _i, _i, _vp, _vp, _vp, _i, _vp, _sz, _vp],
+    "act_pointnet_fwd_groups_f16x3_f32": [_pnd, _pnp, _P(PointnetF16x3), _vp, _i, _i, _vp, _vp, _vp, _i, _vp, _sz, _vp],
     "act_pointnet_bwd_scratch_floats": (_sz, [_pnd]),
     "act_pointnet_bwd_f32": [_pnd, _pnp, _vp, _vp, _vp, _P(PointnetGrads), _vp, _vp, _sz, _vp],
     "act_dgcnn_scratch_floats": (_sz, [_P(Dgcnn)]),
diff --git a/act_amd/composite.py b/act_amd/composite.py
--- a/act_amd/composite.py
+++ b/act_amd/composite.py
@@ -8,6 +8,7 @@
 from . import _C
 from . import kernels as K
 from ._abi import BlockDims, BlockParams, BlockStack, Dgcnn, PointnetDims, PointnetGrads, PointnetParams, PrefixVit, VitBf16x3, VitF16x3, DgcnnF16x3
+from ._abi import PointnetF16x3
 from ._abi import GemmFx
 
 lib, check = _C.lib, _C.check
@@ -251,6 +252,8 @@
 TEACHER_F16X3 = os.environ.get("ACT_TEACHER_F16X3", "1") != "0"
 _VIT_F16 = weakref.WeakKeyDictionary()
 TOKENIZER_F16X3 = os.environ.get("ACT_TOKENIZER_F16X3", "1") != "0"
+TOKENIZER_PN_F16X3 = os.environ.get("ACT_TOKENIZER_PN_F16X3", "1") != "0"
+_PN_F16 = weakref.WeakKeyDictionary()
 _DGCNN_F16 = weakref.WeakKeyDictionary()
 
 
@@ -548,7 +551,7 @@
 class PointnetFn(torch.autograd.Function):
 
     @staticmethod
-    def forward(ctx, x, c1w, c1b, g1, b1, c2w, c2b, c3w, c3b, g2, b2, c4w, c4b, buffers, dims, training, groups=None):
+    def forward(ctx, x, c1w, c1b, g1, b1, c2w, c2b, c3w, c3b, g2, b2, c4w, c4b, buffers, dims, training, groups=None, x3=None):
         dev = x.device
         x = K._f32c(x)
         need_grad = any(ctx.needs_input_grad)
@@ -560,7 +563,10 @@
         args = (ctypes.byref(dims), ctypes.byref(prm), _p(x), int(training), int(need_grad), _p(saved), _p(out),
                 _p(groups) if ng else None, ng, _p(ws), ws.numel() * 4)
         ensure_tuned(("pn_fwd", dims.BG, dims.n, dims.C, ng), lambda: lib.act_pointnet_fwd_groups_f32(*args, _C.stream()), dev)
-        check(lib.act_pointnet_fwd_groups_f32(*args, _C.stream()), "act_pointnet_fwd_groups_f32")
+        if x3 is not None and not need_grad:
+            check(lib.act_pointnet_fwd_groups_f16x3_f32(args[0], args[1], ctypes.byref(x3), *args[2:], _C.stream()), "act_pointnet_fwd_groups_f16x3_f32")
+        else:
+            check(lib.act_pointnet_fwd_groups_f32(*args, _C.stream()), "act_pointnet_fwd_groups_f32")
         if need_grad:
             ctx.save_for_backward(x, saved, c1w, c1b, g1, b1, c2w, c2b, c3w, c3b, g2, b2, c4w, c4b)
             ctx.dims, ctx.training = dims, bool(training)
@@ -583,7 +589,30 @@
         args = (ctypes.byref(dims), ctypes.byref(prm), _p(x), _p(saved), _p(dout), ctypes.byref(gp), _p(scratch), _p(ws), ws.numel() * 4)
         ensure_tuned(("pn_bwd", dims.BG, dims.n, dims.C), lambda: lib.act_pointnet_bwd_f32(*args, _C.stream()), dev)
         check(lib.act_pointnet_bwd_f32(*args, _C.stream()), "act_pointnet_bwd_f32")
-        return (None,) + grads + (None, None, None, None)
+        return (None,) + grads + (None, None, None, None, None)
+
+
+def f16x3_pointnet_bound(gmax, bmax, R):
+    return math.sqrt(R) * gmax + bmax
+
+
+def _pointnet_f16_planes(enc, R):
+    bn2, c4 = enc.second_conv[1], enc.second_conv[3]
+    sig = tuple((t.data_ptr(), t._version) for t in (c4.weight, bn2.weight, bn2.bias))
+    cache = _PN_F16.get(enc)
+    if cache is None or cache[0] != sig:
+        with torch.no_grad():
+            w = c4.weight.detach().reshape(c4.weight.shape[0], c4.weight.shape[1])
+            scale, inv = K.f16x3_row_scales(w)
+            planes = K.split_f16x2(w, 1.0, scale)
+            inv = inv.contiguous()
+            gmax, bmax = torch.stack([bn2.weight.detach().double().abs().max(), bn2.bias.detach().double().abs().max()]).tolist()
+        cache = _PN_F16[enc] = (sig, planes, inv, gmax, bmax, {})
+    _, planes, inv, gmax, bmax, scales = cache
+    a_scale = scales.get(R)
+    if a_scale is None:
+        a_scale = scales[R] = f16x3_act_scale(f16x3_pointnet_bound(gmax, bmax, R))
+    return PointnetF16x3(planes.data_ptr(), inv.data_ptr(), a_scale), cache
 
 
 def pointnet_forward(enc, point_groups, need=None):
@@ -601,9 +630,14 @@
             if bn.num_batches_tracked is not None:
                 bn.num_batches_tracked.add_(1)
     w2 = lambda c: c.weight.view(c.weight.shape[0], c.weight.shape[1])
+    x3 = keep = None
+    if (TOKENIZER_PN_F16X3 and groups is None and training and not torch.is_grad_enabled()
+            and not any(p.requires_grad for p in enc.parameters())):
+        x3, keep = _pointnet_f16_planes(enc, bs * g * n)
     out = PointnetFn.apply(point_groups.reshape(bs * g * n, 3), w2(c1), c1.bias, bn1.weight, bn1.bias, w2(c2), c2.bias, w2(c3), c3.bias,
                            bn2.weight, bn2.bias, w2(c4), c4.bias,
-                           (bn1.running_mean, bn1.running_var, bn2.running_mean, bn2.running_var), dims, training, groups)
+                           (bn1.running_mean, bn1.running_var, bn2.running_mean, bn2.running_var), dims, training, groups, x3)
+    del keep
     return out.reshape(bs, g, dims.C)
 
 
diff --git a/act_amd/csrc/composite.hip b/act_amd/csrc/composite.hip
--- a/act_amd/csrc/composite.hip
+++ b/act_amd/csrc/composite.hip
@@ -683,8 +683,19 @@
     return act_pointnet_fwd_groups_f32(d, w, x, training, keep_for_backward, saved, out, nullptr, 0, ws, wsb, stream);
 }
 
+static int pointnet_fwd(const act_pointnet_dims_t* d, const act_pointnet_params_t* w, const act_pointnet_f16x3_t* x3, const float* x, int training,
+                        int keep_for_backward, float* saved, float* out, const int32_t* groups, int n_groups, float* ws, size_t wsb, act_stream_t stream);
 int act_pointnet_fwd_groups_f32(const act_pointnet_dims_t* d, const act_pointnet_params_t* w, const float* x, int training, int keep_for_backward,
                                 float* saved, float* out, const int32_t* groups, int n_groups, float* ws, size_t wsb, act_stream_t stream) {
+    return pointnet_fwd(d, w, nullptr, x, training, keep_for_backward, saved, out, groups, n_groups, ws, wsb, stream);
+}
+int act_pointnet_fwd_groups_f16x3_f32(const act_pointnet_dims_t* d, const act_pointnet_params_t* w, const act_pointnet_f16x3_t* x3, const float* x,
+                                      int training, int keep_for_backward, float* saved, float* out, const int32_t* groups, int n_groups, float* ws,
+                                      size_t wsb, act_stream_t stream) {
+    return pointnet_fwd(d, w, x3, x, training, keep_for_backward, saved, out, groups, n_groups, ws, wsb, stream);
+}
+static int pointnet_fwd(const act_pointnet_dims_t* d, const act_pointnet_params_t* w, const act_pointnet_f16x3_t* x3, const float* x, int training,
+                        int keep_for_backward, float* saved, float* out, const int32_t* groups, int n_groups, float* ws, size_t wsb, act_stream_t stream) {
     if (!w || !x || !saved || !out) return ACT_E_NULLPTR;
     if (bad_pn(d)) return ACT_E_BADARG;
     if (groups && (n_groups <= 0 || ((long long)n_groups * d->n) % 128)) return ACT_E_BADARG;
@@ -747,6 +758,12 @@
     } else {
         CK(gemm_nt(R, 512, 256, sv.h2, 256, w->c3_w + 256, 512, sv.h3, 512, e, ws, wsb, s));
         RUN(act_bn_eval_affine_f32(w->bn2_w, w->bn2_b, w->bn2_mean, w->bn2_var, d->eps2, 512, scale2, shift2, s));
+    }
+    if (x3 && x3->c4_planes && x3->c4_inv_scale && x3->a_scale > 0.f && !keep_for_backward && !groups && C % 128 == 0 &&
+        act_sgemm_nt_f16x3_gmax_supported(R, C, 512, n)) {
+        if (collecting(1, 1, R, C, 512)) return 0;
+        return act_sgemm_nt_f16x3_gmax_f32(R, C, 512, sv.h3, 512, scale2, shift2, nullptr, nullptr, x3->a_scale, x3->c4_planes,
+                                           x3->c4_planes + (size_t)C * 512, x3->c4_inv_scale, w->c4_b, n, out, C, 0, s);
     }
     {
         act_gemm_fx_t fx{}; fx.a_scale = scale2; fx.a_shift = shift2; fx.gmax = out; fx.garg = keep_for_backward ? sv.arg2 : nullptr; fx.group = n; fx.store_c = 0;
diff --git a/act_amd/csrc/gemm_bf16x3.hip b/act_amd/csrc/gemm_bf16x3.hip
--- a/act_amd/csrc/gemm_bf16x3.hip
+++ b/act_amd/csrc/gemm_bf16x3.hip
@@ -8,13 +8,25 @@
 
 namespace {
 
-template <bool F16>
+__device__ __forceinline__ float4 x3_affine_relu4(const float4& a, const float4& sc, const float4& sh) {
+    return make_float4(fmaxf(__builtin_fmaf(a.x, sc.x, sh.x), 0.f), fmaxf(__builtin_fmaf(a.y, sc.y, sh.y), 0.f),
+                       fmaxf(__builtin_fmaf(a.z, sc.z, sh.z), 0.f), fmaxf(__builtin_fmaf(a.w, sc.w, sh.w), 0.f));
+}
+__device__ __forceinline__ float4 x3_scale4(const float4& a, float s) { return make_float4(a.x * s, a.y * s, a.z * s, a.w * s); }
+
+template <bool F16, bool AFF = false>
 __global__ __launch_bounds__(256) void split_planes_kernel(const float* __restrict__ x, int K4, int ldx, long long n4, float scale,
-                                                           const float* __restrict__ row_scale, unsigned short* __restrict__ p1, unsigned short* __restrict__ p2) {
+                                                           const float* __restrict__ row_scale, unsigned short* __restrict__ p1, unsigned short* __restrict__ p2,
+                                                           const float* __restrict__ col_scale = nullptr, const float* __restrict__ col_shift = nullptr) {
     for (long long i = (long long)blockIdx.x * blockDim.x + threadIdx.x; i < n4; i += (long long)gridDim.x * blockDim.x) {
         const long long row = i / K4; const int c4 = (int)(i - row * K4);
         const float4 v = *reinterpret_cast<const float4*>(x + row * ldx + c4 * 4);
-        store_planes4<F16>(p1, p2, (size_t)i, v, F16 && row_scale ? scale * row_scale[row] : scale);
+        if constexpr (AFF) {
+            const float4 sc = x3_scale4(*reinterpret_cast<const float4*>(col_scale + c4 * 4), scale), sh = x3_scale4(*reinterpret_cast<const float4*>(col_shift + c4 * 4), scale);
+            store_planes4<F16>(p1, p2, (size_t)i, x3_affine_relu4(v, sc, sh), 1.0f);
+        } else {
+            store_planes4<F16>(p1, p2, (size_t)i, v, F16 && row_scale ? scale * row_scale[row] : scale);
+        }
     }
 }
 
@@ -28,7 +40,24 @@
     int M, N, K;
     act_gemm_epilogue_t epi;
     const float* b_inv; float a_inv, o_scale;
+    const float *A32, *a_sc, *a_sh; int lda; float a_fold;
+    int group;
 };
+
+__device__ __forceinline__ void x3_affine_split8(const u32x4v& a0, const u32x4v& a1, const float* sc, const float* sh, u32x4v& h1, u32x4v& h2) {
+#pragma unroll
+    for (int half = 0; half < 2; ++half) {
+        const float4 c = *reinterpret_cast<const float4*>(sc + half * (LROW / 2)), s = *reinterpret_cast<const float4*>(sh + half * (LROW / 2));
+        const float4 v = x3_affine_relu4(__builtin_bit_cast(float4, half ? a1 : a0), c, s);
+        const float e[4] = {v.x, v.y, v.z, v.w};
+        unsigned h[4], l[4];
+#pragma unroll
+        for (int j = 0; j < 4; ++j) split_f16x2(e[j], h[j], l[j]);
+        h1[2 * half] = h[0] | (h[1] << 16); h1[2 * half + 1] = h[2] | (h[3] << 16);
+        h2[2 * half] = l[0] | (l[1] << 16); h2[2 * half + 1] = l[2] | (l[3] << 16);
+        __builtin_amdgcn_sched_barrier(0);
+    }
+}
 
 template <bool F16>
 __device__ __forceinline__ f32x4 x3_mfma(const bf16x8& b, const bf16x8& a, const f32x4& c) {
@@ -38,8 +67,10 @@
 
 constexpr int x3_wgs_per_cu(int waves) { return waves <= 4 ? 2 : 1; }
 
-template <int BM, int BN, int WGM, int WGN, int ACT, bool PLANES, bool F16>
+template <int BM, int BN, int WGM, int WGN, int ACT, bool PLANES, bool F16, bool A32 = false, bool GMAX = false>
 __global__ __launch_bounds__(64 * WGM * WGN, x3_wgs_per_cu(WGM * WGN) * WGM * WGN / 4) void sgemm_nt_bf16x3_kernel(const X3Params p) {
+    static_assert(F16 || !(A32 || GMAX), "the on-load split and the group max belong to the f16 form");
+    static_assert(!GMAX || (BM / WGM == 64 && !PLANES), "a group of 32 or 64 rows lies inside one wave's 64-row block");
     constexpr int NT = 64 * WGM * WGN, RP = NT / 4;
     constexpr int WM = BM / WGM, WN = BN / WGN;
     constexpr int TM = WM / 16, TN = WN / 16;
@@ -73,26 +104,43 @@
             for (int j = 0; j < TN; ++j) acc[x][i][j] = f32x4{0.f, 0.f, 0.f, 0.f};
 
     const int srow = tid >> 2, sch = tid & 3;
-    const size_t goa = (size_t)(m0 + srow) * K + sch * 8, gob = (size_t)(n0 + srow) * K + sch * 8;
-    const unsigned short* gA[2] = {p.Ah + goa, p.Al + goa};
+    const int lda = A32 ? p.lda : K;
+    const size_t goa = (size_t)(m0 + srow) * lda + sch * 8, gob = (size_t)(n0 + srow) * K + sch * 8;
+    const float* gA32[2] = {A32 ? p.A32 + goa : nullptr, A32 ? p.A32 + goa + 4 : nullptr};
+    const unsigned short* gA[2] = {A32 ? nullptr : p.Ah + goa, A32 ? nullptr : p.Al + goa};
     const unsigned short* gB[2] = {p.Bh + gob, p.Bl + gob};
     u32x4v ra0[2][NA], rb0[2][NB], ra1[2][NA], rb1[2][NB];
     const int s_off = srow * LROW + sch * 8;
     const int r = lane & 15, g = lane >> 4;
     const int a_off = (wm * WM + r) * LROW + g * 8, b_off = (wn * WN + r) * LROW + g * 8;
-    const long long ta = (long long)(min(srow + RP * (NA - 1), BM - 1) - srow) * K, tb = (long long)(min(srow + RP * (NB - 1), BN - 1) - srow) * K;
+    const long long ta = (long long)(min(srow + RP * (NA - 1), BM - 1) - srow) * lda, tb = (long long)(min(srow + RP * (NB - 1), BN - 1) - srow) * K;
+    const float* Lf = reinterpret_cast<const float*>(L);
+    const int sx_off = sch * 2 * (LROW / 2) + 16;
 #define X3_WHOLE(I, ROWS) (RP * ((I) + 1) <= (ROWS))
 #define X3_LOAD(RA, RB, T)                                                                                                             \
     _Pragma("unroll") for (int s_ = 0; s_ < 2; ++s_) {                                                                                 \
         _Pragma("unroll") for (int i_ = 0; i_ < NA; ++i_)                                                                              \
-            RA[s_][i_] = *reinterpret_cast<const u32x4v*>(gA[s_] + (X3_WHOLE(i_, BM) ? (long long)(RP * i_) * K : ta) + (T) * BK);      \
+            if constexpr (A32)                                                                                                         \
+                RA[s_][i_] = *reinterpret_cast<const u32x4v*>(gA32[s_] + (X3_WHOLE(i_, BM) ? (long long)(RP * i_) * lda : ta) + (T) * BK); \
+            else                                                                                                                       \
+                RA[s_][i_] = *reinterpret_cast<const u32x4v*>(gA[s_] + (X3_WHOLE(i_, BM) ? (long long)(RP * i_) * K : ta) + (T) * BK);  \
         _Pragma("unroll") for (int i_ = 0; i_ < NB; ++i_)                                                                              \
             RB[s_][i_] = *reinterpret_cast<const u32x4v*>(gB[s_] + (X3_WHOLE(i_, BN) ? (long long)(RP * i_) * K : tb) + (T) * BK);      \
     }
-#define X3_STORE(RA, RB, STG)                                                                                                          \
+#define X3_STORE(RA, RB, STG, T)                                                                                                       \
+    if constexpr (A32) {                                                                                                               \
+        __builtin_amdgcn_sched_barrier(0);                                                                                             \
+        _Pragma("unroll") for (int i_ = 0; i_ < NA; ++i_)                                                                              \
+            if (X3_WHOLE(i_, BM) || srow + RP * i_ < BM) {                                                                             \
+                u32x4v h1_, h2_;                                                                                                       \
+                x3_affine_split8(RA[0][i_], RA[1][i_], Lf + sx_off + (T) * 8 * (LROW / 2), Lf + PA / 2 + sx_off + (T) * 8 * (LROW / 2), h1_, h2_); \
+                *reinterpret_cast<u32x4v*>(&L[(STG) * STAGE + s_off + RP * i_ * LROW]) = h1_;                                          \
+                *reinterpret_cast<u32x4v*>(&L[(STG) * STAGE + PA + s_off + RP * i_ * LROW]) = h2_;                                     \
+            }                                                                                                                          \
+    }                                                                                                                                  \
     _Pragma("unroll") for (int s_ = 0; s_ < 2; ++s_) {                                                                                 \
         _Pragma("unroll") for (int i_ = 0; i_ < NA; ++i_)                                                                              \
-            if (X3_WHOLE(i_, BM) || srow + RP * i_ < BM)                                                                               \
+            if (!A32 && (X3_WHOLE(i_, BM) || srow + RP * i_ < BM))                                                                     \
                 *reinterpret_cast<u32x4v*>(&L[(STG) * STAGE + s_ * PA + s_off + RP * i_ * LROW]) = RA[s_][i_];                         \
         _Pragma("unroll") for (int i_ = 0; i_ < NB; ++i_)                                                                              \
             if (X3_WHOLE(i_, BN) || srow + RP * i_ < BN)                                                                               \
@@ -116,16 +164,24 @@
     }
     X3_LOAD(ra0, rb0, 0)
     X3_LOAD(ra1, rb1, min(1, last))
-    X3_STORE(ra0, rb0, 0)
+    if constexpr (A32) {
+        float* Lw = reinterpret_cast<float*>(L);
+        for (int q = tid; q < K / 4; q += NT) {
+            *reinterpret_cast<float4*>(&Lw[q * (LROW / 2) + 16]) = x3_scale4(*reinterpret_cast<const float4*>(p.a_sc + 4 * q), p.a_fold);
+            *reinterpret_cast<float4*>(&Lw[PA / 2 + q * (LROW / 2) + 16]) = x3_scale4(*reinterpret_cast<const float4*>(p.a_sh + 4 * q), p.a_fold);
+        }
+        __syncthreads();
+    }
+    X3_STORE(ra0, rb0, 0, 0)
     __syncthreads();
     for (int t = 0; t < ntiles; t += 2) {
         X3_LOAD(ra0, rb0, min(t + 2, last))
         X3_COMPUTE(0)
-        X3_STORE(ra1, rb1, 1)
+        X3_STORE(ra1, rb1, 1, min(t + 1, last))
         __syncthreads();
         X3_LOAD(ra1, rb1, min(t + 3, last))
         X3_COMPUTE(1)
-        X3_STORE(ra0, rb0, 0)
+        X3_STORE(ra0, rb0, 0, min(t + 2, last))
         __syncthreads();
     }
 #undef X3_WHOLE
@@ -134,24 +190,57 @@
 #undef X3_COMPUTE
     const bool vec = (((uintptr_t)p.C | (uintptr_t)p.epi.bias | (uintptr_t)p.epi.res | (uintptr_t)p.epi.aux) & 15) == 0 &&
                      ((p.ldc | (p.epi.res ? p.epi.ldr : 0) | (p.epi.aux ? p.epi.ldaux : 0)) & 3) == 0;
+    auto value = [&](int i, int j, int row, int col) -> float4 {
+        float4 v = make_float4(acc[0][i][j][0], acc[0][i][j][1], acc[0][i][j][2], acc[0][i][j][3]);
+        if constexpr (F16) {
+            const float4 bi = *reinterpret_cast<const float4*>(p.b_inv + col);
+            constexpr float W = 1.0f / 2048.0f;
+            v.x = __builtin_fmaf(acc[1][i][j][0], W, v.x) * bi.x * p.a_inv; v.y = __builtin_fmaf(acc[1][i][j][1], W, v.y) * bi.y * p.a_inv;
+            v.z = __builtin_fmaf(acc[1][i][j][2], W, v.z) * bi.z * p.a_inv; v.w = __builtin_fmaf(acc[1][i][j][3], W, v.w) * bi.w * p.a_inv;
+        }
+        if (vec) v = epilogue_apply4_act<ACT>(p.epi, v, row, col);
+        else {
+            v.x = epilogue_apply<ACT>(p.epi, v.x, row, col); v.y = epilogue_apply<ACT>(p.epi, v.y, row, col + 1);
+            v.z = epilogue_apply<ACT>(p.epi, v.z, row, col + 2); v.w = epilogue_apply<ACT>(p.epi, v.w, row, col + 3);
+        }
+        return v;
+    };
+    if constexpr (GMAX) {
+        constexpr float NINF = -__builtin_huge_valf();
+#pragma unroll
+        for (int j = 0; j < TN; ++j) {
+            const int col = n0 + wn * WN + j * 16 + g * 4;
+            float4 m[2] = {make_float4(NINF, NINF, NINF, NINF), make_float4(NINF, NINF, NINF, NINF)};
+#pragma unroll
+            for (int i = 0; i < TM; ++i) {
+                const float4 v = value(i, j, m0 + wm * WM + i * 16 + r, col);
+                float4& d = m[i / (TM / 2)];
+                d.x = fmaxf(d.x, v.x); d.y = fmaxf(d.y, v.y); d.z = fmaxf(d.z, v.z); d.w = fmaxf(d.w, v.w);
+            }
+            if (p.group == 64) { m[0].x = fmaxf(m[0].x, m[1].x); m[0].y = fmaxf(m[0].y, m[1].y); m[0].z = fmaxf(m[0].z, m[1].z); m[0].w = fmaxf(m[0].w, m[1].w); }
+#pragma unroll
+            for (int h = 0; h < 2; ++h) {
+                if (h == 1 && p.group == 64) break;
+#pragma unroll
+                for (int off = 1; off < 16; off <<= 1) {
+                    m[h].x = fmaxf(m[h].x, __shfl_xor(m[h].x, off)); m[h].y = fmaxf(m[h].y, __shfl_xor(m[h].y, off));
+                    m[h].z = fmaxf(m[h].z, __shfl_xor(m[h].z, off)); m[h].w = fmaxf(m[h].w, __shfl_xor(m[h].w, off));
+                }
+                if (r == 0) {
+                    float* cp = p.C + (size_t)((m0 + wm * WM + h * 32) / p.group) * p.ldc + col;
+                    if (vec) *reinterpret_cast<float4*>(cp) = m[h]; else { cp[0] = m[h].x; cp[1] = m[h].y; cp[2] = m[h].z; cp[3] = m[h].w; }
+                }
+            }
+        }
+        return;
+    }
 #pragma unroll
     for (int i = 0; i < TM; ++i)
 #pragma unroll
         for (int j = 0; j < TN; ++j) {
             const int row = m0 + wm * WM + i * 16 + r;
             const int col = n0 + wn * WN + j * 16 + g * 4;
-            float4 v = make_float4(acc[0][i][j][0], acc[0][i][j][1], acc[0][i][j][2], acc[0][i][j][3]);
-            if constexpr (F16) {
-                const float4 bi = *reinterpret_cast<const float4*>(p.b_inv + col);
-                constexpr float W = 1.0f / 2048.0f;
-                v.x = __builtin_fmaf(acc[1][i][j][0], W, v.x) * bi.x * p.a_inv; v.y = __builtin_fmaf(acc[1][i][j][1], W, v.y) * bi.y * p.a_inv;
-                v.z = __builtin_fmaf(acc[1][i][j][2], W, v.z) * bi.z * p.a_inv; v.w = __builtin_fmaf(acc[1][i][j][3], W, v.w) * bi.w * p.a_inv;
-            }
-            if (vec) v = epilogue_apply4_act<ACT>(p.epi, v, row, col);
-            else {
-                v.x = epilogue_apply<ACT>(p.epi, v.x, row, col); v.y = epilogue_apply<ACT>(p.epi, v.y, row, col + 1);
-                v.z = epilogue_apply<ACT>(p.epi, v.z, row, col + 2); v.w = epilogue_apply<ACT>(p.epi, v.w, row, col + 3);
-            }
+            const float4 v = value(i, j, row, col);
             if (!PLANES || p.C) {
                 float* cp = p.C + (size_t)row * p.ldc + col;
                 if (vec) *reinterpret_cast<float4*>(cp) = v; else { cp[0] = v.x; cp[1] = v.y; cp[2] = v.z; cp[3] = v.w; }
@@ -183,6 +272,15 @@
     return 0;
 }
 
+template <int BM, int BN, int WGM, int WGN>
+int launch_x3_gmax(const X3Params& p, bool a32, hipStream_t s) {
+    const dim3 grid((p.M / BM) * (p.N / BN)), block(64 * WGM * WGN);
+    if (a32) hipLaunchKernelGGL((sgemm_nt_bf16x3_kernel<BM, BN, WGM, WGN, ACT_EPI_NONE, false, true, true, true>), grid, block, 0, s, p);
+    else     hipLaunchKernelGGL((sgemm_nt_bf16x3_kernel<BM, BN, WGM, WGN, ACT_EPI_NONE, false, true, false, true>), grid, block, 0, s, p);
+    ACT_LAUNCH_CHECK();
+    return 0;
+}
+
 template <bool F16>
 int split_planes(const float* x, int R, int K, int ldx, float scale, const float* row_scale, uint16_t* p1, uint16_t* p2, act_stream_t stream) {
     if (!x || !p1 || !p2) return ACT_E_NULLPTR;
@@ -250,6 +348,41 @@
 }
 }
 
+extern "C" int act_split_f16x2_affine_relu_f32(const float* x, int R, int K, int ldx, const float* col_scale, const float* col_shift, float scale, uint16_t* h1,
+                                               uint16_t* h2, act_stream_t stream) {
+    if (!x || !col_scale || !col_shift || !h1 || !h2) return ACT_E_NULLPTR;
+    if (R < 0 || K <= 0 || (K & 3) || ldx < K || (ldx & 3) || !(scale > 0.f)) return ACT_E_BADARG;
+    if (((uintptr_t)x | (uintptr_t)h1 | (uintptr_t)h2 | (uintptr_t)col_scale | (uintptr_t)col_shift) & 15) return ACT_E_BADARG;
+    const long long n4 = (long long)R * K / 4; if (n4 == 0) return 0;
+    hipStream_t s = (hipStream_t)stream;
+    ActProfScope ps(KID_ELTWISE, s, 0.0, 8.0 * R * (double)K);
+    long long g = (n4 + 255) / 256; if (g > 8192) g = 8192;
+    hipLaunchKernelGGL((split_planes_kernel<true, true>), dim3((unsigned)g), dim3(256), 0, s, x, K / 4, ldx, n4, scale, nullptr, h1, h2, col_scale, col_shift);
+    ACT_LAUNCH_CHECK(); return 0;
+}
+extern "C" int act_sgemm_nt_f16x3_gmax_supported(int M, int N, int K, int group) {
+    return act_sgemm_nt_f16x3_supported(M, N, K) && K <= 512 && (group == 32 || group == 64);
+}
+extern "C" int act_sgemm_nt_f16x3_gmax_pick_tile(int M, int N, int K, int cus) { return act_sgemm_nt_f16x3_pick_tile(M, N, K, cus); }
+extern "C" int act_sgemm_nt_f16x3_gmax_f32(int M, int N, int K, const float* A, int lda, const float* a_col_scale, const float* a_col_shift,
+                                           const uint16_t* a_h1, const uint16_t* a_h2, float a_scale, const uint16_t* b_h1, const uint16_t* b_h2,
+                                           const float* b_inv_scale, const float* bias, int group, float* out, int ldo, int tile, act_stream_t stream) {
+    const bool a32 = A != nullptr;
+    if (!b_h1 || !b_h2 || !b_inv_scale || !out || (a32 ? (!a_col_scale || !a_col_shift) : (!a_h1 || !a_h2))) return ACT_E_NULLPTR;
+    if (!act_sgemm_nt_f16x3_gmax_supported(M, N, K, group) || ldo < N || !(a_scale > 0.f) || (a32 && (lda < K || (lda & 3)))) return ACT_E_BADARG;
+    if (((uintptr_t)A | (uintptr_t)a_col_scale | (uintptr_t)a_col_shift | (uintptr_t)a_h1 | (uintptr_t)a_h2 | (uintptr_t)b_h1 | (uintptr_t)b_h2 |
+         (uintptr_t)b_inv_scale) & 15) return ACT_E_BADARG;
+    if (tile != 0 && tile != 128 && !(tile == 192 && N % 192 == 0)) return ACT_E_BADARG;
+    if (tile == 0) tile = x3_only_128() ? 128 : act_sgemm_nt_f16x3_gmax_pick_tile(M, N, K, x3_cu_count());
+    X3Params p{};
+    p.A32 = A; p.lda = lda; p.a_sc = a_col_scale; p.a_sh = a_col_shift; p.a_fold = a_scale; p.Ah = a_h1; p.Al = a_h2; p.Bh = b_h1; p.Bl = b_h2;
+    p.C = out; p.ldc = ldo; p.M = M; p.N = N; p.K = K; p.group = group; p.b_inv = b_inv_scale; p.a_inv = 1.0f / a_scale;
+    p.epi = act_gemm_epilogue_t{}; p.epi.alpha = 1.0f; p.epi.bias = bias;
+    hipStream_t s = (hipStream_t)stream;
+    ActProfScope ps(KID_GEMM_BF16X3, s, 2.0 * M * (double)N * K, 4.0 * ((double)M * K + (double)N * K + (double)(M / group) * N));
+    return tile == 192 ? launch_x3_gmax<128, 192, 2, 4>(p, a32, s) : launch_x3_gmax<128, 128, 2, 2>(p, a32, s);
+}
+
 extern "C" int act_sgemm_nt_bf16x3_f32(int M, int N, int K, const uint16_t* a_hi, const uint16_t* a_lo, const uint16_t* b_hi, const uint16_t* b_lo,
                                        float* C, int ldc, const act_gemm_epilogue_t* epilogue, act_stream_t stream) {
     return multiply_planes<false>(M, N, K, a_hi, a_lo, 0.f, b_hi, b_lo, nullptr, C, ldc, nullptr, nullptr, 0.f, epilogue, stream, 128);
diff --git a/act_amd/kernels.py b/act_amd/kernels.py
--- a/act_amd/kernels.py
+++ b/act_amd/kernels.py
@@ -218,6 +218,36 @@
         raise _C.ActHipError("gemm_nt_f16x3: b_inv_scale must hold one value per row of b")
     check(lib.act_sgemm_nt_f16x3_planes_tile_f32(M, N, Kd, a1, a2, float(a_scale), b1, b2, ptr(b_inv_scale), ptr(out), out.stride(0), o1, o2, float(out_scale),
                                                  ctypes.byref(e), stream(), int(tile)), "act_sgemm_nt_f16x3_planes_tile_f32")
+    return out
+
+
+def split_f16x2_affine_relu(x, col_scale, col_shift, scale):
+    x = _f32rows(x, "x")
+    R, Kd = x.shape
+    out = torch.empty(2, R, Kd, dtype=torch.float16, device=x.device)
+    check(lib.act_split_f16x2_affine_relu_f32(_C.ptr_rows(x), R, Kd, x.stride(0), ptr(_f32c(col_scale)), ptr(_f32c(col_shift)), float(scale), ptr(out[0]),
+                                              ptr(out[1]), stream()), "act_split_f16x2_affine_relu_f32")
+    return out
+
+
+def gemm_nt_f16x3_gmax(a, a_scale, b_planes, b_inv_scale, group, bias=None, col_scale=None, col_shift=None, tile=0):
+    planes = a.dtype == torch.float16
+    b_planes, b_inv_scale = b_planes.contiguous(), _f32c(b_inv_scale)
+    N, Kd = b_planes.shape[1], b_planes.shape[2]
+    if planes:
+        a = a.contiguous()
+        M = a.shape[1]
+        args = (None, 0, None, None, ptr(a[0]), ptr(a[1]))
+    else:
+        a = _f32rows(a, "a")
+        M = a.shape[0]
+        args = (_C.ptr_rows(a), a.stride(0), ptr(_f32c(col_scale)), ptr(_f32c(col_shift)), None, None)
+    if a.shape[-1] != Kd or b_inv_scale.numel() != N or M % int(group):
+        raise _C.ActHipError("gemm_nt_f16x3_gmax: shapes do not match")
+    out = torch.empty(M // int(group), N, dtype=torch.float32, device=a.device)
+    check(lib.act_sgemm_nt_f16x3_gmax_f32(M, N, Kd, *args, float(a_scale), ptr(b_planes[0]), ptr(b_planes[1]), ptr(b_inv_scale),
+                                          ptr(_f32c(bias)) if bias is not None else None, int(group), ptr(out), N, int(tile), stream()),
+          "act_sgemm_nt_f16x3_gmax_f32")
     return out
 
 
diff --git a/include/act_hip.h b/include/act_hip.h
--- a/include/act_hip.h
+++ b/include/act_hip.h
@@ -235,6 +235,13 @@
                                      float eps, act_stream_t stream);
 int act_attention_fwd_prefix_f16_planes_f32(const float* kv0, int S0, const float* qkv1, int Sq, float* out, uint16_t* out_h1, uint16_t* out_h2,
                                             float plane_scale, float* lse, int B, int H, int head_dim, float scale, act_stream_t stream);
+int act_split_f16x2_affine_relu_f32(const float* x, int R, int K, int ldx, const float* col_scale, const float* col_shift, float scale, uint16_t* h1,
+                                    uint16_t* h2, act_stream_t stream);
+int act_sgemm_nt_f16x3_gmax_supported(int M, int N, int K, int group);
+int act_sgemm_nt_f16x3_gmax_pick_tile(int M, int N, int K, int cus);
+int act_sgemm_nt_f16x3_gmax_f32(int M, int N, int K, const float* A, int lda, const float* a_col_scale, const float* a_col_shift, const uint16_t* a_h1,
+                                const uint16_t* a_h2, float a_scale, const uint16_t* b_h1, const uint16_t* b_h2, const float* b_inv_scale,
+                                const float* bias, int group, float* out, int ldo, int tile, act_stream_t stream);
 
 int act_gemm_tune_set(int a_kmajor, int b_kmajor, int M, int N, int K, int tile, int splits);
 int act_gemm_tune_get(int a_kmajor, int b_kmajor, int M, int N, int K, int* tile, int* splits);
@@ -356,6 +363,14 @@
 int act_pointnet_fwd_groups_f32(const act_pointnet_dims_t* d, const act_pointnet_params_t* w, const float* x, int training, int keep_for_backward,
                                 float* saved, float* out, const int32_t* groups, int n_groups, float* workspace, size_t workspace_bytes,
                                 act_stream_t stream);
+typedef struct {
+    const uint16_t* c4_planes;
+    const float* c4_inv_scale;
+    float a_scale;
+} act_pointnet_f16x3_t;
+int act_pointnet_fwd_groups_f16x3_f32(const act_pointnet_dims_t* d, const act_pointnet_params_t* w, const act_pointnet_f16x3_t* x3, const float* x,
+                                      int training, int keep_for_backward, float* saved, float* out, const int32_t* groups, int n_groups,
+                                      float* workspace, size_t workspace_bytes, act_stream_t stream);
 size_t act_pointnet_bwd_scratch_floats(const act_pointnet_dims_t* d);
 int act_pointnet_bwd_f32(const act_pointnet_dims_t* d, const act_pointnet_params_t* w, const float* x, const float* saved,
                          const float* dout, const act_pointnet_grads_t* grads, float* scratch, float* workspace,
```

After: 7142 (median of 6 runs). 1.02x the previous value.
